# piotrmwojcik/GI-GS

Measured on AMD Instinct MI355X. Metric: train-step renders/sec (fwd+bwd, G-buffer+indirect) at 800x800; PSNR vs the CPU oracle, higher is better.
Workload: dtype f32; 1 GPU; C2 (configs[1] TensoIR lego stand-in): 300k surface Gaussians, 800x800, SH deg 2, GI step=16 start=8 delta=0.0625; P=300000, N=640000, M=9, hip_graphs=on, fused_glue=on, gi_march=proj, rasterizer=whole step = 2 hand-captured hipGraphs (fwd, bwd), asynchronous binning

## Files before the change

gi-gs_amd/build.py:

```python
from __future__ import annotations

import os
import subprocess
import sys
from concurrent.futures import ThreadPoolExecutor

HERE = os.path.dirname(os.path.abspath(__file__))
CSRC = os.path.join(HERE, "csrc")
OBJ = os.environ.get("GIGS_OBJ", os.path.join(HERE, "build"))
LIB = os.environ.get("GIGS_LIB", os.path.join(HERE, "libgigs_hip.so"))
SOURCES = ["api.hip", "preprocess.hip", "binning.hip", "blend.hip", "gi.hip", "pbr.hip", "stage2.hip", "train_glue.hip", "knn.hip", "lpips.hip",
           "image_out.hip", "mesh.hip"]
HIPCC = os.environ.get("HIPCC", "/opt/rocm/bin/hipcc")
FLAGS = [
    "-O3", "--offload-arch=gfx950", "-ffp-contract=off", "-fPIC", "-std=c++17",
    "-Wall", "-Wno-unused-function", "-Wno-unused-result", "-DNDEBUG",
] + os.environ.get("GIGS_EXTRA_FLAGS", "").split()


def _deps(src: str):
    yield os.path.join(CSRC, src)
    yield os.path.join(CSRC, "gigs_common.h")
    yield os.path.join(CSRC, "pixel_ops.h")
    yield os.path.join(HERE, "..", "include", "gigs_hip.h")


def _stale(target: str, deps) -> bool:
    if not os.path.exists(target):
        return True
    t = os.path.getmtime(target)
    return any(os.path.getmtime(d) > t for d in deps if os.path.exists(d))


def build(force: bool = False, save_temps: bool = False, verbose: bool = True) -> str:
    os.makedirs(OBJ, exist_ok=True)
    sources = [s for s in SOURCES if os.path.exists(os.path.join(CSRC, s))]
    objs, jobs = [], []
    for src in sources:
        obj = os.path.join(OBJ, src.replace(".hip", ".o"))
        objs.append(obj)
        if force or _stale(obj, _deps(src)):
            cmd = [HIPCC, *FLAGS, "-c", os.path.join(CSRC, src), "-o", obj]
            if save_temps:
                cmd += ["-save-temps=obj", "-Rpass-analysis=kernel-resource-usage"]
            jobs.append(cmd)

    def run(cmd):
        if verbose:
            print(" ".join(cmd), flush=True)
        r = subprocess.run(cmd, capture_output=True, text=True)
        if r.returncode != 0:
            raise RuntimeError("hipcc failed:\n" + " ".join(cmd) + "\n" + r.stdout + r.stderr)
        return r.stderr

    with ThreadPoolExecutor(max_workers=min(6, max(1, len(jobs)))) as ex:
        logs = list(ex.map(run, jobs))
    if save_temps:
        with open(os.path.join(OBJ, "resource_usage.txt"), "w") as f:
            f.write("\n".join(logs))
    if jobs or force or _stale(LIB, objs):
        run([HIPCC, "--offload-arch=gfx950", "-shared", "-fPIC", "-o", LIB, *objs])
    return LIB


if __name__ == "__main__":
    print(build(force="--force" in sys.argv, save_temps="--save-temps" in sys.argv))
```

gi-gs_amd/csrc/api.hip:

```cpp
#include <cstdarg>
#include <cstdio>
#include <cstdlib>
#include <cstring>
#include <map>
#include <algorithm>
#include <new>
#include <mutex>
#include <vector>

#include "../../include/gigs_hip.h"
#include "gigs_common.h"

namespace {

thread_local char g_err[512] = "";

int fail(int code, const char* fmt, ...) {
  va_list ap;
  va_start(ap, fmt);
  vsnprintf(g_err, sizeof(g_err), fmt, ap);
  va_end(ap);
  return code;
}

// ... 10 lines not shown
    if (_e == hipSuccess && debug) _e = hipStreamSynchronize(s);                           \
    if (_e != hipSuccess)                                                                  \
      return fail(GIGS_ERR_HIP, "stage '%s' failed: %s", name, hipGetErrorString(_e));     \
  } while (0)

std::mutex g_size_mu;
std::map<int, size_t> g_scan_sizes, g_sort_sizes;
size_t scan_size_cached(int P) {
  std::lock_guard<std::mutex> lk(g_size_mu);
  auto it = g_scan_sizes.find(P);
  if (it != g_scan_sizes.end()) return it->second;
  const size_t v = gigs::scan_temp_bytes(P);
  g_scan_sizes[P] = v;
  return v;
}
size_t sort_size_cached(int R) {
  int bucket = 1024;
  while (bucket < R) bucket <<= 1;
  std::lock_guard<std::mutex> lk(g_size_mu);
  auto it = g_sort_sizes.find(bucket);
  if (it != g_sort_sizes.end()) return it->second;
  const size_t v = std::max(gigs::sort_temp_bytes(bucket), gigs::long_space_bytes((size_t)gigs::kBinMaxTiles, (size_t)bucket));
  g_sort_sizes[bucket] = v;
  return v;
}

uint32_t higher_msb(uint32_t n) {
  uint32_t msb = sizeof(n) * 4;
  uint32_t step = msb;
  while (step > 1) {
    step /= 2;
    if (n >> msb) msb += step;
    else msb -= step;
  }
  if (n >> msb) msb++;
  return msb;
}

enum Stage {
  kPreprocess = 0, kScan, kDuplicate, kSort, kRanges, kBlendFwd, kBlendBwd, kPreprocessBwd,
  kDepthToNormal, kSsao, kSsr, kMedian, kBilateral, kMedianBwd, kShadeFwd, kShadeBwd,
  kCubemapFwd, kCubemapBwd, kGbufferPost, kLossFwd, kLossBwd, kL1SsimFwd, kL1SsimBwd, kTvFwd, kTvBwd,
  kMaskedL1, kAdam, kDensifyStats, kGatherRows, kDist2, kActivateFwd, kActivateBwd, kNumStages
};
const char* kStageNames[kNumStages] = {
  "preprocess_fwd", "scan", "duplicate", "sort", "tile_ranges", "blend_fwd", "blend_bwd",
  "preprocess_bwd", "depth_to_normal", "ssao", "ssr", "median3x3", "bilateral3x3",
  "median3x3_bwd", "shade_fwd", "shade_bwd", "cubemap_fwd", "cubemap_bwd", "gbuffer_post",
  "stage2_loss_fwd", "stage2_loss_bwd", "l1_ssim_fwd", "l1_ssim_bwd", "tv_loss_fwd", "tv_loss_bwd", "masked_l1",
  "adam_step", "densify_stats", "gather_rows", "dist2", "activate_fwd", "activate_bwd"};

int env_int(const char* name, int dflt) {
  const char* e = getenv(name);
  return (e && e[0]) ? atoi(e) : dflt;
}
gigs::Options options_from_env() {
  gigs::Options o;
  const char* b = getenv("GIGS_BINNING");
  o.binning_legacy = (b && strcmp(b, "legacy") == 0) ? 1 : 0;
  o.bucket_max_mean = env_int("GIGS_BUCKET_MAX_MEAN", gigs::kBucketMaxMeanList);
  const char* ll = getenv("GIGS_LONG_LISTS");
  o.long_lists = (ll && ll[0]) ? (ll[0] == '1' ? 1 : 0) : -1;
  o.bucket_target = std::max(256, env_int("GIGS_BUCKET_TARGET", 1536));
  o.bin_bands = std::max(0, env_int("GIGS_BIN_BANDS", 0));
  o.blend_cull = env_int("GIGS_BLEND_CULL", 1) != 0;
  o.pre_bwd_sh_skip = env_int("GIGS_PRE_BWD_SH_SKIP", 1) != 0;
  o.gi_march = 4;
  if (const char* e = getenv("GIGS_GI_MARCH")) {
    if (strcmp(e, "exact") == 0) o.gi_march = 0;
  }
  o.gi_cert = env_int("GIGS_GI_CERT", 1) != 0;
  o.gi_interleave = env_int("GIGS_GI_INTERLEAVE", 1) != 0;
  o.gi_tile_log2w = env_int("GIGS_GI_TILE_LOG2W", 3);
  if (o.gi_tile_log2w < 0 || o.gi_tile_log2w > 6) o.gi_tile_log2w = 3;
  o.gi_zero_rays = env_int("GIGS_GI_ZERO_RAYS", 0) != 0;
  o.spec_max8 = env_int("GIGS_SPEC_MAX8", 128);
  o.spec_max16 = env_int("GIGS_SPEC_MAX16", 1500);
  o.shade_lds_floats = env_int("GIGS_SHADE_LDS_FLOATS", 30 * 1024);
  o.shade_bwd_blocks = std::max(0, env_int("GIGS_SHADE_BWD_BLOCKS", 0));
  o.shade_bwd_rows = env_int("GIGS_SHADE_BWD_ROWS", 0) != 0;
  o.spec_sparse = env_int("GIGS_SPEC_SPARSE", 1) != 0;
  o.spec_sparse_permille = env_int("GIGS_SPEC_SPARSE_PERMILLE", 37);
  if (o.spec_sparse_permille < 0 || o.spec_sparse_permille > 1000) o.spec_sparse_permille = 37;
  return o;
}
const gigs::Ctx& ctx_of(const gigs_ctx* c) { return c ? *reinterpret_cast<const gigs::Ctx*>(c) : gigs::default_ctx(); }

struct ProfRec { int stage; hipEvent_t a, b; };
std::mutex g_prof_mu;
bool g_prof_on = false;
std::vector<ProfRec> g_prof_recs;
std::vector<hipEvent_t> g_prof_pool;

hipEvent_t prof_event() {
  if (!g_prof_pool.empty()) {
    hipEvent_t e = g_prof_pool.back();
    g_prof_pool.pop_back();
    return e;
  }
  hipEvent_t e;
  hipEventCreate(&e);
  return e;
}

struct StageScope {
  hipStream_t s;
  int stage;
  bool on;
  hipEvent_t a, b;
  StageScope(int stage_, hipStream_t s_) : s(s_), stage(stage_), on(false) {
    std::lock_guard<std::mutex> lk(g_prof_mu);
    if (!g_prof_on) return;
    on = true;
    a = prof_event();
    b = prof_event();
    hipEventRecord(a, s);
  }
  ~StageScope() {
    if (!on) return;
    hipEventRecord(b, s);
    std::lock_guard<std::mutex> lk(g_prof_mu);
    g_prof_recs.push_back({stage, a, b});
  }
};

}

namespace gigs {
const Options& default_options() {
  static const Options o = options_from_env();
  return o;
}
const Ctx& default_ctx() {
  static const Ctx c = {default_options(), 0u, nullptr, nullptr, 0, nullptr, nullptr};
  return c;
}
}

extern "C" {
__attribute__((visibility("hidden"))) const gigs::Options* gigs_internal_options(const gigs_ctx* ctx) { return &ctx_of(ctx).opt; }
__attribute__((visibility("hidden"))) int gigs_internal_fail(int code, const char* msg) { return fail(code, "%s", msg); }
__attribute__((visibility("hidden"))) void gigs_internal_stage_begin(int stage, void* stream, void** token) {
  *token = new StageScope(stage, (hipStream_t)stream);
}
__attribute__((visibility("hidden"))) void gigs_internal_stage_end(void* token) { delete (StageScope*)token; }
}

extern "C" {

const char* gigs_last_error(void) { return g_err; }
const char* gigs_build_arch(void) { return "gfx950"; }

size_t gigs_required_geom(int P) {
  if (P < 0) { fail(GIGS_ERR_INVALID, "P < 0"); return 0; }
  return gigs::required_bytes<gigs::GeomState>((size_t)P, scan_size_cached(P));
}
size_t gigs_required_image(int width, int height) {
  const size_t N = (size_t)width * height;
  const size_t T = (size_t)((width + GIGS_BLOCK_X - 1) / GIGS_BLOCK_X) * ((height + GIGS_BLOCK_Y - 1) / GIGS_BLOCK_Y);
  return gigs::required_bytes<gigs::ImageState>(N, T);
}
size_t gigs_required_binning(int R) {
  if (R < 0) { fail(GIGS_ERR_INVALID, "R < 0"); return 0; }
  return gigs::required_bytes<gigs::BinningState>((size_t)R, sort_size_cached(R));
}

long long gigs_geom_offset(int P, int which) {
  char* base = nullptr;
  char* p = base;
  gigs::GeomState g = gigs::GeomState::fromChunk(p, (size_t)P, 0);
  const void* ptrs[] = {g.depths, g.pos_view, g.means2D, g.cov3D, g.conic_opacity, g.rgb,
                        g.clamped, g.tiles_touched, g.point_offsets, g.internal_radii, g.brec, g.grec};
  if (which < 0 || which >= (int)(sizeof(ptrs) / sizeof(ptrs[0]))) return -1;
  return (long long)((const char*)ptrs[which] - base);
}
long long gigs_binning_offset(int R, int which) {
  char* base = nullptr;
  char* p = base;
  gigs::BinningState b = gigs::BinningState::fromChunk(p, (size_t)R, 0);
  const void* ptrs[] = {b.keys_unsorted, b.values_unsorted, b.keys, b.point_list, b.hit_mask};
  if (which < 0 || which >= 5) return -1;
  return (long long)((const char*)ptrs[which] - base);
}
long long gigs_image_offset(int width, int height, int which) {
  const size_t N = (size_t)width * height;
  const size_t T = (size_t)((width + GIGS_BLOCK_X - 1) / GIGS_BLOCK_X) * ((height + GIGS_BLOCK_Y - 1) / GIGS_BLOCK_Y);
  char* base = nullptr;
  char* p = base;
  gigs::ImageState s = gigs::ImageState::fromChunk(p, N, T);
  const void* ptrs[] = {s.final_T, s.n_contrib, s.ranges, s.tile_order};
  if (which < 0 || which >= 4) return -1;
  return (long long)((const char*)ptrs[which] - base);
}

gigs_ctx* gigs_ctx_create(void) {
  gigs::Ctx* c = new (std::nothrow) gigs::Ctx(gigs::default_ctx());
  if (!c) fail(GIGS_ERR_ALLOC, "gigs_ctx_create: out of host memory");
  return reinterpret_cast<gigs_ctx*>(c);
}
void gigs_ctx_destroy(gigs_ctx* ctx) { delete reinterpret_cast<gigs::Ctx*>(ctx); }

int gigs_ctx_get_options(const gigs_ctx* ctx, gigs_options* out) {
  if (!out || out->struct_bytes < (int)sizeof(gigs_options)) return fail(GIGS_ERR_INVALID, "gigs_ctx_get_options: set struct_bytes = sizeof(gigs_options)");
  const gigs::Options& o = ctx_of(ctx).opt;
  out->struct_bytes = (int)sizeof(gigs_options);
  out->binning_legacy = o.binning_legacy; out->bucket_max_mean = o.bucket_max_mean; out->long_lists = o.long_lists;
  out->bucket_target = o.bucket_target; out->bin_bands = o.bin_bands; out->blend_cull = o.blend_cull; out->pre_bwd_sh_skip = o.pre_bwd_sh_skip;
  out->gi_march = o.gi_march; out->gi_cert = o.gi_cert; out->gi_interleave = o.gi_interleave;
  out->gi_tile_log2w = o.gi_tile_log2w; out->gi_zero_rays = o.gi_zero_rays; out->spec_max8 = o.spec_max8;
  out->spec_max16 = o.spec_max16; out->shade_lds_floats = o.shade_lds_floats; out->shade_bwd_blocks = o.shade_bwd_blocks;
  out->shade_bwd_rows = o.shade_bwd_rows; out->spec_sparse = o.spec_sparse; out->spec_sparse_permille = o.spec_sparse_permille;
  return 0;
}
int gigs_ctx_set_options(gigs_ctx* ctx, const gigs_options* in) {
  if (!ctx) return fail(GIGS_ERR_INVALID, "gigs_ctx_set_options: the default context is immutable, create one");
  if (!in || in->struct_bytes < (int)sizeof(gigs_options)) return fail(GIGS_ERR_INVALID, "gigs_ctx_set_options: set struct_bytes = sizeof(gigs_options)");
  if (in->gi_march != 0 && in->gi_march != 4) return fail(GIGS_ERR_INVALID, "gi_march must be 0 (exact) or 4 (proj)");
  if (in->gi_tile_log2w < 0 || in->gi_tile_log2w > 6) return fail(GIGS_ERR_INVALID, "gi_tile_log2w must be 0..6");
  if (in->long_lists < -1 || in->long_lists > 1) return fail(GIGS_ERR_INVALID, "long_lists must be -1, 0 or 1");
  if (in->bucket_target < 256 || in->bucket_max_mean < 0 || in->bin_bands < 0 || in->bin_bands > 64)
    return fail(GIGS_ERR_INVALID, "bucket_target >= 256, bucket_max_mean >= 0, 0 <= bin_bands <= 64");
  if (in->spec_max8 < 0 || in->spec_max16 < in->spec_max8) return fail(GIGS_ERR_INVALID, "0 <= spec_max8 <= spec_max16");
  if (in->shade_lds_floats < 0 || in->shade_bwd_blocks < 0) return fail(GIGS_ERR_INVALID, "shade_lds_floats, shade_bwd_blocks >= 0");
  if (in->spec_sparse_permille < 0 || in->spec_sparse_permille > 1000) return fail(GIGS_ERR_INVALID, "0 <= spec_sparse_permille <= 1000");
  gigs::Options& o = reinterpret_cast<gigs::Ctx*>(ctx)->opt;
  o.binning_legacy = in->binning_legacy != 0; o.bucket_max_mean = in->bucket_max_mean; o.long_lists = in->long_lists;
  o.bucket_target = in->bucket_target; o.bin_bands = in->bin_bands; o.blend_cull = in->blend_cull != 0; o.pre_bwd_sh_skip = in->pre_bwd_sh_skip != 0;
  o.gi_march = in->gi_march; o.gi_cert = in->gi_cert != 0; o.gi_interleave = in->gi_interleave != 0;
  o.gi_tile_log2w = in->gi_tile_log2w; o.gi_zero_rays = in->gi_zero_rays != 0; o.spec_max8 = in->spec_max8;
  o.spec_max16 = in->spec_max16; o.shade_lds_floats = in->shade_lds_floats; o.shade_bwd_blocks = in->shade_bwd_blocks;
  o.shade_bwd_rows = in->shade_bwd_rows != 0; o.spec_sparse = in->spec_sparse != 0; o.spec_sparse_permille = in->spec_sparse_permille;
  return 0;
}
int gigs_ctx_set_reuse_binning(gigs_ctx* ctx, int on) {
  if (!ctx) return fail(GIGS_ERR_INVALID, "gigs_ctx_set_reuse_binning: the default context is immutable, create one");
  reinterpret_cast<gigs::Ctx*>(ctx)->reuse_binning = on != 0;
  return 0;
}
int gigs_ctx_set_split_sh(gigs_ctx* ctx, const float* sh_rest) {
  if (!ctx) return fail(GIGS_ERR_INVALID, "gigs_ctx_set_split_sh: the default context is immutable, create one");
  reinterpret_cast<gigs::Ctx*>(ctx)->sh_rest = sh_rest;
  return 0;
}
int gigs_ctx_set_materials_only(gigs_ctx* ctx, void* violations) {
  if (!ctx) return fail(GIGS_ERR_INVALID, "gigs_ctx_set_materials_only: the default context is immutable, create one");
  reinterpret_cast<gigs::Ctx*>(ctx)->materials_only = reinterpret_cast<unsigned*>(violations);
  return 0;
}
int gigs_ctx_set_blend_begin_event(gigs_ctx* ctx, void* hip_event) {
  if (!ctx) return fail(GIGS_ERR_INVALID, "gigs_ctx_set_blend_begin_event: the default context is immutable, create one");
  reinterpret_cast<gigs::Ctx*>(ctx)->blend_begin_event = hip_event;
  return 0;
}

__global__ void __launch_bounds__(64) stream_delay_kernel(unsigned ticks) {
  const unsigned long long t0 = wall_clock64();
  while (wall_clock64() - t0 < (unsigned long long)ticks) __builtin_amdgcn_s_sleep(8);
}

int gigs_stream_delay(unsigned nanoseconds, void* stream) {
  if (nanoseconds == 0) return 0;
  const unsigned ns = nanoseconds > 1000000u ? 1000000u : nanoseconds;
  hipLaunchKernelGGL(stream_delay_kernel, dim3(1), dim3(64), 0, (hipStream_t)stream, (ns + 9u) / 10u);
  return hipGetLastError() == hipSuccess ? 0 : gigs_internal_fail(GIGS_ERR_HIP, "stream_delay: launch failed");
}

int gigs_ctx_set_async_binning(gigs_ctx* ctx, int r_capacity, unsigned* device_counters) {
  if (!ctx) return fail(GIGS_ERR_INVALID, "gigs_ctx_set_async_binning: the default context is immutable, create one");
  gigs::Ctx* c = reinterpret_cast<gigs::Ctx*>(ctx);
  c->async_capacity = r_capacity > 0 ? (unsigned)r_capacity : 0u;
  c->async_counters = r_capacity > 0 ? device_counters : nullptr;
  return 0;
}

void gigs_profile_begin(void) {
  std::lock_guard<std::mutex> lk(g_prof_mu);
  for (auto& r : g_prof_recs) { g_prof_pool.push_back(r.a); g_prof_pool.push_back(r.b); }
  g_prof_recs.clear();
  g_prof_on = true;
}

int gigs_profile_end(float* total_ms, int* launches, int n) {
  std::vector<ProfRec> recs;
  {
    std::lock_guard<std::mutex> lk(g_prof_mu);
    g_prof_on = false;
    recs.swap(g_prof_recs);
  }
  for (int i = 0; i < n; i++) { total_ms[i] = 0.0f; launches[i] = 0; }
  for (auto& r : recs) {
    hipEventSynchronize(r.b);
    float ms = 0.0f;
    if (hipEventElapsedTime(&ms, r.a, r.b) == hipSuccess && r.stage < n) {
      total_ms[r.stage] += ms;
      launches[r.stage] += 1;
    }
  }
  std::lock_guard<std::mutex> lk(g_prof_mu);
  for (auto& r : recs) { g_prof_pool.push_back(r.a); g_prof_pool.push_back(r.b); }
  return kNumStages;
}

const char* gigs_profile_stage_name(int stage) {
  return (stage >= 0 && stage < kNumStages) ? kStageNames[stage] : "";
}

int gigs_forward(gigs_ctx* ctx, gigs_alloc_fn geometryBuffer, void* geom_user, gigs_alloc_fn binningBuffer,
                 void* binning_user, gigs_alloc_fn imageBuffer, void* image_user, int P, int D, int M,
                 const float* background, int width, int height, const float* means3D,
                 const float* shs, const float* colors_precomp, const float* opacities,
                 const float* normal, const float* albedo, const float* roughness,
                 const float* metallic, const float* scales, float scale_modifier,
                 const float* rotations, const float* cov3D_precomp, const float* viewmatrix,
                 const float* projmatrix, const float* cam_pos, float tan_fovx, float tan_fovy,
                 int prefiltered, int argmax_depth, int inference, float* out_color,
                 float* out_opacity, float* out_depth, float* out_normal, float* out_normal_view,
                 float* out_pos, float* out_albedo, float* out_roughness, float* out_metallic,
                 int* radii, int debug, void* stream) {
  (void)prefiltered;
  hipStream_t s = (hipStream_t)stream;
  const gigs::Ctx& cx = ctx_of(ctx);
  const gigs::Options& opt = cx.opt;
  if (P < 0 || width <= 0 || height <= 0) return fail(GIGS_ERR_INVALID, "bad P / image size");
  if (P == 0) return 0;
  if (!geometryBuffer || !binningBuffer || !imageBuffer) return fail(GIGS_ERR_INVALID, "null allocation callback");
  if (!means3D || !opacities || !normal || !albedo || !roughness || !metallic || !viewmatrix ||
      !projmatrix || !cam_pos || !background)
    return fail(GIGS_ERR_INVALID, "null required input");
  if (!shs && !colors_precomp) return fail(GIGS_ERR_INVALID, "provide SHs or precomputed colors");
  if (!cov3D_precomp && (!scales || !rotations)) return fail(GIGS_ERR_INVALID, "provide scales+rotations or cov3D_precomp");
  if (!colors_precomp && (M <= 0 || (D + 1) * (D + 1) > M || D > 3)) return fail(GIGS_ERR_INVALID, "SH degree %d needs (D+1)^2 <= M=%d, D <= 3", D, M);

  gigs::FwdArgs a;
  a.P = P; a.D = D; a.M = M; a.W = width; a.H = height;
  a.gx = (width + GIGS_BLOCK_X - 1) / GIGS_BLOCK_X;
  a.gy = (height + GIGS_BLOCK_Y - 1) / GIGS_BLOCK_Y;
  a.focal_y = height / (2.0f * tan_fovy);
  a.focal_x = width / (2.0f * tan_fovx);
  a.tan_fovx = tan_fovx; a.tan_fovy = tan_fovy; a.scale_modifier = scale_modifier;
  a.means3D = means3D; a.shs = shs; a.colors_precomp = colors_precomp; a.opacities = opacities;
  a.normal = normal; a.albedo = albedo; a.roughness = roughness; a.metallic = metallic;
  a.scales = scales; a.rotations = rotations; a.cov3D_precomp = cov3D_precomp;
  a.viewmatrix = viewmatrix; a.projmatrix = projmatrix; a.cam_pos = cam_pos; a.background = background;
  a.argmax_depth = argmax_depth; a.inference = inference;
  a.shs_rest = (shs && !colors_precomp && M > 1) ? cx.sh_rest : nullptr;

  const size_t scan_sz = scan_size_cached(P);
  const size_t geom_bytes = gigs::required_bytes<gigs::GeomState>((size_t)P, scan_sz);
  char* geom_chunk = geometryBuffer(geom_bytes, geom_user);
  if (!geom_chunk) return fail(GIGS_ERR_ALLOC, "geometry buffer allocation of %zu bytes failed", geom_bytes);
  gigs::GeomState geom = gigs::GeomState::fromChunk(geom_chunk, (size_t)P, scan_sz);
  if (radii == nullptr) radii = geom.internal_radii;

  const size_t N = (size_t)width * height, T = (size_t)a.gx * a.gy;
  const size_t img_bytes = gigs::required_bytes<gigs::ImageState>(N, T);
  char* img_chunk = imageBuffer(img_bytes, image_user);
  if (!img_chunk) return fail(GIGS_ERR_ALLOC, "image buffer allocation of %zu bytes failed", img_bytes);
  gigs::ImageState img = gigs::ImageState::fromChunk(img_chunk, N, T);

  {
    StageScope sc(kPreprocess, s);
    gigs::launch_preprocess_fwd(a, geom, radii, s);
  }
  STAGE_CHECK("preprocess");
  int num_rendered = 0;
  gigs::BinningState bin;
  const unsigned async_cap = cx.async_capacity;
  const bool bucket = !opt.binning_legacy && T <= (size_t)gigs::kBinMaxTiles;
  if (async_cap > 0 && !bucket) return fail(GIGS_ERR_INVALID, "asynchronous binning needs the tile-bucketed path (options.binning_legacy = 0, <= %d tiles)", gigs::kBinMaxTiles);
  auto long_lists = [&](size_t est_mean) {
    if (opt.long_lists >= 0) return opt.long_lists == 1;
    return est_mean > (size_t)opt.bucket_max_mean;
  };
  bool dense = false;
  if (cx.reuse_binning) {
    if (async_cap == 0 || !bucket)
      return fail(GIGS_ERR_INVALID, "reuse_binning needs asynchronous binning (gigs_ctx_set_async_binning) on the tile-bucketed path");
    num_rendered = (int)async_cap;
    const size_t sort_sz = sort_size_cached(num_rendered);
    const size_t bin_bytes = gigs::required_bytes<gigs::BinningState>((size_t)num_rendered, sort_sz);
    char* bin_chunk = binningBuffer(bin_bytes, binning_user);
    if (!bin_chunk) return fail(GIGS_ERR_ALLOC, "binning buffer allocation of %zu bytes failed", bin_bytes);
    bin = gigs::BinningState::fromChunk(bin_chunk, (size_t)num_rendered, sort_sz);
  } else if (bucket) {
    {
      StageScope sc(kDuplicate, s);
      gigs::launch_bin_count(P, radii, a.gx, a.gy, geom, img, s);
      gigs::launch_bin_prefix(P, (int)T, async_cap > 0 ? async_cap : 0x7fffffffu, img, cx.async_counters, s);
    }
    STAGE_CHECK("bin count / prefix");
    if (async_cap > 0) {
      num_rendered = (int)async_cap;
      dense = long_lists((size_t)async_cap / (2 * T));
    } else {
      uint32_t num_rendered_u = 0;
      HIP_TRY(hipMemcpyAsync(&num_rendered_u, img.bin_counters, sizeof(uint32_t), hipMemcpyDeviceToHost, s));
      HIP_TRY(hipStreamSynchronize(s));
      if (num_rendered_u > 0x7fffffffu) return fail(GIGS_ERR_INVALID, "num_rendered overflows int");
      num_rendered = (int)num_rendered_u;
      dense = long_lists((size_t)num_rendered / T);
    }
    const size_t sort_sz = sort_size_cached(num_rendered);
    const size_t bin_bytes = gigs::required_bytes<gigs::BinningState>((size_t)num_rendered, sort_sz);
    char* bin_chunk = binningBuffer(bin_bytes, binning_user);
    if (!bin_chunk) return fail(GIGS_ERR_ALLOC, "binning buffer allocation of %zu bytes failed", bin_bytes);
    bin = gigs::BinningState::fromChunk(bin_chunk, (size_t)num_rendered, sort_sz);
    {
      StageScope sc(kRanges, s);
      gigs::launch_tile_order((int)T, img.ranges, img.tile_order, s);
    }
    {
      StageScope sc(kSort, s);
      const unsigned bands = opt.bin_bands > 0 ? (unsigned)opt.bin_bands : (dense ? 4u : 1u);
      gigs::launch_bin_scatter(P, radii, a.gx, a.gy, (unsigned)num_rendered, bands, geom, bin, img, s);
      if (gigs::launch_bin_sort((int)T, P, dense && num_rendered > 0, (unsigned)opt.bucket_target, (unsigned)num_rendered, bin, img, s) != 0)
        return fail(GIGS_ERR_HIP, "bin_sort: cannot fork the sort streams");
    }
    STAGE_CHECK("bin scatter / sort");
  } else {
  {
    StageScope sc(kScan, s);
    HIP_TRY(gigs::scan_tiles(geom, P, s));
  }
  STAGE_CHECK("scan");
  uint32_t num_rendered_u = 0;
  HIP_TRY(hipMemcpyAsync(&num_rendered_u, geom.point_offsets + P - 1, sizeof(uint32_t), hipMemcpyDeviceToHost, s));
  HIP_TRY(hipStreamSynchronize(s));
  if (num_rendered_u > 0x7fffffffu) return fail(GIGS_ERR_INVALID, "num_rendered overflows int");
  num_rendered = (int)num_rendered_u;

  const size_t sort_sz = sort_size_cached(num_rendered);
  const size_t bin_bytes = gigs::required_bytes<gigs::BinningState>((size_t)num_rendered, sort_sz);
  char* bin_chunk = binningBuffer(bin_bytes, binning_user);
  if (!bin_chunk) return fail(GIGS_ERR_ALLOC, "binning buffer allocation of %zu bytes failed", bin_bytes);
  bin = gigs::BinningState::fromChunk(bin_chunk, (size_t)num_rendered, sort_sz);

  {
    StageScope sc(kDuplicate, s);
    gigs::launch_duplicate(P, radii, a.gx, a.gy, geom, bin, s);
  }
  STAGE_CHECK("duplicateWithKeys");
  const int bit = (int)higher_msb(a.gx * a.gy);
  if (num_rendered > 0) {
    StageScope sc(kSort, s);
    HIP_TRY(gigs::sort_pairs(bin, num_rendered, 32 + bit, s));
  }
  STAGE_CHECK("sort");
  {
    StageScope sc(kRanges, s);
    HIP_TRY(hipMemsetAsync(img.ranges, 0, T * sizeof(uint2), s));
    gigs::launch_tile_ranges(num_rendered, bin, img.ranges, s);
    gigs::launch_tile_order((int)T, img.ranges, img.tile_order, s);
  }
  STAGE_CHECK("identifyTileRanges");
  }
  if (void* ev = cx.blend_begin_event) HIP_TRY(hipEventRecord((hipEvent_t)ev, s));
  {
    StageScope sc(kBlendFwd, s);
    gigs::launch_blend_fwd(a, geom, bin, img, out_color, out_opacity, out_depth, out_normal,
                           out_normal_view, out_pos, out_albedo, out_roughness, out_metallic, opt.blend_cull,
                           (size_t)num_rendered, s, cx.reuse_binning != 0);
  }
  STAGE_CHECK("render");
  return num_rendered;
}

namespace {
struct LiteChunk { char* base; size_t bytes; };
char* lite_chunk_alloc(size_t n, void* user) {
  LiteChunk* c = static_cast<LiteChunk*>(user);
  return n <= c->bytes ? c->base : nullptr;
}
}

int gigs_lite_forward(gigs_ctx* ctx, gigs_alloc_fn geometryBuffer, void* geom_user, gigs_alloc_fn binningBuffer, void* binning_user,
                      gigs_alloc_fn imageBuffer, void* image_user, int P, int D, int M, const float* background, int width,
                      int height, const float* means3D, const float* shs, const float* colors_precomp, const float* opacities,
                      const float* scales, float scale_modifier, const float* rotations, const float* cov3D_precomp,
                      const float* viewmatrix, const float* projmatrix, const float* cam_pos, float tan_fovx, float tan_fovy,
                      int prefiltered, int argmax_depth, float* out_color, float* out_opacity, float* out_depth, int* radii,
                      int debug, void* stream) {
  if (P < 0 || width <= 0 || height <= 0) return fail(GIGS_ERR_INVALID, "bad P / image size");
  if (P == 0) return 0;
  if (!geometryBuffer || !binningBuffer || !imageBuffer) return fail(GIGS_ERR_INVALID, "null allocation callback");
  if (!out_color || !out_opacity || !out_depth) return fail(GIGS_ERR_INVALID, "null output");
  const size_t N = (size_t)width * height;
  const size_t geom_bytes = gigs_required_geom(P), img_bytes = gigs_required_image(width, height);
  const size_t geom_extra = 8 * (size_t)P * sizeof(float) + gigs::kAlign, img_extra = 14 * N * sizeof(float) + gigs::kAlign;
  char* gb = geometryBuffer(geom_bytes + geom_extra, geom_user);
  char* ib = imageBuffer(img_bytes + img_extra, image_user);
  if (!gb || !ib) return fail(GIGS_ERR_ALLOC, "lite_forward: scratch allocation failed");
  auto up = [](char* p) { return reinterpret_cast<char*>((reinterpret_cast<uintptr_t>(p) + gigs::kAlign - 1) & ~(uintptr_t)(gigs::kAlign - 1)); };
  float* zeros = reinterpret_cast<float*>(up(gb + geom_bytes));
  float* spare = reinterpret_cast<float*>(up(ib + img_bytes));
  gigs::launch_zero_words(reinterpret_cast<uint32_t*>(zeros), 8 * (size_t)P, (hipStream_t)stream);
  LiteChunk gc{gb, geom_bytes}, ic{ib, img_bytes};
  return gigs_forward(ctx, lite_chunk_alloc, &gc, binningBuffer, binning_user, lite_chunk_alloc, &ic, P, D, M, background, width, height,
                      means3D, shs, colors_precomp, opacities, zeros, zeros + 3 * (size_t)P, zeros + 6 * (size_t)P,
                      zeros + 7 * (size_t)P, scales, scale_modifier, rotations, cov3D_precomp, viewmatrix, projmatrix, cam_pos,
                      tan_fovx, tan_fovy, prefiltered, argmax_depth, 0, out_color, out_opacity, out_depth, spare, spare + 3 * N,
                      spare + 6 * N, spare + 9 * N, spare + 12 * N, spare + 13 * N, radii, debug, stream);
}

int gigs_backward(gigs_ctx* ctx, int P, int D, int M, int R, const float* background, int width, int height,
                  const float* means3D, const float* shs, const float* colors_precomp,
                  const float* normal, const float* albedo, const float* roughness,
                  const float* metallic, const float* scales, const float* rotations,
                  const float* cov3D_precomp, const float* viewmatrix, const float* projmatrix,
                  const float* cam_pos, const int* radii, float scale_modifier, float tan_fovx,
                  float tan_fovy, char* geom_buffer, char* binning_buffer, char* image_buffer,
                  const float* dL_dpix_depth, const float* dL_dpix, const float* dL_dpix_opacity,
                  const float* dL_dpix_normal, const float* dL_dpix_albedo,
                  const float* dL_dpix_roughness, const float* dL_dpix_metallic, float* dL_dmean2D,
                  float* dL_dconic, float* dL_ddepth, float* dL_dopacity, float* dL_dnormal,
                  float* dL_dalbedo, float* dL_droughness, float* dL_dmetallic, float* dL_dcolor,
                  float* dL_dmean3D, float* dL_dcov3D, float* dL_dsh, float* dL_dscale,
                  float* dL_drot, int debug, void* stream) {
  (void)normal; (void)albedo; (void)roughness; (void)metallic;
  hipStream_t s = (hipStream_t)stream;
  if (P == 0) return 0;
  if (P < 0 || R < 0 || width <= 0 || height <= 0) return fail(GIGS_ERR_INVALID, "bad sizes");
  if (!geom_buffer || !binning_buffer || !image_buffer) return fail(GIGS_ERR_INVALID, "null scratch buffer");
  unsigned* const materials_only = ctx_of(ctx).materials_only;
  if (ctx_of(ctx).sh_rest && shs && M > 1 && !materials_only)
    return fail(GIGS_ERR_INVALID, "a split-SH forward (gigs_ctx_set_split_sh) has a materials-only backward only");
  if (!dL_dmean2D || !dL_dalbedo || !dL_droughness || !dL_dmetallic)
    return fail(GIGS_ERR_INVALID, "null gradient output");
  if (!materials_only && (!dL_dopacity || !dL_dnormal || !dL_dcolor || !dL_dmean3D || !dL_dcov3D || !dL_dscale || !dL_drot ||
                          (shs && !dL_dsh)))
    return fail(GIGS_ERR_INVALID, "null gradient output");

  gigs::BwdArgs a;
  a.P = P; a.D = D; a.M = M; a.R = R; a.W = width; a.H = height;
  a.gx = (width + GIGS_BLOCK_X - 1) / GIGS_BLOCK_X;
  a.gy = (height + GIGS_BLOCK_Y - 1) / GIGS_BLOCK_Y;
  a.focal_y = height / (2.0f * tan_fovy);
  a.focal_x = width / (2.0f * tan_fovx);
  a.tan_fovx = tan_fovx; a.tan_fovy = tan_fovy; a.scale_modifier = scale_modifier;
  a.means3D = means3D; a.shs = shs; a.colors_precomp = colors_precomp; a.scales = scales;
  a.rotations = rotations; a.cov3D_precomp = cov3D_precomp; a.viewmatrix = viewmatrix;
  a.projmatrix = projmatrix; a.cam_pos = cam_pos; a.background = background;
  a.dL_dpix_depth = dL_dpix_depth; a.dL_dpix = dL_dpix; a.dL_dpix_opacity = dL_dpix_opacity;
  a.dL_dpix_normal = dL_dpix_normal; a.dL_dpix_albedo = dL_dpix_albedo;
  a.dL_dpix_roughness = dL_dpix_roughness; a.dL_dpix_metallic = dL_dpix_metallic;
  a.dL_dmean2D = dL_dmean2D; a.dL_dconic = dL_dconic; a.dL_ddepth = dL_ddepth;
  a.dL_dopacity = dL_dopacity; a.dL_dnormal = dL_dnormal; a.dL_dalbedo = dL_dalbedo;
  a.dL_droughness = dL_droughness; a.dL_dmetallic = dL_dmetallic; a.dL_dcolor = dL_dcolor;
  a.dL_dmean3D = dL_dmean3D; a.dL_dcov3D = dL_dcov3D; a.dL_dsh = dL_dsh; a.dL_dscale = dL_dscale;
  a.dL_drot = dL_drot;

  const size_t N = (size_t)width * height, T = (size_t)a.gx * a.gy;
  char* gp = geom_buffer;
  gigs::GeomState geom = gigs::GeomState::fromChunk(gp, (size_t)P, scan_size_cached(P));
  char* bp = binning_buffer;
  gigs::BinningState bin = gigs::BinningState::fromChunk(bp, (size_t)R, 0);
  char* ip = image_buffer;
  gigs::ImageState img = gigs::ImageState::fromChunk(ip, N, T);
  a.radii = radii ? radii : geom.internal_radii;

  {
    StageScope sc(kBlendBwd, s);
    gigs::launch_blend_bwd(a, geom, bin, img, s);
  }
  STAGE_CHECK("render backward");
  {
    StageScope sc(kPreprocessBwd, s);
    gigs::launch_preprocess_bwd(a, geom, ctx_of(ctx).opt.pre_bwd_sh_skip, s, materials_only);
  }
  STAGE_CHECK("preprocess backward");
  return 0;
}

int gigs_mark_visible(int P, const float* means3D, const float* viewmatrix,
                      const float* projmatrix, uint8_t* present, void* stream) {
  (void)projmatrix;
  if (P == 0) return 0;
  if (P < 0 || !means3D || !viewmatrix || !present) return fail(GIGS_ERR_INVALID, "bad argument");
  gigs::launch_mark_visible(P, means3D, viewmatrix, present, (hipStream_t)stream);
  HIP_TRY(hipGetLastError());
  return 0;
// ... 197 lines not shown
```

gi-gs_amd/csrc/binning.hip:

```cpp
#include <algorithm>
#include <cstdlib>
#include <cstring>
#include <mutex>
#include <string.h>
#include <rocprim/block/block_radix_sort.hpp>
#include <rocprim/device/device_radix_sort.hpp>
#include <rocprim/device/device_scan.hpp>

#include "gigs_common.h"

namespace gigs {

size_t scan_temp_bytes(int P) {
  size_t bytes = 0;
  uint32_t* dummy = nullptr;
  (void)rocprim::inclusive_scan(nullptr, bytes, dummy, dummy, (size_t)P, rocprim::plus<uint32_t>());
  return bytes;
}

hipError_t scan_tiles(const GeomState& g, int P, hipStream_t s) {
  size_t bytes = g.scan_size;
  return rocprim::inclusive_scan(g.scan_space, bytes, g.tiles_touched, g.point_offsets, (size_t)P,
                                 rocprim::plus<uint32_t>(), s);
}

size_t sort_temp_bytes(int R) {
  size_t bytes = 0;
  uint64_t* k = nullptr;
  uint32_t* v = nullptr;
  (void)rocprim::radix_sort_pairs(nullptr, bytes, k, k, v, v, (size_t)R, 0, 64);
  return bytes;
}

hipError_t sort_pairs(const BinningState& b, int R, int end_bit, hipStream_t s) {
  size_t bytes = b.sort_size;
  return rocprim::radix_sort_pairs(b.sort_space, bytes, b.keys_unsorted, b.keys, b.values_unsorted,
                                   b.point_list, (size_t)R, 0, (unsigned)end_bit, s);
}

__global__ void __launch_bounds__(256)
duplicate_kernel(int P, const int* __restrict__ radii, unsigned gx, unsigned gy,
                 const float* __restrict__ means2D, const float* __restrict__ depths,
                 const uint32_t* __restrict__ offsets, uint64_t* __restrict__ keys,
                 uint32_t* __restrict__ values) {
  const int idx = blockIdx.x * 256 + threadIdx.x;
  if (idx >= P) return;
  const int r = radii[idx];
  if (r > 0) {
    uint32_t off = (idx == 0) ? 0 : offsets[idx - 1];
    const float2 xy = reinterpret_cast<const float2*>(means2D)[idx];
    unsigned minx, miny, maxx, maxy;
    tile_rect(xy.x, xy.y, r, gx, gy, minx, miny, maxx, maxy);
    const uint32_t dbits = __float_as_uint(depths[idx]);
    for (int y = (int)miny; y < (int)maxy; y++) {
      for (int x = (int)minx; x < (int)maxx; x++) {
        uint64_t key = (uint64_t)(y * gx + x);
        key <<= 32;
        key |= dbits;
        keys[off] = key;
        values[off] = (uint32_t)idx;
        off++;
      }
    }
  }
}

void launch_duplicate(int P, const int* radii, unsigned gx, unsigned gy, const GeomState& g,
                      const BinningState& b, hipStream_t s) {
  hipLaunchKernelGGL(duplicate_kernel, dim3((P + 255) / 256), dim3(256), 0, s, P, radii, gx, gy,
                     g.means2D, g.depths, g.point_offsets, b.keys_unsorted, b.values_unsorted);
}

__global__ void __launch_bounds__(256)
tile_ranges_kernel(int L, const uint64_t* __restrict__ keys, uint2* __restrict__ ranges) {
  const int idx = blockIdx.x * 256 + threadIdx.x;
  if (idx >= L) return;
  const uint32_t currtile = (uint32_t)(keys[idx] >> 32);
  if (idx == 0) {
    ranges[currtile].x = 0;
  } else {
    const uint32_t prevtile = (uint32_t)(keys[idx - 1] >> 32);
    if (currtile != prevtile) {
      ranges[prevtile].y = idx;
      ranges[currtile].x = idx;
    }
  }
  if (idx == L - 1) ranges[currtile].y = L;
}

constexpr int kMaxOrderedTiles = 16384;
__global__ void __launch_bounds__(256)
tile_order_kernel(int T, const uint2* __restrict__ ranges, uint32_t* __restrict__ order, int identity) {
  const int t = blockIdx.x * 4 + (threadIdx.x >> 6), lane = threadIdx.x & 63;
  if (t >= T) return;
  if (identity) {
    if (lane == 0) order[t] = (uint32_t)t;
    return;
  }
  const uint32_t mine = ranges[t].y - ranges[t].x;
  uint32_t rank = 0;
  for (int base = 0; base < T; base += 64) {
    const int u = base + lane;
    const uint32_t other = u < T ? ranges[u].y - ranges[u].x : 0u;
    const bool before = u < T && (other > mine || (other == mine && u < t));
    rank += (uint32_t)__popcll(__ballot(before));
  }
  if (lane == 0) order[rank] = (uint32_t)t;
}

void launch_tile_order(int T, const uint2* ranges, uint32_t* tile_order, hipStream_t s) {
  hipLaunchKernelGGL(tile_order_kernel, dim3((T + 3) / 4), dim3(256), 0, s, T, ranges, tile_order,
                     T > kMaxOrderedTiles ? 1 : 0);
}

void launch_tile_ranges(int R, const BinningState& b, uint2* ranges, hipStream_t s) {
  if (R > 0)
    hipLaunchKernelGGL(tile_ranges_kernel, dim3((R + 255) / 256), dim3(256), 0, s, R, b.keys, ranges);
}


__device__ __forceinline__ bool bin_rect(int idx, int end, const int* __restrict__ radii, const float* __restrict__ means2D,
                                         unsigned gx, unsigned gy, unsigned& minx, unsigned& miny, unsigned& w, unsigned& n,
                                         unsigned row0 = 0u, unsigned row1 = 0xffffffffu) {
  minx = miny = w = n = 0;
  if (idx >= end) return false;
  const int r = radii[idx];
  if (r <= 0) return false;
  const float2 xy = reinterpret_cast<const float2*>(means2D)[idx];
  unsigned maxx, maxy;
  tile_rect(xy.x, xy.y, r, gx, gy, minx, miny, maxx, maxy);
  miny = max(miny, row0);
  maxy = min(maxy, row1);
  if (maxy <= miny) return false;
  w = maxx - minx;
  n = w * (maxy - miny);
  return n > 0;
}

constexpr unsigned kBinWaveExpand = 12;

template <typename Pay, typename F>
__device__ __forceinline__ void bin_walk(int P, const int* __restrict__ radii, const float* __restrict__ means2D, unsigned gx,
                                         unsigned gy, Pay pay, F f, unsigned row0 = 0u, unsigned row1 = 0xffffffffu) {
  const int groups = min((int)kBinGroups, (P + 255) / 256);
  const int chunk = (P + groups - 1) / groups;
  const int begin = blockIdx.x * chunk, end = min(P, begin + chunk);
  const int lane = threadIdx.x & 63;
  for (int base = begin; base < end; base += blockDim.x) {
    const int idx = base + threadIdx.x;
    unsigned minx, miny, w, n;
    const bool any = bin_rect(idx, end, radii, means2D, gx, gy, minx, miny, w, n, row0, row1);
    const unsigned payload = any ? pay(idx) : 0u;
    const bool big = any && n > kBinWaveExpand;
    if (any && !big) {
      unsigned x = 0, y = 0;
      for (unsigned k = 0; k < n; k++) {
        f(idx, (miny + y) * gx + minx + x, payload);
        if (++x == w) { x = 0; y++; }
      }
    }
    unsigned long long m = __builtin_amdgcn_ballot_w64(big);
    while (m) {
      const int l = __builtin_ctzll(m);
      m &= m - 1;
      const unsigned bminx = __shfl(minx, l), bminy = __shfl(miny, l), bw = __shfl(w, l), bn = __shfl(n, l);
      const unsigned bpay = __shfl(payload, l);
      const int bidx = __shfl(idx, l);
      const unsigned bh = bn / max(bw, 1u);
      for (unsigned y = 0; y < bh; y++)
        for (unsigned x = lane; x < bw; x += 64) f(bidx, (bminy + y) * gx + bminx + x, bpay);
    }
  }
}
struct NoPay { __device__ __forceinline__ unsigned operator()(int) const { return 0u; } };

template <int kLanes>
__global__ void __launch_bounds__(kLanes)
bin_count_kernel(int P, int T, const int* __restrict__ radii, const float* __restrict__ means2D, unsigned gx, unsigned gy,
                 uint32_t* __restrict__ bin_hist) {
  extern __shared__ uint32_t s_hist[];
  for (int t = threadIdx.x; t < T; t += kLanes) s_hist[t] = 0;
  __syncthreads();
  bin_walk(P, radii, means2D, gx, gy, NoPay(), [&](int, unsigned tile, unsigned) { atomicAdd(&s_hist[tile], 1u); });
  __syncthreads();
  uint32_t* row = bin_hist + (size_t)blockIdx.x * T;
  for (int t = threadIdx.x; t < T; t += kLanes) row[t] = s_hist[t];
}

__global__ void __launch_bounds__(1024)
bin_prefix_groups_kernel(int groups, int T, uint32_t* __restrict__ bin_hist, uint32_t* __restrict__ totals) {
  __shared__ uint32_t s_q[16][64];
  const int tl = threadIdx.x & 63, q = threadIdx.x >> 6;
  const int t = blockIdx.x * 64 + tl;
  const int per = (groups + 15) / 16, g0 = min(groups, q * per), g1 = min(groups, g0 + per);
  constexpr int kPer = (kBinGroups + 15) / 16;
  uint32_t c[kPer];
  uint32_t run = 0;
  if (t < T) {
#pragma unroll
    for (int k = 0; k < kPer; k++) c[k] = (g0 + k < g1) ? bin_hist[(size_t)(g0 + k) * T + t] : 0u;
#pragma unroll
    for (int k = 0; k < kPer; k++) { const uint32_t v = c[k]; c[k] = run; run += v; }
  }
  s_q[q][tl] = run;
  __syncthreads();
  uint32_t add = 0;
  for (int k = 0; k < q; k++) add += s_q[k][tl];
  if (t < T) {
#pragma unroll
    for (int k = 0; k < kPer; k++)
      if (g0 + k < g1) bin_hist[(size_t)(g0 + k) * T + t] = c[k] + add;
    if (q == 15) totals[t] = add + run;
  }
}

__global__ void __launch_bounds__(1024)
bin_prefix_tiles_kernel(int T, unsigned capacity, unsigned P, const uint32_t* __restrict__ totals, uint2* __restrict__ ranges,
                        uint32_t* __restrict__ tile_start, uint32_t* __restrict__ counters,
                        uint32_t* __restrict__ user_counters) {
  __shared__ uint32_t s_sum[1024];
  const int per = (T + 1023) / 1024;
  const int t0 = threadIdx.x * per, t1 = min(T, t0 + per);
  uint32_t local = 0;
  for (int t = t0; t < t1; t++) local += totals[t];
  s_sum[threadIdx.x] = local;
  __syncthreads();
  for (int off = 1; off < 1024; off <<= 1) {
    const uint32_t v = threadIdx.x >= (unsigned)off ? s_sum[threadIdx.x - off] : 0u;
    __syncthreads();
    s_sum[threadIdx.x] += v;
    __syncthreads();
  }
  uint32_t run = s_sum[threadIdx.x] - local;
  for (int t = t0; t < t1; t++) {
    const uint32_t c = totals[t];
    ranges[t] = c ? make_uint2(min(run, capacity), min(run + c, capacity)) : make_uint2(0u, 0u);
    tile_start[t] = run;
    run += c;
  }
  if (threadIdx.x == 1023) {
    const uint32_t R = s_sum[1023];
    counters[0] = R;
    counters[1] = R > capacity ? R : 0u;
    counters[2] = P;
    counters[3] = capacity;
    if (user_counters) { user_counters[0] = R; user_counters[1] = R > capacity ? R : 0u; }
  }
}

template <int kLanes>
__global__ void __launch_bounds__(kLanes)
bin_scatter_kernel(int P, int T, const int* __restrict__ radii, const float* __restrict__ means2D,
                   const float* __restrict__ depths, unsigned gx, unsigned gy, unsigned capacity, unsigned idx_bits,
                   const uint32_t* __restrict__ bin_hist, const uint32_t* __restrict__ tile_start,
                   uint64_t* __restrict__ keys, unsigned bands) {
  extern __shared__ uint32_t s_cur[];
  const uint32_t* row = bin_hist + (size_t)blockIdx.x * T;
  for (int t = threadIdx.x; t < T; t += kLanes) s_cur[t] = tile_start[t] + row[t];
  __syncthreads();
  const unsigned rows = (gy + bands - 1) / bands;
  for (unsigned b = 0; b < bands; b++)
    bin_walk(P, radii, means2D, gx, gy, NoPay(), [&](int idx, unsigned tile, unsigned) {
      const uint32_t slot = atomicAdd(&s_cur[tile], 1u);
      if (slot < capacity) keys[slot] = ((uint64_t)__float_as_uint(depths[idx]) << idx_bits) | (uint32_t)idx;
    }, b * rows, min(gy, (b + 1) * rows));
}

template <typename Get, typename Put>
__device__ __forceinline__ void bitonic_sort_asc(unsigned n, unsigned npad_log2, unsigned nthreads, Get get, Put put) {
  const unsigned half = (1u << npad_log2) >> 1;
  for (unsigned kb = 1; kb <= npad_log2; kb++) {
    const unsigned k = 1u << kb;
    for (unsigned i = threadIdx.x; i < half; i += nthreads) {
      const unsigned blk = i >> (kb - 1), off = i & ((k >> 1) - 1);
      const unsigned a = (blk << kb) + off, b = (blk << kb) + (k - 1 - off);
      if (b < n) {
        const uint64_t x = get(a), y = get(b);
        if (x > y) { put(a, y); put(b, x); }
      }
    }
    __syncthreads();
    for (int jb = (int)kb - 2; jb >= 0; jb--) {
      const unsigned j = 1u << jb;
      for (unsigned i = threadIdx.x; i < half; i += nthreads) {
        const unsigned a = ((i >> jb) << (jb + 1)) + (i & (j - 1)), b = a + j;
        if (b < n) {
          const uint64_t x = get(a), y = get(b);
          if (x > y) { put(a, y); put(b, x); }
        }
      }
      __syncthreads();
    }
  }
}

template <int kItems, typename Storage, int kBlock = 1024>
__device__ __forceinline__ void sort_tile_radix(Storage& storage, const uint64_t* __restrict__ src, unsigned n, unsigned idx_bits,
                                                uint64_t tile_hi, uint32_t base, uint64_t* __restrict__ keys_out,
                                                uint32_t* __restrict__ point_list) {
  using sorter = rocprim::block_radix_sort<uint64_t, kBlock, kItems, rocprim::empty_type, 1, 1, 8>;
  static_assert(sizeof(Storage) >= sizeof(uint64_t) * kBlock * kItems, "the sorted keys are staged in the sorter's storage");
  const uint64_t idx_mask = (1ull << idx_bits) - 1;
  uint64_t k[kItems];
#pragma unroll
  for (int i = 0; i < kItems; i++) {
    const unsigned idx = threadIdx.x * kItems + i;
    k[i] = idx < n ? src[idx] : ~0ull;
  }
  __shared__ unsigned long long s_diff;
  if (threadIdx.x == 0) s_diff = 0ull;
  __syncthreads();
  {
    const uint64_t ref = src[0];
    uint64_t diff = 0;
#pragma unroll
    for (int i = 0; i < kItems; i++)
      if (threadIdx.x * kItems + i < n) diff |= k[i] ^ ref;
    diff >>= idx_bits;
    if (diff) atomicOr(&s_diff, (unsigned long long)diff);
  }
  __syncthreads();
  const unsigned dd = (unsigned)s_diff;
  const unsigned hi = dd ? 32u - (unsigned)__builtin_clz(dd) : 1u;
  sorter().sort(k, storage, idx_bits, idx_bits + hi);
  __syncthreads();
  uint64_t* s_k = reinterpret_cast<uint64_t*>(&storage);
#pragma unroll
  for (int i = 0; i < kItems; i++) s_k[threadIdx.x * kItems + i] = k[i];
  __syncthreads();
  bool tie = false;
#pragma unroll
  for (int i = 0; i < kItems; i++) {
    const unsigned idx = threadIdx.x * kItems + i;
    if (idx > 0 && idx < n) {
      const uint64_t prev = i > 0 ? k[i - 1] : s_k[idx - 1];
      tie |= (prev >> idx_bits) == (k[i] >> idx_bits) && prev > k[i];
    }
  }
  if (__syncthreads_or(tie)) {
    constexpr unsigned kPairs = (unsigned)kBlock * kItems / 2;
    constexpr int kFixRounds = 64;
    bool more = true;
    for (int round = 0; round < kFixRounds && more; round++) {
      bool swapped = false;
#pragma unroll
      for (int phase = 0; phase < 2; phase++) {
        for (unsigned p = threadIdx.x; p < kPairs; p += kBlock) {
          const unsigned a = 2 * p + phase, c = a + 1;
          if (c < n) {
            const uint64_t x = s_k[a], y = s_k[c];
            if ((x >> idx_bits) == (y >> idx_bits) && x > y) { s_k[a] = y; s_k[c] = x; swapped = true; }
          }
        }
        __syncthreads();
      }
      more = __syncthreads_or(swapped);
    }
    if (more) {
#pragma unroll
      for (int i = 0; i < kItems; i++) k[i] = s_k[threadIdx.x * kItems + i];
      __syncthreads();
      sorter().sort(k, storage, 0, idx_bits + hi);
      __syncthreads();
#pragma unroll
      for (int i = 0; i < kItems; i++) s_k[threadIdx.x * kItems + i] = k[i];
      __syncthreads();
    }
  }
  for (unsigned idx = threadIdx.x; idx < n; idx += kBlock) {
    const uint64_t kk = s_k[idx];
    point_list[base + idx] = (uint32_t)(kk & idx_mask);
    keys_out[base + idx] = tile_hi | (kk >> idx_bits);
  }
  __syncthreads();
}

using SortS4 = rocprim::block_radix_sort<uint64_t, 1024, 4, rocprim::empty_type, 1, 1, 8>::storage_type;
using SortS8 = rocprim::block_radix_sort<uint64_t, 1024, 8, rocprim::empty_type, 1, 1, 8>::storage_type;
using SortS16 = rocprim::block_radix_sort<uint64_t, 1024, 16, rocprim::empty_type, 1, 1, 8>::storage_type;

constexpr unsigned kSmallList = 2048;
using SortSmall = rocprim::block_radix_sort<uint64_t, 256, 8, rocprim::empty_type, 1, 1, 8>::storage_type;
__global__ void __launch_bounds__(256)
bin_sort_small_kernel(int T, unsigned idx_bits, const uint32_t* __restrict__ tile_order, const uint2* __restrict__ ranges,
                      const uint64_t* __restrict__ keys_unsorted, uint64_t* __restrict__ keys_out,
                      uint32_t* __restrict__ point_list) {
  __shared__ SortSmall storage;
  for (int ob = T - 1 - (int)blockIdx.x; ob >= 0; ob -= (int)gridDim.x) {
    const uint32_t tile = tile_order[ob];
    const uint2 rg = ranges[tile];
    const unsigned n = rg.y - rg.x;
    if (n > kSmallList) break;
    if (n == 0) continue;
    sort_tile_radix<8, SortSmall, 256>(storage, keys_unsorted + rg.x, n, idx_bits, (uint64_t)tile << 32, rg.x, keys_out,
                                       point_list);
  }
}

template <bool kBig>
__global__ void __launch_bounds__(1024)
bin_sort_kernel(int T, unsigned idx_bits, const uint32_t* __restrict__ tile_order, const uint2* __restrict__ ranges,
                uint64_t* __restrict__ keys_unsorted, uint64_t* __restrict__ keys_out, uint32_t* __restrict__ point_list) {
  __shared__ union SortStorage {
    SortS4 s4; SortS8 s8;
    char big[kBig ? sizeof(SortS16) : 8];
    __device__ SortStorage() {}
  } storage;
  constexpr unsigned kSplit = 8192;
  for (int ob = blockIdx.x; ob < T; ob += gridDim.x) {
    const uint32_t tile = tile_order[ob];
    const uint2 rg = ranges[tile];
    const unsigned n = rg.y - rg.x;
    if (kBig ? n <= kSplit : n <= kSmallList) break;
    if (!kBig && n > kSplit) continue;
    uint64_t* src = keys_unsorted + rg.x;
    const uint64_t tile_hi = (uint64_t)tile << 32;
    if constexpr (kBig) {
      if (n <= 16384) {
        sort_tile_radix<16>(*reinterpret_cast<SortS16*>(storage.big), src, n, idx_bits, tile_hi, rg.x, keys_out, point_list);
      } else {
        const uint64_t idx_mask = (1ull << idx_bits) - 1;
        unsigned npad = 0;
        while ((1u << npad) < n) npad++;
        bitonic_sort_asc(n, npad, 1024u, [&](unsigned i) { return __builtin_nontemporal_load(src + i); },
                         [&](unsigned i, uint64_t v) { __builtin_nontemporal_store(v, src + i); });
        for (unsigned i = threadIdx.x; i < n; i += 1024) {
          const uint64_t kk = __builtin_nontemporal_load(src + i);
          point_list[rg.x + i] = (uint32_t)(kk & idx_mask);
          keys_out[rg.x + i] = tile_hi | (kk >> idx_bits);
        }
      }
    } else {
      if (n <= 4096) sort_tile_radix<4>(storage.s4, src, n, idx_bits, tile_hi, rg.x, keys_out, point_list);
      else sort_tile_radix<8>(storage.s8, src, n, idx_bits, tile_hi, rg.x, keys_out, point_list);
    }
  }
}

constexpr unsigned kLongList = 8192;
constexpr unsigned kBucketTarget = 1536;
constexpr unsigned kMaxBuckets = 32;
constexpr unsigned kPartChunk = 4096;
#ifndef GIGS_SAMPLE_PER_LANE
#define GIGS_SAMPLE_PER_LANE 2
#endif
constexpr int kSamplePerLane = GIGS_SAMPLE_PER_LANE;
constexpr unsigned kSampleMax = 256 * kSamplePerLane;

struct LongTile { uint32_t tile, B, first_chunk, nchunks; };
struct LongState {
  uint32_t* counts;
  LongTile* tiles;
  uint64_t* splitters;
  uint32_t* bucket_start;
  uint2* chunk_desc;
  uint32_t* chunk_hist;
  uint4* cls_list;
  size_t max_chunks, max_buckets;
  static LongState fromChunk(char*& chunk, size_t T, size_t R) {
    LongState st;
    st.max_chunks = R / kPartChunk + T + 1;
    st.max_buckets = (R / kLongList + 1) * kMaxBuckets;
    carve(chunk, st.counts, 8);
    carve(chunk, st.tiles, T);
    carve(chunk, st.splitters, T * kMaxBuckets);
// ... 106 lines not shown
        run += v;
      }
    uint32_t incl = run;
#pragma unroll
    for (int off = 1; off < 32; off <<= 1) {
      const uint32_t v = __shfl_up(incl, off);
      if ((int)(b & 31) >= off) incl += v;
    }
    const uint32_t start = incl - run;
    if (b < kMaxBuckets) st.bucket_start[(size_t)slot * kMaxBuckets + b] = start;
    const int cls = (b < kMaxBuckets && run) ? (run <= 2048u ? 0 : run <= 8192u ? 1 : run <= 16384u ? 2 : 3) : -1;
#pragma unroll
    for (int c = 0; c < 4; c++) {
      const unsigned long long m = __builtin_amdgcn_ballot_w64(cls == c);
      if (m == 0) continue;
      uint32_t base = 0;
      if (threadIdx.x == 0) base = atomicAdd(&st.counts[4 + c], (uint32_t)__popcll(m));
      base = __shfl(base, 0);
      if (cls == c)
        st.cls_list[(size_t)c * st.max_buckets + base + (uint32_t)__popcll(m & ((1ull << threadIdx.x) - 1))] =
            make_uint4(rg.x + start, run, lt.tile, 0u);
    }
  }
}

__global__ void __launch_bounds__(256)
long_sort_small_kernel(unsigned idx_bits, LongState st, uint64_t* __restrict__ keys_out, uint32_t* __restrict__ point_list) {
  __shared__ SortSmall storage;
  const unsigned count = st.counts[4];
  for (unsigned i = blockIdx.x; i < count; i += gridDim.x) {
    const uint4 d = st.cls_list[i];
    sort_tile_radix<8, SortSmall, 256>(storage, keys_out + d.x, d.y, idx_bits, (uint64_t)d.z << 32, d.x, keys_out, point_list);
  }
}

template <bool kHuge>
__global__ void __launch_bounds__(1024)
long_sort_kernel(unsigned idx_bits, LongState st, uint64_t* __restrict__ keys_out, uint32_t* __restrict__ point_list) {
  __shared__ union SortStorage {
    SortS4 s4; SortS8 s8;
    char big[kHuge ? sizeof(SortS16) : 8];
    __device__ SortStorage() {}
  } storage;
  const unsigned n2 = kHuge ? st.counts[6] : 0u, count = kHuge ? n2 + st.counts[7] : st.counts[5];
  for (unsigned i = blockIdx.x; i < count; i += gridDim.x) {
    const uint4 d = !kHuge ? st.cls_list[st.max_buckets + i]
                           : i < n2 ? st.cls_list[2 * st.max_buckets + i] : st.cls_list[3 * st.max_buckets + (i - n2)];
    const unsigned n = d.y;
    uint64_t* src = keys_out + d.x;
    const uint64_t tile_hi = (uint64_t)d.z << 32;
    if constexpr (!kHuge) {
      if (n <= 4096) sort_tile_radix<4>(storage.s4, src, n, idx_bits, tile_hi, d.x, keys_out, point_list);
      else sort_tile_radix<8>(storage.s8, src, n, idx_bits, tile_hi, d.x, keys_out, point_list);
    } else if (n <= 16384) {
      sort_tile_radix<16>(*reinterpret_cast<SortS16*>(storage.big), src, n, idx_bits, tile_hi, d.x, keys_out, point_list);
    } else {
      const uint64_t idx_mask = (1ull << idx_bits) - 1;
      unsigned npad = 0;
      while ((1u << npad) < n) npad++;
      bitonic_sort_asc(n, npad, 1024u, [&](unsigned k) { return __builtin_nontemporal_load(src + k); },
                       [&](unsigned k, uint64_t v) { __builtin_nontemporal_store(v, src + k); });
      for (unsigned k = threadIdx.x; k < n; k += 1024) {
        const uint64_t kk = __builtin_nontemporal_load(src + k);
        point_list[d.x + k] = (uint32_t)(kk & idx_mask);
        keys_out[d.x + k] = tile_hi | (kk >> idx_bits);
      }
      __syncthreads();
    }
  }
}

__global__ void __launch_bounds__(256) zero_words_kernel(uint32_t* __restrict__ p, size_t n) {
  const size_t n4 = n / 4, stride = (size_t)gridDim.x * 256;
  uint4* p4 = reinterpret_cast<uint4*>(p);
  for (size_t i = (size_t)blockIdx.x * 256 + threadIdx.x; i < n4; i += stride) p4[i] = make_uint4(0, 0, 0, 0);
  if (blockIdx.x == 0 && threadIdx.x < (n & 3)) p[4 * n4 + threadIdx.x] = 0;
}
void launch_zero_words(uint32_t* p, size_t n, hipStream_t s) {
  if (n == 0) return;
  const unsigned blocks = (unsigned)std::min<size_t>((n / 4 + 255) / 256 + 1, 2048);
  hipLaunchKernelGGL(zero_words_kernel, dim3(blocks), dim3(256), 0, s, p, n);
}

static unsigned bin_index_bits(int P) {
  unsigned ib = 1;
  while (ib < 32 && (1ull << ib) < (unsigned long long)P) ib++;
  return ib;
}

static int bin_groups(int P) { return std::min((int)kBinGroups, (P + 255) / 256); }
constexpr int kWideWalk = 1 << 20;

void launch_bin_count(int P, const int* radii, unsigned gx, unsigned gy, const GeomState& g, const ImageState& img, hipStream_t s) {
  const int T = (int)(gx * gy);
  if (P >= kWideWalk)
    hipLaunchKernelGGL(bin_count_kernel<1024>, dim3(bin_groups(P)), dim3(1024), (size_t)T * sizeof(uint32_t), s, P, T, radii,
                       g.means2D, gx, gy, img.bin_hist);
  else
    hipLaunchKernelGGL(bin_count_kernel<256>, dim3(bin_groups(P)), dim3(256), (size_t)T * sizeof(uint32_t), s, P, T, radii,
                       g.means2D, gx, gy, img.bin_hist);
}

void launch_bin_prefix(int P, int T, unsigned capacity, const ImageState& img, unsigned* user_counters, hipStream_t s) {
  uint32_t* totals = img.bin_hist + (size_t)(kBinGroups) * T;
  uint32_t* tile_start = img.bin_hist + (size_t)(kBinGroups + 1) * T;
  hipLaunchKernelGGL(bin_prefix_groups_kernel, dim3((T + 63) / 64), dim3(1024), 0, s, bin_groups(P), T, img.bin_hist, totals);
  hipLaunchKernelGGL(bin_prefix_tiles_kernel, dim3(1), dim3(1024), 0, s, T, capacity, (unsigned)P, totals, img.ranges, tile_start,
                     img.bin_counters, user_counters);
}

void launch_bin_scatter(int P, const int* radii, unsigned gx, unsigned gy, unsigned capacity, unsigned bands, const GeomState& g,
                        const BinningState& b, const ImageState& img, hipStream_t s) {
  const int T = (int)(gx * gy);
  const uint32_t* tile_start = img.bin_hist + (size_t)(kBinGroups + 1) * T;
  bands = std::max(1u, std::min(bands, gy));
  if (P >= kWideWalk)
    hipLaunchKernelGGL(bin_scatter_kernel<1024>, dim3(bin_groups(P)), dim3(1024), (size_t)T * sizeof(uint32_t), s, P, T, radii,
                       g.means2D, g.depths, gx, gy, capacity, bin_index_bits(P), img.bin_hist, tile_start, b.keys_unsorted, bands);
  else
    hipLaunchKernelGGL(bin_scatter_kernel<256>, dim3(bin_groups(P)), dim3(256), (size_t)T * sizeof(uint32_t), s, P, T, radii,
                       g.means2D, g.depths, gx, gy, capacity, bin_index_bits(P), img.bin_hist, tile_start, b.keys_unsorted, bands);
}

void launch_long_lists(int T, int P, unsigned target, unsigned capacity, const BinningState& b, const ImageState& img, hipStream_t s) {
  char* space = b.sort_space;
  LongState st = LongState::fromChunk(space, (size_t)T, (size_t)capacity);
  const unsigned ib = bin_index_bits(P);
  launch_zero_words(st.counts, 8, s);
  if (target < 256u) target = kBucketTarget;
  hipLaunchKernelGGL(long_plan_kernel, dim3(std::min(T, 1024)), dim3(256), 0, s, T, ib, target, img.ranges, b.keys_unsorted, st);
  hipLaunchKernelGGL(long_chunks_kernel<false>, dim3(2048), dim3(256), 0, s, img.ranges, b.keys_unsorted, b.keys, st);
  hipLaunchKernelGGL(long_prefix_kernel, dim3(std::min(T, 1024)), dim3(64), 0, s, img.ranges, st);
  hipLaunchKernelGGL(long_chunks_kernel<true>, dim3(2048), dim3(256), 0, s, img.ranges, b.keys_unsorted, b.keys, st);
  hipLaunchKernelGGL(long_sort_kernel<true>, dim3(256), dim3(1024), 0, s, ib, st, b.keys, b.point_list);
  hipLaunchKernelGGL(long_sort_kernel<false>, dim3(512), dim3(1024), 0, s, ib, st, b.keys, b.point_list);
  hipLaunchKernelGGL(long_sort_small_kernel, dim3(2048), dim3(256), 0, s, ib, st, b.keys, b.point_list);
}

int launch_bin_sort(int T, int P, bool long_lists, unsigned bucket_target, unsigned capacity, const BinningState& b, const ImageState& img,
                    hipStream_t s) {
  const unsigned ib = bin_index_bits(P);
  if (long_lists)
    launch_long_lists(T, P, bucket_target, capacity, b, img, s);
  else
    hipLaunchKernelGGL(bin_sort_kernel<true>, dim3(std::min(T, 256)), dim3(1024), 0, s, T, ib, img.tile_order, img.ranges,
                       b.keys_unsorted, b.keys, b.point_list);
  hipLaunchKernelGGL(bin_sort_kernel<false>, dim3(std::min(T, 512)), dim3(1024), 0, s, T, ib, img.tile_order, img.ranges,
                     b.keys_unsorted, b.keys, b.point_list);
  hipLaunchKernelGGL(bin_sort_small_kernel, dim3(std::min(T, 2048)), dim3(256), 0, s, T, ib, img.tile_order, img.ranges,
                     b.keys_unsorted, b.keys, b.point_list);
  return 0;
}

}
```

gi-gs_amd/csrc/blend.hip:

```cpp
#include <cstdlib>
#include "gigs_common.h"

namespace gigs {

typedef float f32x2 __attribute__((ext_vector_type(2)));

__device__ __forceinline__ unsigned long long ballot64(bool p) { return __builtin_amdgcn_ballot_w64(p); }

constexpr int kLongTile = 2048;

template <int kCtrl, int kRowMask = 0xf, int kBankMask = 0xf>
__device__ __forceinline__ float dpp_mov0(float v) {
  return __int_as_float(__builtin_amdgcn_update_dpp(0, __float_as_int(v), kCtrl, kRowMask, kBankMask, false));
}
template <int N>
__device__ __forceinline__ void wave_sum_n(float* v);
template <>
__device__ __forceinline__ void wave_sum_n<1>(float* v) {
  asm("s_nop 4\n\t"
      "v_add_f32_dpp %0, %0, %0 quad_perm:[1,0,3,2] row_mask:0xf bank_mask:0xf bound_ctrl:1\n\t"
      "s_nop 1\n\t"
      "v_add_f32_dpp %0, %0, %0 quad_perm:[2,3,0,1] row_mask:0xf bank_mask:0xf bound_ctrl:1\n\t"
      "s_nop 1\n\t"
      "v_add_f32_dpp %0, %0, %0 row_ror:4 row_mask:0xf bank_mask:0xf bound_ctrl:1\n\t"
      "s_nop 1\n\t"
      "v_add_f32_dpp %0, %0, %0 row_ror:8 row_mask:0xf bank_mask:0xf bound_ctrl:1\n\t"
      "s_nop 1\n\t"
      "v_add_f32_dpp %0, %0, %0 row_bcast:15 row_mask:0xa bank_mask:0xf\n\t"
      "s_nop 1\n\t"
      "v_add_f32_dpp %0, %0, %0 row_bcast:31 row_mask:0xc bank_mask:0xf\n\t"
      "s_nop 1"
      : "+v"(v[0]));
}
template <>
__device__ __forceinline__ void wave_sum_n<3>(float* v) {
  asm("s_nop 4\n\t"
      "v_add_f32_dpp %0, %0, %0 quad_perm:[1,0,3,2] row_mask:0xf bank_mask:0xf bound_ctrl:1\n\t"
      "v_add_f32_dpp %1, %1, %1 quad_perm:[1,0,3,2] row_mask:0xf bank_mask:0xf bound_ctrl:1\n\t"
      "v_add_f32_dpp %2, %2, %2 quad_perm:[1,0,3,2] row_mask:0xf bank_mask:0xf bound_ctrl:1\n\t"
      "v_add_f32_dpp %0, %0, %0 quad_perm:[2,3,0,1] row_mask:0xf bank_mask:0xf bound_ctrl:1\n\t"
      "v_add_f32_dpp %1, %1, %1 quad_perm:[2,3,0,1] row_mask:0xf bank_mask:0xf bound_ctrl:1\n\t"
      "v_add_f32_dpp %2, %2, %2 quad_perm:[2,3,0,1] row_mask:0xf bank_mask:0xf bound_ctrl:1\n\t"
      "v_add_f32_dpp %0, %0, %0 row_ror:4 row_mask:0xf bank_mask:0xf bound_ctrl:1\n\t"
      "v_add_f32_dpp %1, %1, %1 row_ror:4 row_mask:0xf bank_mask:0xf bound_ctrl:1\n\t"
      "v_add_f32_dpp %2, %2, %2 row_ror:4 row_mask:0xf bank_mask:0xf bound_ctrl:1\n\t"
      "v_add_f32_dpp %0, %0, %0 row_ror:8 row_mask:0xf bank_mask:0xf bound_ctrl:1\n\t"
      "v_add_f32_dpp %1, %1, %1 row_ror:8 row_mask:0xf bank_mask:0xf bound_ctrl:1\n\t"
      "v_add_f32_dpp %2, %2, %2 row_ror:8 row_mask:0xf bank_mask:0xf bound_ctrl:1\n\t"
      "v_add_f32_dpp %0, %0, %0 row_bcast:15 row_mask:0xa bank_mask:0xf\n\t"
      "v_add_f32_dpp %1, %1, %1 row_bcast:15 row_mask:0xa bank_mask:0xf\n\t"
      "v_add_f32_dpp %2, %2, %2 row_bcast:15 row_mask:0xa bank_mask:0xf\n\t"
      "v_add_f32_dpp %0, %0, %0 row_bcast:31 row_mask:0xc bank_mask:0xf\n\t"
      "v_add_f32_dpp %1, %1, %1 row_bcast:31 row_mask:0xc bank_mask:0xf\n\t"
      "v_add_f32_dpp %2, %2, %2 row_bcast:31 row_mask:0xc bank_mask:0xf"
      : "+v"(v[0]), "+v"(v[1]), "+v"(v[2]));
}
template <>
__device__ __forceinline__ void wave_sum_n<5>(float* v) {
  asm("s_nop 4\n\t"
      "v_add_f32_dpp %0, %0, %0 quad_perm:[1,0,3,2] row_mask:0xf bank_mask:0xf bound_ctrl:1\n\t"
      "v_add_f32_dpp %1, %1, %1 quad_perm:[1,0,3,2] row_mask:0xf bank_mask:0xf bound_ctrl:1\n\t"
      "v_add_f32_dpp %2, %2, %2 quad_perm:[1,0,3,2] row_mask:0xf bank_mask:0xf bound_ctrl:1\n\t"
      "v_add_f32_dpp %3, %3, %3 quad_perm:[1,0,3,2] row_mask:0xf bank_mask:0xf bound_ctrl:1\n\t"
      "v_add_f32_dpp %4, %4, %4 quad_perm:[1,0,3,2] row_mask:0xf bank_mask:0xf bound_ctrl:1\n\t"
      "v_add_f32_dpp %0, %0, %0 quad_perm:[2,3,0,1] row_mask:0xf bank_mask:0xf bound_ctrl:1\n\t"
      "v_add_f32_dpp %1, %1, %1 quad_perm:[2,3,0,1] row_mask:0xf bank_mask:0xf bound_ctrl:1\n\t"
      "v_add_f32_dpp %2, %2, %2 quad_perm:[2,3,0,1] row_mask:0xf bank_mask:0xf bound_ctrl:1\n\t"
      "v_add_f32_dpp %3, %3, %3 quad_perm:[2,3,0,1] row_mask:0xf bank_mask:0xf bound_ctrl:1\n\t"
      "v_add_f32_dpp %4, %4, %4 quad_perm:[2,3,0,1] row_mask:0xf bank_mask:0xf bound_ctrl:1\n\t"
      "v_add_f32_dpp %0, %0, %0 row_ror:4 row_mask:0xf bank_mask:0xf bound_ctrl:1\n\t"
      "v_add_f32_dpp %1, %1, %1 row_ror:4 row_mask:0xf bank_mask:0xf bound_ctrl:1\n\t"
      "v_add_f32_dpp %2, %2, %2 row_ror:4 row_mask:0xf bank_mask:0xf bound_ctrl:1\n\t"
      "v_add_f32_dpp %3, %3, %3 row_ror:4 row_mask:0xf bank_mask:0xf bound_ctrl:1\n\t"
      "v_add_f32_dpp %4, %4, %4 row_ror:4 row_mask:0xf bank_mask:0xf bound_ctrl:1\n\t"
      "v_add_f32_dpp %0, %0, %0 row_ror:8 row_mask:0xf bank_mask:0xf bound_ctrl:1\n\t"
      "v_add_f32_dpp %1, %1, %1 row_ror:8 row_mask:0xf bank_mask:0xf bound_ctrl:1\n\t"
      "v_add_f32_dpp %2, %2, %2 row_ror:8 row_mask:0xf bank_mask:0xf bound_ctrl:1\n\t"
      "v_add_f32_dpp %3, %3, %3 row_ror:8 row_mask:0xf bank_mask:0xf bound_ctrl:1\n\t"
      "v_add_f32_dpp %4, %4, %4 row_ror:8 row_mask:0xf bank_mask:0xf bound_ctrl:1\n\t"
      "v_add_f32_dpp %0, %0, %0 row_bcast:15 row_mask:0xa bank_mask:0xf\n\t"
      "v_add_f32_dpp %1, %1, %1 row_bcast:15 row_mask:0xa bank_mask:0xf\n\t"
      "v_add_f32_dpp %2, %2, %2 row_bcast:15 row_mask:0xa bank_mask:0xf\n\t"
      "v_add_f32_dpp %3, %3, %3 row_bcast:15 row_mask:0xa bank_mask:0xf\n\t"
      "v_add_f32_dpp %4, %4, %4 row_bcast:15 row_mask:0xa bank_mask:0xf\n\t"
// ... 25 lines not shown
      "v_add_f32_dpp %5, %5, %5 quad_perm:[2,3,0,1] row_mask:0xf bank_mask:0xf bound_ctrl:1\n\t"
      "v_add_f32_dpp %6, %6, %6 quad_perm:[2,3,0,1] row_mask:0xf bank_mask:0xf bound_ctrl:1\n\t"
      "v_add_f32_dpp %7, %7, %7 quad_perm:[2,3,0,1] row_mask:0xf bank_mask:0xf bound_ctrl:1\n\t"
      "v_add_f32_dpp %8, %8, %8 quad_perm:[2,3,0,1] row_mask:0xf bank_mask:0xf bound_ctrl:1\n\t"
      "v_add_f32_dpp %9, %9, %9 quad_perm:[2,3,0,1] row_mask:0xf bank_mask:0xf bound_ctrl:1\n\t"
      "v_add_f32_dpp %0, %0, %0 row_ror:4 row_mask:0xf bank_mask:0xf bound_ctrl:1\n\t"
      "v_add_f32_dpp %1, %1, %1 row_ror:4 row_mask:0xf bank_mask:0xf bound_ctrl:1\n\t"
      "v_add_f32_dpp %2, %2, %2 row_ror:4 row_mask:0xf bank_mask:0xf bound_ctrl:1\n\t"
      "v_add_f32_dpp %3, %3, %3 row_ror:4 row_mask:0xf bank_mask:0xf bound_ctrl:1\n\t"
      "v_add_f32_dpp %4, %4, %4 row_ror:4 row_mask:0xf bank_mask:0xf bound_ctrl:1\n\t"
      "v_add_f32_dpp %5, %5, %5 row_ror:4 row_mask:0xf bank_mask:0xf bound_ctrl:1\n\t"
      "v_add_f32_dpp %6, %6, %6 row_ror:4 row_mask:0xf bank_mask:0xf bound_ctrl:1\n\t"
      "v_add_f32_dpp %7, %7, %7 row_ror:4 row_mask:0xf bank_mask:0xf bound_ctrl:1\n\t"
      "v_add_f32_dpp %8, %8, %8 row_ror:4 row_mask:0xf bank_mask:0xf bound_ctrl:1\n\t"
      "v_add_f32_dpp %9, %9, %9 row_ror:4 row_mask:0xf bank_mask:0xf bound_ctrl:1\n\t"
      "v_add_f32_dpp %0, %0, %0 row_ror:8 row_mask:0xf bank_mask:0xf bound_ctrl:1\n\t"
      "v_add_f32_dpp %1, %1, %1 row_ror:8 row_mask:0xf bank_mask:0xf bound_ctrl:1\n\t"
      "v_add_f32_dpp %2, %2, %2 row_ror:8 row_mask:0xf bank_mask:0xf bound_ctrl:1\n\t"
      "v_add_f32_dpp %3, %3, %3 row_ror:8 row_mask:0xf bank_mask:0xf bound_ctrl:1\n\t"
      "v_add_f32_dpp %4, %4, %4 row_ror:8 row_mask:0xf bank_mask:0xf bound_ctrl:1\n\t"
      "v_add_f32_dpp %5, %5, %5 row_ror:8 row_mask:0xf bank_mask:0xf bound_ctrl:1\n\t"
      "v_add_f32_dpp %6, %6, %6 row_ror:8 row_mask:0xf bank_mask:0xf bound_ctrl:1\n\t"
      "v_add_f32_dpp %7, %7, %7 row_ror:8 row_mask:0xf bank_mask:0xf bound_ctrl:1\n\t"
      "v_add_f32_dpp %8, %8, %8 row_ror:8 row_mask:0xf bank_mask:0xf bound_ctrl:1\n\t"
      "v_add_f32_dpp %9, %9, %9 row_ror:8 row_mask:0xf bank_mask:0xf bound_ctrl:1\n\t"
      "v_add_f32_dpp %0, %0, %0 row_bcast:15 row_mask:0xa bank_mask:0xf\n\t"
      "v_add_f32_dpp %1, %1, %1 row_bcast:15 row_mask:0xa bank_mask:0xf\n\t"
      "v_add_f32_dpp %2, %2, %2 row_bcast:15 row_mask:0xa bank_mask:0xf\n\t"
      "v_add_f32_dpp %3, %3, %3 row_bcast:15 row_mask:0xa bank_mask:0xf\n\t"
      "v_add_f32_dpp %4, %4, %4 row_bcast:15 row_mask:0xa bank_mask:0xf\n\t"
      "v_add_f32_dpp %5, %5, %5 row_bcast:15 row_mask:0xa bank_mask:0xf\n\t"
      "v_add_f32_dpp %6, %6, %6 row_bcast:15 row_mask:0xa bank_mask:0xf\n\t"
      "v_add_f32_dpp %7, %7, %7 row_bcast:15 row_mask:0xa bank_mask:0xf\n\t"
      "v_add_f32_dpp %8, %8, %8 row_bcast:15 row_mask:0xa bank_mask:0xf\n\t"
      "v_add_f32_dpp %9, %9, %9 row_bcast:15 row_mask:0xa bank_mask:0xf\n\t"
      "v_add_f32_dpp %0, %0, %0 row_bcast:31 row_mask:0xc bank_mask:0xf\n\t"
      "v_add_f32_dpp %1, %1, %1 row_bcast:31 row_mask:0xc bank_mask:0xf\n\t"
      "v_add_f32_dpp %2, %2, %2 row_bcast:31 row_mask:0xc bank_mask:0xf\n\t"
      "v_add_f32_dpp %3, %3, %3 row_bcast:31 row_mask:0xc bank_mask:0xf\n\t"
      "v_add_f32_dpp %4, %4, %4 row_bcast:31 row_mask:0xc bank_mask:0xf\n\t"
      "v_add_f32_dpp %5, %5, %5 row_bcast:31 row_mask:0xc bank_mask:0xf\n\t"
      "v_add_f32_dpp %6, %6, %6 row_bcast:31 row_mask:0xc bank_mask:0xf\n\t"
      "v_add_f32_dpp %7, %7, %7 row_bcast:31 row_mask:0xc bank_mask:0xf\n\t"
      "v_add_f32_dpp %8, %8, %8 row_bcast:31 row_mask:0xc bank_mask:0xf\n\t"
      "v_add_f32_dpp %9, %9, %9 row_bcast:31 row_mask:0xc bank_mask:0xf"
      : "+v"(v[0]), "+v"(v[1]), "+v"(v[2]), "+v"(v[3]), "+v"(v[4]), "+v"(v[5]), "+v"(v[6]), "+v"(v[7]), "+v"(v[8]), "+v"(v[9]));
}
__device__ __forceinline__ float wave_sum_lane63(float v) {
  wave_sum_n<1>(&v);
  return v;
}

__device__ __forceinline__ bool box_never_blends(float ua, float ub, float va, float vb, float A, float B, float C, float op) {
  if (op < 1.0f / 255.0f) return true;
  if (!(A > 0.0f && C > 0.0f && A * C - B * B > 0.0f)) return false;
  if (ua <= 0.0f && ub >= 0.0f && va <= 0.0f && vb >= 0.0f) return false;
  const float iA = __builtin_amdgcn_rcpf(A), iC = __builtin_amdgcn_rcpf(C);
  auto f = [&](float u, float v) { return 0.5f * (A * u * u + C * v * v) + B * u * v; };
  const float q1 = f(ua, fminf(fmaxf(-B * ua * iC, va), vb));
  const float q2 = f(ub, fminf(fmaxf(-B * ub * iC, va), vb));
  const float q3 = f(fminf(fmaxf(-B * va * iA, ua), ub), va);
  const float q4 = f(fminf(fmaxf(-B * vb * iA, ua), ub), vb);
  const float qmin = fminf(fminf(q1, q2), fminf(q3, q4));
  const float um = fmaxf(fabsf(ua), fabsf(ub)), vm = fmaxf(fabsf(va), fabsf(vb));
  const float smax = 0.5f * (A * um * um + C * vm * vm) + fabsf(B) * um * vm;
  const float tau = __logf(255.0f * op);
  return qmin > tau + 1e-5f * smax + 1e-2f;
}

__device__ __forceinline__ float blend_exp(float x) {
  const float L = 0x1.715476p+0f, L_lo = 0x1.4ae0cp-26f;
  const float y = x * L;
  const float lo = __builtin_fmaf(x, L_lo, __builtin_fmaf(x, L, -y));
  const float e = __builtin_amdgcn_exp2f(y);
  return __builtin_fmaf(e, lo * 0x1.62e43p-1f, e);
}

struct BlendOut {
  float *color, *opacity, *depth, *normal, *normal_view, *pos, *albedo, *roughness, *metallic;
};

__global__ void __launch_bounds__(GIGS_TILE)
blend_fwd_kernel(int W, int H, unsigned gx, const uint2* __restrict__ ranges,
                 const uint32_t* __restrict__ point_list, const float4* __restrict__ brec,
                 const float* __restrict__ viewmatrix, const float* __restrict__ bg_color,
                 uint32_t* __restrict__ n_contrib, float* __restrict__ final_T, BlendOut o,
                 int argmax_depth, int inference, uint8_t* __restrict__ hit_mask, size_t hit_stride, int cull,
                 const uint32_t* __restrict__ tile_order, const uint32_t* __restrict__ reuse_guard, uint2 reuse_expect) {
  __shared__ float4 s_rec[4][GIGS_BREC_F4 * 64];

  const unsigned tile = tile_order[blockIdx.x];
  const unsigned ty = tile / gx, tx = tile - ty * gx;
  const int tid = threadIdx.x, wave = tid >> 6, lane = tid & 63;
  const unsigned px = tx * GIGS_BLOCK_X + (wave & 1) * 8 + (lane & 7);
  const unsigned py = ty * GIGS_BLOCK_Y + (wave >> 1) * 8 + (lane >> 3);
  const bool inside = px < (unsigned)W && py < (unsigned)H;
  const size_t pix_id = (size_t)W * py + px;
  float pixfx = (float)px, pixfy = (float)py;
  asm volatile("" : "+v"(pixfx), "+v"(pixfy));
  bool done = !inside;

  uint2 range = ranges[tile];
  if (reuse_guard && (reuse_guard[2] != reuse_expect.x || reuse_guard[3] != reuse_expect.y || range.y > reuse_expect.y ||
                      range.x > range.y))
    range = make_uint2(0u, 0u);
  const int n = (int)(range.y - range.x);
  if (n > kLongTile) __builtin_amdgcn_s_setprio(3);
  float4* sw = s_rec[wave];
  uint8_t* hit = hit_mask + (size_t)wave * hit_stride + range.x;

  float T = 1.0f;
  uint32_t last_contributor = 0;
  f32x2 C01 = {0, 0}, C2P0 = {0, 0}, N01 = {0, 0}, N2P1 = {0, 0}, A01 = {0, 0}, A2P2 = {0, 0}, RM = {0, 0};
  float O = 0;
  float max_weight = 0.0f, e0 = 0, e1 = 0, e2 = 0;

  const float qx0 = (float)(tx * GIGS_BLOCK_X + (wave & 1) * 8), qy0 = (float)(ty * GIGS_BLOCK_Y + (wave >> 1) * 8);

  float4 rec[GIGS_BREC_F4];
#pragma unroll
  for (int k = 0; k < GIGS_BREC_F4; k++) rec[k] = make_float4(0, 0, 0, 0);
  if (lane < n) {
    const float4* src = brec + (size_t)point_list[range.x + lane] * GIGS_BREC_F4;
#pragma unroll
    for (int k = 0; k < GIGS_BREC_F4; k++) rec[k] = src[k];
  }
  uint32_t id_next = (64 + lane < n) ? point_list[range.x + 64 + lane] : 0u;

  int base = 0;
  bool wave_done = ballot64(!done) == 0ull;
  for (; base < n && !wave_done; base += 64) {
    const bool valid = base + lane < n;
    const float4 q0 = rec[0], q1 = rec[1];
#pragma unroll
    for (int k = 0; k < GIGS_BREC_F4; k++) sw[k * 64 + lane] = rec[k];
    if (base + 64 + lane < n) {
      const float4* src = brec + (size_t)id_next * GIGS_BREC_F4;
#pragma unroll
      for (int k = 0; k < GIGS_BREC_F4; k++) rec[k] = src[k];
    }
    id_next = (base + 128 + lane < n) ? point_list[range.x + base + 128 + lane] : 0u;

    const unsigned long long open_px = ballot64(!done);
    unsigned long long fold = open_px | (open_px >> 32);
    fold |= fold >> 16;
    fold |= fold >> 8;
    const unsigned cols = (unsigned)fold & 0xffu;
    const float bx0 = qx0 + (float)__builtin_ctz(cols), bx1 = qx0 + (float)(31 - __builtin_clz(cols));
    const float by0 = qy0 + (float)(__builtin_ctzll(open_px) >> 3), by1 = qy0 + (float)((63 - __builtin_clzll(open_px)) >> 3);
    unsigned long long m = ballot64(
        valid && !(cull && box_never_blends(q0.x - bx1, q0.x - bx0, q0.y - by1, q0.y - by0, q1.x, q1.y, q1.z, q1.w)));
    unsigned long long hits = 0ull;
    __builtin_amdgcn_fence(__ATOMIC_RELEASE, "wavefront");
    __builtin_amdgcn_wave_barrier();
    while (m != 0ull) {
      const int bit = __builtin_ctzll(m);
      m &= m - 1ull;
      const float4 r0 = sw[bit];
      const float4 r1 = sw[64 + bit];
      const float dx = r0.x - pixfx, dy = r0.y - pixfy;
      const float power = -0.5f * (r1.x * dx * dx + r1.z * dy * dy) - r1.y * dx * dy;
      const float alpha = fminf(0.99f, r1.w * blend_exp(power));
      const float test_T = T * (1 - alpha);
      const bool cand = !done && !(power > 0.0f) && !(alpha < 1.0f / 255.0f);
      const bool stop = cand && test_T < 0.0001f;
      const bool contrib = cand && !stop;
      if (stop) done = true;
      if (ballot64(contrib) != 0ull) hits |= 1ull << bit;
      if (contrib) {
        const float weight = alpha * T;
        const float4 r2 = sw[2 * 64 + bit];
        const float4 r3 = sw[3 * 64 + bit];
        const float4 r4 = sw[4 * 64 + bit];
        const f32x2 w2 = {weight, weight};
        C01 += f32x2{r2.x, r2.y} * w2; C2P0 += f32x2{r2.z, r2.w} * w2;
        N01 += f32x2{r3.x, r3.y} * w2; N2P1 += f32x2{r3.z, r3.w} * w2;
        A01 += f32x2{r4.x, r4.y} * w2; A2P2 += f32x2{r4.z, r4.w} * w2;
        RM += f32x2{r0.z, r0.w} * w2;
        O += weight;
        if (argmax_depth) {
          if (weight > max_weight) {
            e0 = r2.w; e1 = r3.w; e2 = r4.w;
            max_weight = weight;
          }
        }
        T = test_T;
        last_contributor = (uint32_t)(base + bit + 1);
      }
    }
    wave_done = ballot64(!done) == 0ull;
    __builtin_amdgcn_wave_barrier();
    if (valid) hit[base + lane] = (uint8_t)((hits >> lane) & 1ull);
  }
  for (int i = base + lane; i < n; i += 64) hit[i] = 0;

  const float C0 = C01.x, C1 = C01.y, C2 = C2P0.x, P0 = C2P0.y, N0 = N01.x, N1 = N01.y, N2 = N2P1.x, P1 = N2P1.y;
  const float A0 = A01.x, A1 = A01.y, A2 = A2P2.x, P2 = A2P2.y, Rr = RM.x, Mm = RM.y;
  if (inside) {
    const size_t HW = (size_t)H * W;
    final_T[pix_id] = T;
    n_contrib[pix_id] = last_contributor;
    const v3 nv = normalize3(xform_vec_4x3({N0, N1, N2}, viewmatrix));
    o.normal_view[pix_id] = nv.x;
    o.normal_view[HW + pix_id] = nv.y;
    o.normal_view[2 * HW + pix_id] = nv.z;
    o.color[pix_id] = C0 + T * bg_color[0];
    o.color[HW + pix_id] = C1 + T * bg_color[1];
    o.color[2 * HW + pix_id] = C2 + T * bg_color[2];
    o.normal[pix_id] = N0; o.normal[HW + pix_id] = N1; o.normal[2 * HW + pix_id] = N2;
    o.albedo[pix_id] = A0; o.albedo[HW + pix_id] = A1; o.albedo[2 * HW + pix_id] = A2;
    o.roughness[pix_id] = inference ? (Rr + T) : Rr;
    o.metallic[pix_id] = Mm;
    if ((double)O > 1e-6) {
      o.depth[pix_id] = argmax_depth ? e2 : P2 / O;
      o.pos[pix_id] = argmax_depth ? e0 : P0 / O;
      o.pos[HW + pix_id] = argmax_depth ? e1 : P1 / O;
      o.pos[2 * HW + pix_id] = argmax_depth ? e2 : P2 / O;
    } else {
      o.depth[pix_id] = 0.0f;
      o.pos[pix_id] = 0.0f;
      o.pos[HW + pix_id] = 0.0f;
      o.pos[2 * HW + pix_id] = 0.0f;
    }
    o.opacity[pix_id] = O;
  }
}

void launch_blend_fwd(const FwdArgs& a, const GeomState& g, const BinningState& b,
                      const ImageState& im, float* out_color, float* out_opacity,
                      float* out_depth, float* out_normal, float* out_normal_view, float* out_pos,
                      float* out_albedo, float* out_roughness, float* out_metallic, int cull, size_t hit_stride,
                      hipStream_t s, bool reused_lists) {
  BlendOut o{out_color, out_opacity, out_depth, out_normal, out_normal_view,
             out_pos, out_albedo, out_roughness, out_metallic};
  hipLaunchKernelGGL(blend_fwd_kernel, dim3(a.gx * a.gy), dim3(GIGS_TILE), 0, s, a.W, a.H, a.gx,
                     im.ranges, b.point_list, g.brec, a.viewmatrix, a.background, im.n_contrib,
                     im.final_T, o, a.argmax_depth, a.inference, b.hit_mask, hit_stride, cull, im.tile_order,
                     reused_lists ? (const uint32_t*)im.bin_counters : (const uint32_t*)nullptr,
                     make_uint2((unsigned)a.P, (unsigned)hit_stride));
}

struct BlendGradIn {
  const float *depth, *color, *opacity, *normal, *albedo, *roughness, *metallic;
};

__global__ void __launch_bounds__(GIGS_TILE)
blend_bwd_kernel(int W, int H, unsigned gx, const uint2* __restrict__ ranges,
                 const uint32_t* __restrict__ point_list, const float4* __restrict__ brec,
                 const float* __restrict__ bg_color, const float* __restrict__ final_Ts,
                 const uint32_t* __restrict__ n_contrib, BlendGradIn gi, float* __restrict__ grec,
                 const uint8_t* __restrict__ hit_mask, size_t hit_stride, const uint32_t* __restrict__ tile_order) {
  __shared__ float4 s_rec[4][3 * 64];
  __shared__ __align__(16) float s_sum[4][2][GIGS_GREC];

  const unsigned tile = tile_order[blockIdx.x];
  const unsigned ty = tile / gx, tx = tile - ty * gx;
  const int tid = threadIdx.x, wave = tid >> 6, lane = tid & 63;
  const unsigned px = tx * GIGS_BLOCK_X + (wave & 1) * 8 + (lane & 7);
  const unsigned py = ty * GIGS_BLOCK_Y + (wave >> 1) * 8 + (lane >> 3);
  const bool inside = px < (unsigned)W && py < (unsigned)H;
  const size_t pix_id = (size_t)W * py + px;
  const size_t HW = (size_t)H * W;
  const float pixfx = (float)px, pixfy = (float)py;

  const uint2 range = ranges[tile];
  const int n = (int)(range.y - range.x);
  if (n > kLongTile) __builtin_amdgcn_s_setprio(3);
  float4* sw = s_rec[wave];
  float* ssum = s_sum[wave][0];
  float* ssum2 = s_sum[wave][1];
  const uint8_t* hit = hit_mask + (size_t)wave * hit_stride + range.x;

  const float T_final = inside ? final_Ts[pix_id] : 0;
  float T = T_final;
  const int last_contributor = inside ? (int)n_contrib[pix_id] : 0;

  float last_alpha = 0.0f, accum_opacity = 0.0f;
  float ar0 = 0, ar1 = 0, ar2 = 0, lc0 = 0, lc1 = 0, lc2 = 0;
  float dp0 = 0, dp1 = 0, dp2 = 0, dn0 = 0, dn1 = 0, dn2 = 0, da0 = 0, da1 = 0, da2 = 0;
  float dop = 0, drg = 0, dmt = 0, ddp = 0;
  if (inside) {
    if (gi.color) { dp0 = gi.color[pix_id]; dp1 = gi.color[HW + pix_id]; dp2 = gi.color[2 * HW + pix_id]; }
    if (gi.normal) { dn0 = gi.normal[pix_id]; dn1 = gi.normal[HW + pix_id]; dn2 = gi.normal[2 * HW + pix_id]; }
    if (gi.albedo) { da0 = gi.albedo[pix_id]; da1 = gi.albedo[HW + pix_id]; da2 = gi.albedo[2 * HW + pix_id]; }
    if (gi.opacity) dop = gi.opacity[pix_id];
    if (gi.roughness) drg = gi.roughness[pix_id];
    if (gi.metallic) dmt = gi.metallic[pix_id];
    if (gi.depth) ddp = gi.depth[pix_id];
  }
  if (px == 0 || px == (unsigned)(W - 1) || py == 0 || py == (unsigned)(H - 1)) {
    dn0 = dn1 = dn2 = 0.0f;
  }
  const float ddelx_dx = (float)(0.5 * W), ddely_dy = (float)(0.5 * H);
  const float bg_dot_dpixel = 0 + bg_color[0] * dp0 + bg_color[1] * dp1 + bg_color[2] * dp2;
  const bool any_geo = __any((dp0 != 0.0f) | (dp1 != 0.0f) | (dp2 != 0.0f) | (dop != 0.0f)) != 0;
  const bool any_nrm = __any((dn0 != 0.0f) | (dn1 != 0.0f) | (dn2 != 0.0f)) != 0;
  const bool any_mat = __any((da0 != 0.0f) | (da1 != 0.0f) | (da2 != 0.0f) | (drg != 0.0f) | (dmt != 0.0f)) != 0;
  const bool any_dep = __any(ddp != 0.0f) != 0;
  if (!(any_geo || any_nrm || any_mat || any_dep)) return;

  auto fetch_id = [&](int base, uint32_t& id, bool& h) {
    const int idx = n - 1 - (base + lane);
    h = idx >= 0 && hit[idx] != 0;
    id = h ? point_list[range.x + idx] : 0u;
  };
  uint32_t id_cur, id_next;
  bool h_cur, h_next;
  fetch_id(0, id_cur, h_cur);
  fetch_id(64, id_next, h_next);
  float4 rec[3];
#pragma unroll
  for (int k = 0; k < 3; k++) rec[k] = make_float4(0, 0, 0, 0);
  if (h_cur) {
    const float4* src = brec + (size_t)id_cur * GIGS_BREC_F4;
#pragma unroll
    for (int k = 0; k < 3; k++) rec[k] = src[k];
  }

  if (lane < GIGS_GREC) { ssum[lane] = 0.0f; ssum2[lane] = 0.0f; }
  const bool mat_only = any_mat && !any_geo && !any_nrm && !any_dep;
  for (int base = 0; base < n; base += 64) {
    unsigned long long m = __ballot(h_cur);
// ... 159 lines not shown
```

gi-gs_amd/csrc/gi.hip:

```cpp
#include <cmath>
#include <cstdlib>
#include <cstring>
#include <mutex>
#include <type_traits>
#include <vector>

#include "gigs_common.h"
#include "pixel_ops.h"

namespace gigs {

constexpr float kPiF = 3.14159265358979323846f;

__device__ __forceinline__ v3 get_position(int x, int y, float cx, float cy, float fx, float fy,
                                           float depth) {
  const v3 dir = {((float)x - cx) / fx, ((float)y - cy) / fy, 1.0f};
  return dir * depth;
}

__global__ void __launch_bounds__(256)
depth_to_normal_kernel(int W, int H, float fx, float fy, const float* __restrict__ vm,
                       const float* __restrict__ depth_map, float* __restrict__ normal_out,
                       float* __restrict__ depth_pos) {
  const int x = blockIdx.x * 16 + (threadIdx.x & 15);
// ... 580 lines not shown
            const u64 h = look & __builtin_amdgcn_ballot_w64(fabsf(z[k][g] - mid) <= c.hh);
            hit[k] = __builtin_amdgcn_inverse_ballot_w64(h) ? (int)off[k][g] : hit[k];
            open_m[k] &= ~((need & ~inb[k][g]) | h);
          }
        }
    }
    if ((open_m[0] | open_m[1]) == 0ull) break;
  }
}

__device__ __forceinline__ FastPix make_fast(const GiParams& p, v3 pos, float cx, float cy) {
  FastPix c;
  c.cxy = f32x2{cx + 0.49999997f, cy + 0.49999997f};
  c.cm = 0.5f * (p.bias - p.thick) - 0.0000001f;
  c.hh = 0.5f * (p.bias + p.thick);
  c.Axy = f32x2{pos.x * p.fx, pos.y * p.fy};
  c.Dz = pos.z + 0.0000001f;
  return c;
}
struct FastTbn { v3 mx, my, mz; };
__device__ __forceinline__ CertPix make_cert(const GiParams& p, const FastPix& c, float inv_scale) {
  CertPix cp;
  cp.Axy = c.Axy * inv_scale;
  cp.cxy = c.cxy * inv_scale;
  cp.scale = 1.0f / inv_scale;
  cp.bw = p.cert_w;
  cp.bh = p.cert_h;
  return cp;
}
__device__ __forceinline__ FastTbn make_fast_tbn(const GiParams& p, const Tbn& m, float a, float xy_scale = 1.0f) {
  const float s = a * a * p.radius;
  const float sx = (s * p.fx) * xy_scale, sy = (s * p.fy) * xy_scale;
  FastTbn r;
  r.mx = {m.t.x * sx, m.b.x * sx, m.n.x * sx};
  r.my = {m.t.y * sy, m.b.y * sy, m.n.y * sy};
  r.mz = {m.t.z * s, m.b.z * s, m.n.z * s};
  return r;
}
__device__ __forceinline__ void fast_ray(const FastTbn& ft, float4 ra, f32x2& bxy, float& bz) {
  const float bx = __builtin_fmaf(ft.mx.z, ra.z, __builtin_fmaf(ft.mx.y, ra.y, ft.mx.x * ra.x));
  const float by = __builtin_fmaf(ft.my.z, ra.z, __builtin_fmaf(ft.my.y, ra.y, ft.my.x * ra.x));
  bz = __builtin_fmaf(ft.mz.z, ra.z, __builtin_fmaf(ft.mz.y, ra.y, ft.mz.x * ra.x));
  bxy = f32x2{bx, by};
}

#ifndef GIGS_GI_GROUP
#define GIGS_GI_GROUP 4
#endif
#ifndef GIGS_GI_RAYS
#define GIGS_GI_RAYS 2
#endif
constexpr int kGiGroup = GIGS_GI_GROUP;
constexpr int kGiRays = GIGS_GI_RAYS;
constexpr int kGiWaves = 4;
constexpr int kGiTileLog2W = 3;

__device__ __forceinline__ bool gi_pixel(const GiParams& p, int& x, int& y, int& wave) {
  const int lane = threadIdx.x & 63;
  wave = __builtin_amdgcn_readfirstlane(threadIdx.x >> 6);
  x = (blockIdx.x << p.tile_log2w) + (lane & ((1 << p.tile_log2w) - 1));
  y = blockIdx.y * (64 >> p.tile_log2w) + (lane >> p.tile_log2w);
  return x < p.W && y < p.H;
}

#ifndef GIGS_GI_WAVES
#define GIGS_GI_WAVES 0
#endif
#if GIGS_GI_WAVES > 0
#define GIGS_GI_OCC __attribute__((amdgpu_waves_per_eu(GIGS_GI_WAVES, GIGS_GI_WAVES)))
#define GIGS_SSR_OCC GIGS_GI_OCC
#else
#define GIGS_GI_OCC
#define GIGS_SSR_OCC __attribute__((amdgpu_waves_per_eu(5)))
#endif
#ifndef GIGS_SSR_MULTI_WAVES
#define GIGS_SSR_MULTI_WAVES 4
#endif
#if GIGS_GI_WAVES > 0
#define GIGS_SSR_OCC_L(L) GIGS_SSR_OCC
#else
#define GIGS_SSR_OCC_L(L) __attribute__((amdgpu_waves_per_eu((L) == 1 ? 5 : GIGS_SSR_MULTI_WAVES)))
#endif

enum class March { kExactPow2, kExact, kProj, kProjCert };
constexpr bool march_is_proj(March m) { return m == March::kProj || m == March::kProjCert; }

template <March kMarch>
__global__ void __launch_bounds__(256) GIGS_GI_OCC
ssao_kernel(GiParams p, const float4* __restrict__ rays, float sum_w,
            const float* __restrict__ nrm, const float* __restrict__ pos_map,
            float* __restrict__ occlusion, const float2* __restrict__ cert_tab) {
  __shared__ float s_part[kGiWaves][64];
  extern __shared__ float2 s_cert[];
  constexpr bool kPow2 = kMarch == March::kExactPow2, kCert = kMarch == March::kProjCert;
  constexpr int kCertOff = sizeof(float) * kGiWaves * 64;
  if constexpr (kCert) {
    if ((unsigned)(size_t)s_cert != (unsigned)kCertOff) __builtin_trap();
    const int nb = (p.cert_w + 1) * (p.cert_h + 1);
    for (int i = threadIdx.x; i < nb; i += 256) s_cert[i] = cert_tab[i];
    __syncthreads();
  }
  int x, y, wave;
  const bool inside = gi_pixel(p, x, y, wave);
  const int lane = threadIdx.x & 63;
  const size_t HW = (size_t)p.H * p.W;
  const size_t pix_id = inside ? (size_t)p.W * y + x : 0;
  float occ = 0.0f;
  if (inside && p.start < p.step) {
    const Tbn tbn = make_tbn({nrm[pix_id], nrm[HW + pix_id], nrm[2 * HW + pix_id]});
    if (!tbn_never_hits(tbn)) {
      const v3 pos = {pos_map[pix_id], pos_map[HW + pix_id], pos_map[2 * HW + pix_id]};
      const __amdgpu_buffer_rsrc_t pos_z = z_plane_rsrc(pos_map + 2 * HW, HW);
      const float a = 1 + pos.z / 100;
      const float cx = float(p.W) / 2.0f, cy = float(p.H) / 2.0f;
      const int chunk = (p.n_live + kGiWaves - 1) / kGiWaves;
      const int r0 = wave * chunk, r1 = min(p.n_live, r0 + chunk);
      const bool mag_ok = gi_mag_ok(pos, a, p.radius);
      if constexpr (march_is_proj(kMarch)) {
        if (mag_ok) {
          const FastPix c = make_fast(p, pos, cx, cy);
          const float inv_scale = kCert ? __uint_as_float((127u - (unsigned)p.cert_shift) << 23) : 1.0f;
          const FastTbn ft = make_fast_tbn(p, tbn, a, inv_scale);
          const CertPix cp = make_cert(p, c, inv_scale);
          const int rs = p.ray_interleave ? 2 * wave : r0, re = p.ray_interleave ? p.n_live : r1;
          const int rstep = p.ray_interleave ? 2 * kGiWaves : 2;
          auto pair = [&](int r, int rb) {
            f32x2 Bxy[2], Bz2;
            float bz0, bz1;
            fast_ray(ft, rays[2 * r], Bxy[0], bz0);
            fast_ray(ft, rays[2 * rb], Bxy[1], bz1);
            Bz2 = f32x2{bz0, bz1};
            int hit[2];
            if constexpr (kCert) march2_cert<kGiGroup, kCertOff>(p, c, cp, Bxy, Bz2, pos_z, hit);
            else march2_fast<kGiGroup>(p, c, Bxy, Bz2, pos_z, hit);
            occ += hit[0] >= 0 ? rays[2 * r + 1].y : 0.0f;
            occ += (hit[1] >= 0 && rb != r) ? rays[2 * rb + 1].y : 0.0f;
          };
          for (int r = rs; r < re; r += rstep) pair(r, min(r + 1, re - 1));
          for (int r = p.n_live + wave; r < p.nrays; r += kGiWaves) pair(r, r);
        }
      } else {
      const unsigned sv_min_bits = gi_sv_min_bits(a, p.radius, p.inv_step);
      int r = r0;
      for (; r + kGiRays <= r1; r += kGiRays) {
        v3 sv[kGiRays];
        float w[kGiRays];
        int hit[kGiRays];
#pragma unroll
        for (int k = 0; k < kGiRays; k++) {
          const float4 ra = rays[2 * (r + k)];
          w[k] = rays[2 * (r + k) + 1].y;
          sv[k] = tbn_apply(tbn, ra.x, ra.y, ra.z);
        }
        march<kPow2, kGiGroup, kGiRays>(p, pos, a, sv, cx, cy, pos_z, mag_ok, sv_min_bits, hit);
#pragma unroll
        for (int k = 0; k < kGiRays; k++) occ += hit[k] >= 0 ? w[k] : 0.0f;
      }
      auto single = [&](int q) {
        const float4 ra = rays[2 * q];
        const v3 sv = tbn_apply(tbn, ra.x, ra.y, ra.z);
        int hit;
        march<kPow2, kGiGroup, 1>(p, pos, a, &sv, cx, cy, pos_z, mag_ok, sv_min_bits, &hit);
        occ += hit >= 0 ? rays[2 * q + 1].y : 0.0f;
      };
      for (; r < r1; r++) single(r);
      for (r = p.n_live + wave; r < p.nrays; r += kGiWaves) single(r);
      }
    }
  }
  s_part[wave][lane] = occ;
  __syncthreads();
  if (wave == 0 && inside) {
    const float tot = ((s_part[0][lane] + s_part[1][lane]) + s_part[2][lane]) + s_part[3][lane];
    if (sum_w > 0.0f)
      occlusion[pix_id] = fmaxf(0.0f, fminf(1.0f, (float)(1.0 - (double)(tot / sum_w))));
    else
      occlusion[pix_id] = 1.0f;
  }
}

struct SsrHits {
  unsigned* counts;
  const unsigned* offsets;
  uint2* entries;
  unsigned capacity;
};

__device__ __forceinline__ void ssr_finish(v3 diffuse, const Tbn& tbn, v3 pos, size_t pix_id, size_t HW, int nrays_total,
                                           const float* __restrict__ albedo_map, const float* __restrict__ metallic_map,
                                           const float* __restrict__ F0_map, float* __restrict__ color, float* __restrict__ abd) {
  const v3 N = tbn.n;
  const v3 alb = {albedo_map[pix_id], albedo_map[HW + pix_id], albedo_map[2 * HW + pix_id]};
  const v3 F0 = {F0_map[pix_id], F0_map[HW + pix_id], F0_map[2 * HW + pix_id]};
  const float metallic = metallic_map[pix_id];
  const v3 V = normalize3({-pos.x, -pos.y, -pos.z});
  const float cosTheta = fmaxf(dot3(N, V), (float)0.0000001);
  const float pw = (float)pow((double)fminf(fmaxf((float)(1.0 - (double)cosTheta), (float)0.000001), 1.0f), 5.0);
  const v3 F = {F0.x + (1.0f - F0.x) * pw, F0.y + (1.0f - F0.y) * pw, F0.z + (1.0f - F0.z) * pw};
  v3 kD = {(float)(1.0 - (double)F.x), (float)(1.0 - (double)F.y), (float)(1.0 - (double)F.z)};
  kD.x = (float)((double)kD.x * (1.0 - (double)metallic));
  kD.y = (float)((double)kD.y * (1.0 - (double)metallic));
  kD.z = (float)((double)kD.z * (1.0 - (double)metallic));
  const float nrSamples = (float)nrays_total;
  v3 gd;
  if (nrSamples > 0.0f) {
    gd.x = (float)((double)(kPiF * diffuse.x) * (1.0 / (double)nrSamples) * (double)kD.x);
    gd.y = (float)((double)(kPiF * diffuse.y) * (1.0 / (double)nrSamples) * (double)kD.y);
    gd.z = (float)((double)(kPiF * diffuse.z) * (1.0 / (double)nrSamples) * (double)kD.z);
    diffuse = {gd.x * alb.x, gd.y * alb.y, gd.z * alb.z};
  } else {
    diffuse = {(float)0.0000001, (float)0.0000001, (float)0.0000001};
    gd = diffuse;
  }
  color[pix_id] = diffuse.x;
  color[HW + pix_id] = diffuse.y;
  color[2 * HW + pix_id] = diffuse.z;
  abd[pix_id] = gd.x;
  abd[HW + pix_id] = gd.y;
  abd[2 * HW + pix_id] = gd.z;
}

template <March kMarch, int kHits = 0, int kLights = 1>
__global__ void __launch_bounds__(256) GIGS_SSR_OCC_L(kLights)
ssr_kernel(GiParams p, const float4* __restrict__ rays, const float* __restrict__ nrm,
           const float* __restrict__ pos_map, const float* __restrict__ rgb,
           const float* __restrict__ albedo_map, const float* __restrict__ metallic_map,
           const float* __restrict__ F0_map, float* __restrict__ color, float* __restrict__ abd,
           const float2* __restrict__ cert_tab, SsrHits hits) {
  __shared__ float s_part[kGiWaves][3][64];
  extern __shared__ float2 s_cert[];
  static_assert(kHits == 0 || march_is_proj(kMarch), "hit lists exist for the projective march only");
  constexpr bool kPow2 = kMarch == March::kExactPow2, kCert = kMarch == March::kProjCert;
  constexpr int kCertOff = sizeof(float) * kGiWaves * 3 * 64;
  if constexpr (kCert) {
    if ((unsigned)(size_t)s_cert != (unsigned)kCertOff) __builtin_trap();
    const int nb = (p.cert_w + 1) * (p.cert_h + 1);
    for (int i = threadIdx.x; i < nb; i += 256) s_cert[i] = cert_tab[i];
    __syncthreads();
  }
  int x, y, wave;
  const bool inside = gi_pixel(p, x, y, wave);
  const int lane = threadIdx.x & 63;
  const size_t HW = (size_t)p.H * p.W;
  const size_t pix_id = inside ? (size_t)p.W * y + x : 0;
  const v3 pos = {pos_map[pix_id], pos_map[HW + pix_id], pos_map[2 * HW + pix_id]};
  const Tbn tbn = make_tbn({nrm[pix_id], nrm[HW + pix_id], nrm[2 * HW + pix_id]});
  v3 diffuse[kLights];
#pragma unroll
  for (int l = 0; l < kLights; l++) diffuse[l] = {0, 0, 0};
  unsigned hpos = 0;
  if (inside && p.start < p.step && !tbn_never_hits(tbn)) {
    const __amdgpu_buffer_rsrc_t pos_z = z_plane_rsrc(pos_map + 2 * HW, HW);
    const float a = 1 + pos.z / 100;
    const float cx = float(p.W) / 2.0f, cy = float(p.H) / 2.0f;
    const int chunk = (p.n_live + kGiWaves - 1) / kGiWaves;
    const int r0 = wave * chunk, r1 = min(p.n_live, r0 + chunk);
    const bool mag_ok = gi_mag_ok(pos, a, p.radius);
    if constexpr (kHits == 2) hpos = hits.offsets[4 * pix_id + wave];
    auto add_hit = [&](int q, float cos_t, float sin_t, int ray) {
      if (q >= 0) {
#pragma unroll
        for (int l = 0; l < kLights; l++) {
          const float* c = rgb + (size_t)l * 3 * HW;
          diffuse[l].x += c[q] * cos_t * sin_t;
          diffuse[l].y += c[HW + q] * cos_t * sin_t;
          diffuse[l].z += c[2 * HW + q] * cos_t * sin_t;
        }
        if constexpr (kHits == 1) hpos++;
        if constexpr (kHits == 2) {
          if (hpos < hits.capacity) hits.entries[hpos] = make_uint2((unsigned)q, (unsigned)ray);
          hpos++;
        }
      }
      (void)ray;
    };
    if constexpr (march_is_proj(kMarch)) {
      if (mag_ok) {
        const FastPix c = make_fast(p, pos, cx, cy);
        const float inv_scale = kCert ? __uint_as_float((127u - (unsigned)p.cert_shift) << 23) : 1.0f;
        const FastTbn ft = make_fast_tbn(p, tbn, a, inv_scale);
        const CertPix cp = make_cert(p, c, inv_scale);
        const int rs = p.ray_interleave ? 2 * wave : r0, re = p.ray_interleave ? p.n_live : r1;
        const int rstep = p.ray_interleave ? 2 * kGiWaves : 2;
        auto pair = [&](int r, int rb) {
          const float4 ra0 = rays[2 * r], ra1 = rays[2 * rb];
          f32x2 Bxy[2], Bz2;
          float bz0, bz1;
          fast_ray(ft, ra0, Bxy[0], bz0);
          fast_ray(ft, ra1, Bxy[1], bz1);
          Bz2 = f32x2{bz0, bz1};
          int hit[2];
          if constexpr (kCert) march2_cert<kGiGroup, kCertOff>(p, c, cp, Bxy, Bz2, pos_z, hit);
          else march2_fast<kGiGroup>(p, c, Bxy, Bz2, pos_z, hit);
          if (rb == r) hit[1] = -1;
          if (__any(hit[0] >= 0 || hit[1] >= 0)) {
            add_hit(hit[0], ra0.w, rays[2 * r + 1].x, r);
            add_hit(hit[1], ra1.w, rays[2 * rb + 1].x, rb);
          }
        };
        for (int r = rs; r < re; r += rstep) pair(r, min(r + 1, re - 1));
        for (int r = p.n_live + wave; r < p.nrays; r += kGiWaves) pair(r, r);
      }
    } else {
    const unsigned sv_min_bits = gi_sv_min_bits(a, p.radius, p.inv_step);
    int r = r0;
    for (; r + kGiRays <= r1; r += kGiRays) {
      v3 sv[kGiRays];
      float ct[kGiRays], st[kGiRays];
      int hit[kGiRays];
#pragma unroll
      for (int k = 0; k < kGiRays; k++) {
        const float4 ra = rays[2 * (r + k)];
        ct[k] = ra.w;
        st[k] = rays[2 * (r + k) + 1].x;
        sv[k] = tbn_apply(tbn, ra.x, ra.y, ra.z);
      }
      march<kPow2, kGiGroup, kGiRays>(p, pos, a, sv, cx, cy, pos_z, mag_ok, sv_min_bits, hit);
      bool any_hit = false;
#pragma unroll
      for (int k = 0; k < kGiRays; k++) any_hit = any_hit || hit[k] >= 0;
      if (__any(any_hit)) {
#pragma unroll
        for (int k = 0; k < kGiRays; k++) add_hit(hit[k], ct[k], st[k], r + k);
      }
    }
    auto single = [&](int q) {
      const float4 ra = rays[2 * q];
      const v3 sv = tbn_apply(tbn, ra.x, ra.y, ra.z);
      int hit;
      march<kPow2, kGiGroup, 1>(p, pos, a, &sv, cx, cy, pos_z, mag_ok, sv_min_bits, &hit);
      add_hit(hit, ra.w, rays[2 * q + 1].x, q);
    };
    for (; r < r1; r++) single(r);
    for (r = p.n_live + wave; r < p.nrays; r += kGiWaves) single(r);
// ... 86 lines not shown
          d[l].x += c[3 * l] * cos_t * sin_t;
          d[l].y += c[3 * l + 1] * cos_t * sin_t;
          d[l].z += c[3 * l + 2] * cos_t * sin_t;
        }
      }
#pragma unroll
      for (int l = 0; l < kLights; l++) {
        if (w == 0) sum[l] = d[l];
        else sum[l] = {sum[l].x + d[l].x, sum[l].y + d[l].y, sum[l].z + d[l].z};
      }
    }
#pragma unroll
    for (int l = 0; l < kLights; l++)
      ssr_finish(sum[l], tbn, pos, pix_id, HW, nrays_total, albedo_map, metallic_map, F0_map, color + (size_t)l * 3 * HW,
                 abd + (size_t)l * 3 * HW);
    return;
  }
  v3 part[4];
#pragma unroll
  for (int w = 0; w < 4; w++) {
    v3 d = {0, 0, 0};
    const unsigned e0 = offsets[4 * pix_id + w], e1 = offsets[4 * pix_id + w + 1];
    for (unsigned e = e0; e < e1; e++) {
      const uint2 h = entries[e];
      const float cos_t = rays[2 * h.y].w, sin_t = rays[2 * h.y + 1].x;
      d.x += rgb[h.x] * cos_t * sin_t;
      d.y += rgb[HW + h.x] * cos_t * sin_t;
      d.z += rgb[2 * HW + h.x] * cos_t * sin_t;
    }
    part[w] = d;
  }
  const v3 diffuse = {((part[0].x + part[1].x) + part[2].x) + part[3].x, ((part[0].y + part[1].y) + part[2].y) + part[3].y,
                      ((part[0].z + part[1].z) + part[2].z) + part[3].z};
  ssr_finish(diffuse, tbn, pos, pix_id, HW, nrays_total, albedo_map, metallic_map, F0_map, color, abd);
}

static GiParams make_params(const Options& o, int W, int H, float fx, float fy, float radius, float bias, float thick,
                            int step, int start, const RayTable& t, bool ssr, bool& pow2) {
  GiParams p;
  p.W = W; p.H = H; p.fx = fx; p.fy = fy; p.radius = radius; p.bias = bias; p.thick = thick;
  p.step = step; p.start = start;
  p.n_live = t.n_live;
  p.nrays = t.n_live + (o.gi_zero_rays ? t.n_dead : (ssr && t.n_dead > 0 ? 1 : 0));
  p.nrays_total = t.nrays;
  pow2 = step > 0 && (step & (step - 1)) == 0 && step <= (1 << 20);
  p.inv_step = pow2 ? 1.0f / (float)step : 0.0f;
  if (step - start > 64 - kGiGroup) pow2 = false;
  for (int k = 0; k < 64; k++) p.fjt[k] = pow2 ? (float)(start + k) * p.inv_step : (float)(start + k) / (float)step;
  for (int k = 0; k < 64; k++) p.fjc[k] = p.fjt[k < step - 1 - start ? k : (step - 1 - start > 0 ? step - 1 - start : 0)];
  p.tile_log2w = (o.gi_tile_log2w >= 0 && o.gi_tile_log2w <= 6) ? o.gi_tile_log2w : kGiTileLog2W;
  p.ray_interleave = o.gi_interleave ? 1 : 0;
  return p;
}
__global__ void __launch_bounds__(64)
gi_minmax_kernel(int W, int H, int shift, int bw, int bh, CertK ck, const float* __restrict__ z, float2* __restrict__ tab) {
  const int bx = (int)blockIdx.x, by = (int)blockIdx.y, B = 1 << shift;
  float mn = __builtin_inff(), mx = 0.0f;
  const bool full = bx < bw && by < bh && ((bx + 1) << shift) <= W && ((by + 1) << shift) <= H;
  if (full) {
    for (int i = threadIdx.x; i < B * B; i += 64) {
      const float v = z[(size_t)((by << shift) + (i >> shift)) * W + (bx << shift) + (i & (B - 1))];
      if (v != 0.0f) mn = fminf(mn, v);
      mx = fmaxf(mx, v);
    }
#pragma unroll
    for (int o = 32; o > 0; o >>= 1) {
      mn = fminf(mn, __shfl_xor(mn, o));
      mx = fmaxf(mx, __shfl_xor(mx, o));
    }
  } else {
    mn = -__builtin_inff();
    mx = __builtin_inff();
  }
  if (threadIdx.x == 0) {
    float t_hi = (mx - ck.lo_k) / (1.0f - 0x1p-16f);
    t_hi = t_hi + fabsf(t_hi) * 0x1p-20f + 1e-30f;
    float t_lo = (mn - ck.hi_k) / (1.0f + 0x1p-16f);
    t_lo = t_lo - fabsf(t_lo) * 0x1p-20f - 1e-30f;
    if (!(mx == mx) || !(mn == mn)) { t_hi = __builtin_inff(); t_lo = -__builtin_inff(); }
    tab[(size_t)by * (bw + 1) + bx] = make_float2(t_lo, t_hi);
  }
}

constexpr int kCertMaxBytes = 40 * 1024;
static size_t cert_table_bytes(int W, int H, int sh) {
  return (size_t)(((W + (1 << sh) - 1) >> sh) + 2) * (((H + (1 << sh) - 1) >> sh) + 2) * sizeof(float2);
}
static int cert_shift_for(int W, int H) {
  for (int sh = 4; sh <= 6; sh++)
    if (cert_table_bytes(W, H, sh) <= (size_t)kCertMaxBytes) return sh;
  return 0;
}
size_t gi_scratch_bytes(int W, int H) {
  const int sh = cert_shift_for(W, H);
  return sh ? cert_table_bytes(W, H, sh) : 0;
}
static size_t prepare_cert(const Options& o, GiParams& p, int mode, const float* pos, void* scratch, hipStream_t s) {
  p.cert_shift = p.cert_w = p.cert_h = 0;
  p.cert_d0 = cert_consts(p.bias, p.thick).d0;
  if (!scratch || mode != 4 || !o.gi_cert) return 0;
  const int sh = cert_shift_for(p.W, p.H);
  if (!sh) return 0;
  p.cert_shift = sh;
  p.cert_w = (p.W + (1 << sh) - 1) >> sh;
  p.cert_h = (p.H + (1 << sh) - 1) >> sh;
  hipLaunchKernelGGL(gi_minmax_kernel, dim3(p.cert_w + 1, p.cert_h + 1), dim3(64), 0, s, p.W, p.H, sh, p.cert_w, p.cert_h,
                     cert_consts(p.bias, p.thick), pos + 2 * (size_t)p.H * p.W, (float2*)scratch);
  return cert_table_bytes(p.W, p.H, sh);
}

#ifndef GIGS_GI_DEFAULT_MODE
#define GIGS_GI_DEFAULT_MODE 4
#endif
static int gi_march_mode(const Options& o, int step, int start) {
  int mode = (o.gi_march == 0 || o.gi_march == 4) ? o.gi_march : GIGS_GI_DEFAULT_MODE;
  if (step - start > 64 - kGiGroup || step <= 0) mode = 0;
  return mode;
}
template <March kMarch> using MarchTag = std::integral_constant<March, kMarch>;
template <class F>
static void gi_dispatch_march(int mode, bool pow2, size_t cert, F&& f) {
  if (mode == 4) {
    if (cert) f(MarchTag<March::kProjCert>{}, cert);
    else f(MarchTag<March::kProj>{}, (size_t)0);
  } else {
    if (pow2) f(MarchTag<March::kExactPow2>{}, (size_t)0);
    else f(MarchTag<March::kExact>{}, (size_t)0);
  }
}
static dim3 gi_grid(const GiParams& p) {
  const int tw = 1 << p.tile_log2w, th = 64 >> p.tile_log2w;
  return dim3((p.W + tw - 1) / tw, (p.H + th - 1) / th);
}

int launch_ssao(const Options& o, int W, int H, float fx, float fy, float radius, float bias, float thick,
                float delta, int step, int start, const float* normal, const float* pos,
                float* occlusion, void* scratch, hipStream_t s) {
  RayTable t;
  const int rc = get_ray_table(delta, s, t);
  if (rc) return rc;
  bool pow2;
  GiParams p = make_params(o, W, H, fx, fy, radius, bias, thick, step, start, t,  false, pow2);
  if (W >= (1 << 15) || H >= (1 << 15)) return -2;
  const dim3 grid = gi_grid(p);
  const int mode = gi_march_mode(o, step, start);
  const size_t cert = (start < step) ? prepare_cert(o, p, mode, pos, scratch, s) : 0;
  const float2* tab = (const float2*)scratch;
  gi_dispatch_march(mode, pow2, cert, [&](auto m, size_t lds) {
    hipLaunchKernelGGL((ssao_kernel<decltype(m)::value>), grid, dim3(256), lds, s, p, t.dev, t.sum_w, normal, pos, occlusion, tab);
  });
  return 0;
}

int launch_ssr_apply(int W, int H, float delta, const unsigned* offsets, const void* entries, const float* normal,
                     const float* pos, const float* rgb, const float* albedo, const float* metallic, const float* F0,
                     float* color, float* abd, hipStream_t s) {
  RayTable t;
  const int rc = get_ray_table(delta, s, t);
  if (rc) return rc;
  const size_t HW = (size_t)W * H;
  hipLaunchKernelGGL(ssr_apply_kernel<1>, dim3((unsigned)((HW + 255) / 256)), dim3(256), 0, s, W, H, t.nrays, t.dev, offsets,
                     (const uint2*)entries, normal, pos, rgb, albedo, metallic, F0, color, abd);
  return 0;
}

#ifndef GIGS_SSR_APPLY_LIGHTS
#define GIGS_SSR_APPLY_LIGHTS 8
// ... 439 lines not shown
```

gi-gs_amd/csrc/gigs_common.h:

```cpp
#pragma once
#include <hip/hip_runtime.h>
#include <stdint.h>

#define GIGS_BLOCK_X 16
#define GIGS_BLOCK_Y 16
#define GIGS_TILE (GIGS_BLOCK_X * GIGS_BLOCK_Y)
#define GIGS_BREC_F4 5
#define GIGS_GREC 20

namespace gigs {

struct v3 { float x, y, z; };
struct v4 { float x, y, z, w; };

__device__ __forceinline__ v3 operator+(v3 a, v3 b) { return {a.x + b.x, a.y + b.y, a.z + b.z}; }
__device__ __forceinline__ v3 operator-(v3 a, v3 b) { return {a.x - b.x, a.y - b.y, a.z - b.z}; }
__device__ __forceinline__ v3 operator*(v3 a, float s) { return {a.x * s, a.y * s, a.z * s}; }
__device__ __forceinline__ float dot3(v3 a, v3 b) { return a.x * b.x + a.y * b.y + a.z * b.z; }
__device__ __forceinline__ v3 cross3(v3 a, v3 b) {
  return {a.y * b.z - a.z * b.y, a.z * b.x - a.x * b.z, a.x * b.y - a.y * b.x};
}
__device__ __forceinline__ v3 normalize3(v3 v) {
  float inv = 1.0f / sqrtf(dot3(v, v));
  return v * inv;
// ... 104 lines not shown
    carve(chunk, g.point_offsets, P);
    carve(chunk, g.internal_radii, P);
    carve(chunk, g.brec, GIGS_BREC_F4 * P);
    carve(chunk, g.grec, (size_t)GIGS_GREC * P);
    g.scan_size = scan_size;
    carve(chunk, g.scan_space, scan_size);
    return g;
  }
};

#ifndef GIGS_BIN_GROUPS
#define GIGS_BIN_GROUPS 512
#endif
constexpr int kBinGroups = GIGS_BIN_GROUPS;
constexpr int kBinMaxTiles = 16384;
constexpr int kBucketMaxMeanList = 2500;

struct ImageState {
  float* final_T;
  uint32_t* n_contrib;
  uint2* ranges;
  uint32_t* tile_order;
  uint32_t* bin_hist;
  uint32_t* bin_counters;
  static ImageState fromChunk(char*& chunk, size_t N, size_t T) {
    ImageState s;
    carve(chunk, s.final_T, N);
    carve(chunk, s.n_contrib, N);
    carve(chunk, s.ranges, T);
    carve(chunk, s.tile_order, T);
    carve(chunk, s.bin_hist, (size_t)(kBinGroups + 2) * T);
    carve(chunk, s.bin_counters, 4);
    return s;
  }
};

struct BinningState {
  uint64_t* keys_unsorted;
  uint32_t* values_unsorted;
  uint64_t* keys;
  uint32_t* point_list;
  uint8_t* hit_mask;
  char* sort_space;
  size_t sort_size;
  static BinningState fromChunk(char*& chunk, size_t R, size_t sort_size) {
    BinningState b;
    carve(chunk, b.keys_unsorted, R);
    carve(chunk, b.values_unsorted, R);
    carve(chunk, b.keys, R);
    carve(chunk, b.point_list, R);
    carve(chunk, b.hit_mask, 4 * R);
    b.sort_size = sort_size;
    carve(chunk, b.sort_space, sort_size);
    return b;
  }
};

template <typename S, typename... A>
inline size_t required_bytes(A... a) {
  char* p = nullptr;
  S::fromChunk(p, a...);
  return reinterpret_cast<size_t>(p) + kAlign;
}

struct Options {
  int binning_legacy;
  int bucket_max_mean;
  int long_lists;
  int bucket_target;
  int bin_bands;
  int blend_cull;
  int pre_bwd_sh_skip;
  int gi_march;
  int gi_cert;
  int gi_interleave;
  int gi_tile_log2w;
  int gi_zero_rays;
  int spec_max8, spec_max16;
  int shade_lds_floats;
  int shade_bwd_blocks;
  int shade_bwd_rows;
  int spec_sparse;
  int spec_sparse_permille;
};
struct Ctx {
  Options opt;
  unsigned async_capacity;
  unsigned* async_counters;
  void* blend_begin_event;
  int reuse_binning;
  unsigned* materials_only;
  const float* sh_rest;
};
const Options& default_options();
const Ctx& default_ctx();

struct FwdArgs {
  int P, D, M, W, H;
  unsigned gx, gy;
  float focal_x, focal_y, tan_fovx, tan_fovy, scale_modifier;
  const float *means3D, *shs, *colors_precomp, *opacities, *normal, *albedo, *roughness,
      *metallic, *scales, *rotations, *cov3D_precomp, *viewmatrix, *projmatrix, *cam_pos,
      *background;
  int argmax_depth, inference;
  const float* shs_rest;
};

void launch_preprocess_fwd(const FwdArgs& a, const GeomState& g, int* radii, hipStream_t s);
void launch_zero_words(uint32_t* p, size_t n, hipStream_t s);
void launch_bin_count(int P, const int* radii, unsigned gx, unsigned gy, const GeomState& g, const ImageState& img, hipStream_t s);
void launch_bin_prefix(int P, int T, unsigned capacity, const ImageState& img, unsigned* user_counters, hipStream_t s);
void launch_bin_scatter(int P, const int* radii, unsigned gx, unsigned gy, unsigned capacity, unsigned bands, const GeomState& g,
                        const BinningState& b, const ImageState& img, hipStream_t s);
int launch_bin_sort(int T, int P, bool long_lists, unsigned bucket_target, unsigned capacity, const BinningState& b, const ImageState& img,
                    hipStream_t s);
size_t long_space_bytes(size_t T, size_t R);
void launch_mark_visible(int P, const float* means3D, const float* viewmatrix, uint8_t* present,
                         hipStream_t s);
hipError_t scan_tiles(const GeomState& g, int P, hipStream_t s);
size_t scan_temp_bytes(int P);
size_t sort_temp_bytes(int R);
void launch_duplicate(int P, const int* radii, unsigned gx, unsigned gy, const GeomState& g,
                      const BinningState& b, hipStream_t s);
hipError_t sort_pairs(const BinningState& b, int R, int end_bit, hipStream_t s);
void launch_tile_ranges(int R, const BinningState& b, uint2* ranges, hipStream_t s);
void launch_tile_order(int T, const uint2* ranges, uint32_t* tile_order, hipStream_t s);
void launch_blend_fwd(const FwdArgs& a, const GeomState& g, const BinningState& b,
                      const ImageState& im, float* out_color, float* out_opacity,
                      float* out_depth, float* out_normal, float* out_normal_view, float* out_pos,
                      float* out_albedo, float* out_roughness, float* out_metallic, int cull, size_t hit_stride,
                      hipStream_t s, bool reused_lists = false);

struct BwdArgs {
  int P, D, M, R, W, H;
  unsigned gx, gy;
  float focal_x, focal_y, tan_fovx, tan_fovy, scale_modifier;
  const float *means3D, *shs, *colors_precomp, *scales, *rotations, *cov3D_precomp, *viewmatrix,
      *projmatrix, *cam_pos, *background;
  const int* radii;
  const float *dL_dpix_depth, *dL_dpix, *dL_dpix_opacity, *dL_dpix_normal, *dL_dpix_albedo,
      *dL_dpix_roughness, *dL_dpix_metallic;
  float *dL_dmean2D, *dL_dconic, *dL_ddepth, *dL_dopacity, *dL_dnormal, *dL_dalbedo,
      *dL_droughness, *dL_dmetallic, *dL_dcolor, *dL_dmean3D, *dL_dcov3D, *dL_dsh, *dL_dscale,
      *dL_drot;
};
void launch_blend_bwd(const BwdArgs& a, const GeomState& g, const BinningState& b,
                      const ImageState& im, hipStream_t s);
void launch_preprocess_bwd(const BwdArgs& a, const GeomState& g, int sh_skip, hipStream_t s, unsigned* materials_only = nullptr);

void launch_depth_to_normal(int W, int H, float fx, float fy, const float* viewmatrix,
                            const float* depth, float* normal, float* depth_pos, hipStream_t s);
int launch_ssao(const Options& o, int W, int H, float fx, float fy, float radius, float bias, float thick,
                float delta, int step, int start, const float* normal, const float* pos,
                float* occlusion, void* scratch, hipStream_t s);
size_t gi_scratch_bytes(int W, int H);
int launch_ssr(const Options& o, int W, int H, float fx, float fy, float radius, float bias, float thick,
               float delta, int step, int start, const float* normal, const float* pos,
               const float* rgb, const float* albedo, const float* roughness,
               const float* metallic, const float* F0, float* color, float* abd, void* scratch, hipStream_t s,
               int hits_mode = 0, unsigned* hit_counts = nullptr, const unsigned* hit_offsets = nullptr,
               void* hit_entries = nullptr, unsigned hit_capacity = 0);
int launch_ssr_multi(const Options& o, int n_lights, int W, int H, float fx, float fy, float radius, float bias, float thick,
                     float delta, int step, int start, const float* normal, const float* pos, const float* rgb,
                     const float* albedo, const float* metallic, const float* F0, float* color, float* abd, void* scratch,
                     hipStream_t s);
int launch_ssr_apply(int W, int H, float delta, const unsigned* offsets, const void* entries, const float* normal,
                     const float* pos, const float* rgb, const float* albedo, const float* metallic, const float* F0,
                     float* color, float* abd, hipStream_t s);
int launch_ssr_apply_multi(int n_lights, int W, int H, float delta, const unsigned* offsets, const void* entries,
                           const float* normal, const float* pos, const float* rgb, const float* albedo, const float* metallic,
                           const float* F0, float* color, float* abd, void* scratch, hipStream_t s);
size_t ssr_apply_multi_scratch_bytes(int n_lights, int W, int H);
void launch_median3x3(int C, int H, int W, const float* in, float* out, hipStream_t s);
void launch_median3x3_bwd(int C, int H, int W, const float* in, const float* gout, float* gin,
                          hipStream_t s);
void launch_bilateral3x3(int C, int H, int W, float sigma_color, float sx, float sy,
                         const float* in, float* out, hipStream_t s);
void launch_derive_normal_fused(int W, int H, float fx, float fy, const float* viewmatrix, float sigma_color, float sx,
                                float sy, const float* depth_raw, float* normal_out, float* pos_filter_out, hipStream_t s);

}
```

gi-gs_amd/gigs_lib.py:

```python
from __future__ import annotations

import ctypes as C
import functools
import os
import threading

_HERE = os.path.dirname(os.path.abspath(__file__))
LIB_PATH = os.environ.get("GIGS_LIB", os.path.join(_HERE, "libgigs_hip.so"))

ALLOC_FN = C.CFUNCTYPE(C.c_void_p, C.c_size_t, C.c_void_p)

_f = C.c_void_p
_i = C.c_int
_fl = C.c_float

SIGNATURES = {
    "gigs_last_error": (C.c_char_p, []),
    "gigs_build_arch": (C.c_char_p, []),
    "gigs_required_geom": (C.c_size_t, [_i]),
    "gigs_required_image": (C.c_size_t, [_i, _i]),
    "gigs_required_binning": (C.c_size_t, [_i]),
    "gigs_forward": (_i, [C.c_void_p, ALLOC_FN, C.c_void_p, ALLOC_FN, C.c_void_p, ALLOC_FN, C.c_void_p,
                          _i, _i, _i, _f, _i, _i,
                          _f, _f, _f, _f, _f, _f, _f, _f,
# ... 66 lines not shown
                                  C.POINTER(C.c_void_p), C.POINTER(C.c_int), _f, _i, _i, _i, _i, _f, _f, C.c_void_p]),
    "gigs_shade_bwd_ex": (_i, [C.c_void_p, _i, _i, _f, _f, _f, _f, _f, _f, _f, _f, _i, _i, C.POINTER(C.c_void_p),
                               C.POINTER(C.c_int), _f, _i, _i, _i, _i, _f, _f, _f, _f, _f, _f, _f, _f,
                               C.POINTER(C.c_void_p), C.c_void_p, C.c_void_p]),
    "gigs_gbuffer_post": (_i, [_i, _i, _f, _f, _f, _f, _f, _f, _f, C.c_void_p]),
    "gigs_gbuffer_post_pad": (_i, [_i, _i, _f, _f, _f, _f, _f, _f, _f, _f, _f, _f, _f, _f, C.c_void_p]),
    "gigs_gbuffer_post_bwd": (_i, [_i, _i, _f, _f, _f, _f, _f, C.c_void_p]),
    "gigs_normalize_mask": (_i, [_i, _i, _f, _f, _f, C.c_void_p]),
    "gigs_nonzero_mask": (_i, [_i, _i, _f, _f, C.c_void_p]),
    "gigs_stage2_loss_fwd": (_i, [_i, _i, _f, _f, _f, _f, _f, _f, _f, _f, _f, C.c_void_p]),
    "gigs_stage2_loss_bwd": (_i, [_i, _i, _f, _f, _f, _f, _f, _f, _f, _f, _f, _f, C.c_void_p]),
    "gigs_stage2_loss_fwd_grad": (_i, [_i, _i, _f, _f, _f, _f, _f, _f, _f, _f, _f, _f, _f, C.c_void_p]),
    "gigs_cube_texture_fwd": (_i, [_i, _f, _i, _f, _f, _i, C.c_void_p]),
    "gigs_cube_texture_fwd_precise": (_i, [_i, _f, _i, _f, _f, C.c_void_p]),
    "gigs_cube_texture_bwd": (_i, [_i, _i, _f, _f, _f, _i, C.c_void_p]),
    "gigs_cube_taps": (_i, [_i, _i, _f, _f, _f, C.c_void_p]),
    "gigs_cube_texture_bwd_gather": (_i, [_i, _i, _i, _f, _f, _f, _i, _i, _f, _f, _f, C.c_void_p]),
    "gigs_latlong_to_cubemap": (_i, [_i, _i, _i, _i, _i, _f, _f, C.c_void_p]),
    "gigs_latlong_to_cubemap_rot": (_i, [_i, _i, _i, _i, _i, _f, _i, _f, _f, C.c_void_p]),
    "gigs_loss_scratch_floats": (C.c_size_t, [_i, _i, _i]),
    "gigs_l1_ssim_fwd": (_i, [_i, _i, _i, _f, _f, C.c_float, _f, _f, _f, _f, _f, C.c_void_p]),
    "gigs_l1_ssim_bwd": (_i, [_i, _i, _i, _f, _f, C.c_float, _f, _f, _f, _f, _f, C.c_void_p]),
    "gigs_image_metrics_scratch_bytes": (C.c_size_t, [_i, _i, _i]),
    "gigs_image_metrics": (_i, [_i, _i, _i, _f, _f, _f, _f, _f, _f, C.c_void_p]),
    "gigs_normal_angular_error": (_i, [_i, _i, _f, _f, _i, _f, _f, _f, C.c_void_p]),
    "gigs_lpips_vgg_weight_floats": (C.c_size_t, []),
    "gigs_lpips_vgg_pack": (_i, [C.POINTER(C.c_void_p), C.POINTER(C.c_void_p), C.POINTER(C.c_void_p), _f, C.c_void_p]),
    "gigs_lpips_vgg_scratch_bytes": (C.c_size_t, [_i, _i, _i]),
    "gigs_lpips_vgg": (_i, [_i, _i, _i, _f, _f, _i, _f, _f, _f, _f, C.POINTER(C.c_void_p), C.c_void_p]),
    "gigs_pack_images": (_i, [_i, _f, C.c_void_p]),
    "gigs_plane_minmax": (_i, [C.c_longlong, _f, _f, _f, C.c_void_p]),
    "gigs_png_filter": (_i, [_i, _f, C.c_void_p]),
    "gigs_tsdf_integrate": (_i, [C.c_void_p, _i, C.c_void_p, C.c_void_p]),
    "gigs_mesh_count": (_i, [C.c_void_p, _fl, _f, _f, C.c_void_p]),
    "gigs_mesh_write": (_i, [C.c_void_p, _fl, _f, _f, _i, _i, _f, _f, _f, _f, _f, _f, _f, C.c_void_p]),
    "gigs_tv_loss_fwd": (_i, [_i, _i, _i, _i, _f, _f, _f, _f, _f, C.c_void_p]),
    "gigs_tv_loss_bwd": (_i, [_i, _i, _i, _i, _f, _f, _f, _f, _f, C.c_void_p]),
    "gigs_masked_l1_fwd": (_i, [_i, _i, _i, _f, _f, _f, _f, _f, C.c_void_p]),
    "gigs_masked_l1_bwd": (_i, [_i, _i, _i, _f, _f, _f, _f, _f, _f, _f, C.c_void_p]),
    "gigs_adam_step": (_i, [_i, C.c_void_p, C.c_double, C.c_double, C.c_double, _i, C.c_void_p]),
    "gigs_adam_step_dyn": (_i, [_i, C.c_void_p, C.c_double, C.c_double, C.c_double, _i, _f, C.c_void_p]),
    "gigs_adam_scalars": (None, [C.c_double, _i, C.c_double, C.c_double, C.POINTER(C.c_float)]),
    "gigs_adam_step_watch": (_i, [_i, C.c_void_p, C.c_double, C.c_double, C.c_double, _i, _f, C.c_char_p, _f, C.c_void_p]),
    "gigs_adam_step_guarded": (_i, [_i, C.c_void_p, C.c_double, C.c_double, C.c_double, _i, _f, C.c_char_p, _f, _f, C.c_void_p]),
    "gigs_ctx_set_reuse_binning": (_i, [C.c_void_p, _i]),
    "gigs_ctx_set_materials_only": (_i, [C.c_void_p, C.c_void_p]),
    "gigs_ctx_set_split_sh": (_i, [C.c_void_p, C.c_void_p]),
    "gigs_activate_fwd": (_i, [_i, _i, C.c_void_p, C.c_void_p, C.c_void_p]),
    "gigs_activate_bwd": (_i, [_i, _i, C.c_void_p, C.c_void_p, C.c_void_p, C.c_void_p]),
    "gigs_densify_stats": (_i, [_i, _f, _f, _f, _f, _f, _f, _f, C.c_void_p]),
    "gigs_densify_stats_guarded": (_i, [_i, _f, _f, _f, _f, _f, _f, _f, _f, C.c_void_p]),
    "gigs_gather_rows": (_i, [_i, C.c_void_p, C.c_longlong, C.c_longlong, _f, _f, C.c_void_p]),
    "gigs_dist2_scratch_bytes": (C.c_size_t, [_i]),
    "gigs_dist2": (_i, [_i, _f, _f, _f, C.c_size_t, C.c_void_p]),
    "gigs_geom_offset": (C.c_longlong, [_i, _i]),
    "gigs_binning_offset": (C.c_longlong, [_i, _i]),
    "gigs_image_offset": (C.c_longlong, [_i, _i, _i]),
    "gigs_selftest_div2": (_i, [_i, _f, _f, _f, _f, _f, _f, C.c_void_p]),
    "gigs_selftest_round": (_i, [_f, C.c_void_p]),
    "gigs_ctx_set_blend_begin_event": (_i, [C.c_void_p, C.c_void_p]),
    "gigs_stream_delay": (_i, [C.c_uint, C.c_void_p]),
    "gigs_ctx_set_async_binning": (_i, [C.c_void_p, _i, C.c_void_p]),
    "gigs_ctx_create": (C.c_void_p, []),
    "gigs_ctx_destroy": (None, [C.c_void_p]),
    "gigs_ctx_get_options": (_i, [C.c_void_p, C.c_void_p]),
    "gigs_ctx_set_options": (_i, [C.c_void_p, C.c_void_p]),
    "gigs_profile_begin": (None, []),
    "gigs_profile_end": (_i, [C.POINTER(C.c_float), C.POINTER(C.c_int), _i]),
    "gigs_profile_stage_name": (C.c_char_p, [_i]),
}

class ShadeExt(C.Structure):
    _fields_ = [("planar", C.c_int), ("rough_scale", C.c_float), ("rough_bias", C.c_float),
                ("out_F0", C.c_void_p), ("out_linear", C.c_void_p), ("out_roughness", C.c_void_p),
                ("g_albedo_mul_a", C.c_void_p), ("g_albedo_mul_b", C.c_void_p),
                ("g_roughness_add", C.c_void_p), ("g_metallic_add", C.c_void_p),
                ("g_scale", C.c_void_p), ("lamb_mask", C.c_void_p), ("lamb_acc4", C.c_void_p)]


class Options(C.Structure):
    _fields_ = [(n, C.c_int) for n in (
        "struct_bytes", "binning_legacy", "bucket_max_mean", "long_lists", "bucket_target", "bin_bands", "blend_cull",
        "pre_bwd_sh_skip", "gi_march", "gi_cert", "gi_interleave", "gi_tile_log2w", "gi_zero_rays", "spec_max8",
        "spec_max16", "shade_lds_floats", "shade_bwd_blocks", "shade_bwd_rows", "spec_sparse", "spec_sparse_permille")]


OPTION_NAMES = tuple(n for n, _ in Options._fields_ if n != "struct_bytes")
GI_MARCHES = {0: "exact", 4: "proj"}
_GI_MARCH_VALUES = {name: value for value, name in GI_MARCHES.items()}


class SpecLevel(C.Structure):
    _fields_ = [("res", C.c_int), ("avg_window", C.c_int), ("src", C.c_void_p), ("bounds", C.c_void_p),
                ("offsets", C.c_void_p), ("weights", C.c_void_p), ("dst", C.c_void_p), ("wsum", C.c_void_p)]


class AdamGroup(C.Structure):
    _fields_ = [("param", C.c_void_p), ("grad", C.c_void_p), ("exp_avg", C.c_void_p), ("exp_avg_sq", C.c_void_p),
                ("n", C.c_longlong), ("lr", C.c_double), ("step", C.c_int)]


class ActivationRaw(C.Structure):
    _fields_ = [(n, C.c_void_p) for n in ("f_dc", "f_rest", "opacity", "normal", "albedo", "roughness", "metallic",
                                          "scaling", "rotation")]


class ActivationOut(C.Structure):
    _fields_ = [(n, C.c_void_p) for n in ("shs", "opacities", "normal", "albedo", "roughness", "metallic", "scales",
                                          "rotations")]


class GatherTensor(C.Structure):
    _fields_ = [("src", C.c_void_p), ("dst", C.c_void_p), ("row_floats", C.c_int), ("zero_new", C.c_int)]


class PackDesc(C.Structure):
    _fields_ = [("src", C.c_void_p), ("dst", C.c_void_p), ("lohi", C.c_void_p), ("channels", C.c_int), ("height", C.c_int),
                ("width", C.c_int), ("dst_x", C.c_int), ("dst_stride", C.c_int), ("bias", C.c_float)]


class FilterDesc(C.Structure):
    _fields_ = [("sheet", C.c_void_p), ("out", C.c_void_p), ("height", C.c_int), ("width", C.c_int), ("stride", C.c_int),
                ("reserved", C.c_int)]


class TsdfGrid(C.Structure):
    _fields_ = [("lo", C.c_float * 3), ("voxel", C.c_float), ("dims", C.c_int * 3), ("trunc", C.c_float),
                ("opacity_min", C.c_float), ("carve", C.c_int), ("tsdf", C.c_void_p), ("weight", C.c_void_p),
                ("attr_weight", C.c_void_p), ("attr", C.c_void_p)]


class TsdfView(C.Structure):
    _fields_ = [("viewmatrix", C.c_float * 16), ("tanfovx", C.c_float), ("tanfovy", C.c_float), ("width", C.c_int),
                ("height", C.c_int), ("opacity", C.c_void_p), ("depth", C.c_void_p), ("normal", C.c_void_p),
                ("albedo", C.c_void_p), ("roughness", C.c_void_p), ("metallic", C.c_void_p)]


TSDF_MAX_VIEWS = 8
TSDF_MAX_AXIS = 1024
SPEC_SPARSE_STATE_INTS = 32
MAX_IMAGES = 4096
MINMAX_SCRATCH_FLOATS = 512

_lib = None


class GigsError(RuntimeError):
    pass


def lib():
    global _lib
    if _lib is None:
        if not os.path.exists(LIB_PATH):
            raise ImportError(
                f"{LIB_PATH} not found: build it with `python gi-gs_amd/build.py` "
                "(hipcc, --offload-arch=gfx950). There is no CPU fallback.")
        l = C.CDLL(LIB_PATH)
        for name, (res, args) in SIGNATURES.items():
            fn = getattr(l, name)
            fn.restype = res
            fn.argtypes = args
        _lib = l
    return _lib


def check(rc: int, what: str) -> int:
# ... 175 lines not shown
```

include/gigs_hip.h:

```cpp
#ifndef GIGS_HIP_H_
#define GIGS_HIP_H_

#include <stddef.h>
#include <stdint.h>

#ifdef __cplusplus
extern "C" {
#endif

#define GIGS_OK 0
#define GIGS_ERR_INVALID (-1)
#define GIGS_ERR_HIP (-2)
#define GIGS_ERR_ALLOC (-3)

typedef char* (*gigs_alloc_fn)(size_t nbytes, void* user);

const char* gigs_last_error(void);
const char* gigs_build_arch(void);

typedef struct gigs_ctx gigs_ctx;
typedef struct gigs_options {
  int struct_bytes;
  int binning_legacy;
  int bucket_max_mean;
  int long_lists;
  int bucket_target;
  int bin_bands;
  int blend_cull;
  int pre_bwd_sh_skip;
  int gi_march;
  int gi_cert;
  int gi_interleave;
  int gi_tile_log2w;
  int gi_zero_rays;
  int spec_max8;
  int spec_max16;
  int shade_lds_floats;
  int shade_bwd_blocks;
  int shade_bwd_rows;
  int spec_sparse;
  int spec_sparse_permille;
} gigs_options;
gigs_ctx* gigs_ctx_create(void);
void gigs_ctx_destroy(gigs_ctx* ctx);
int gigs_ctx_get_options(const gigs_ctx* ctx, gigs_options* out);
int gigs_ctx_set_options(gigs_ctx* ctx, const gigs_options* in);

size_t gigs_required_geom(int P);
size_t gigs_required_image(int width, int height);
size_t gigs_required_binning(int num_rendered);

int gigs_forward(gigs_ctx* ctx, gigs_alloc_fn geometryBuffer, void* geom_user, gigs_alloc_fn binningBuffer,
                 void* binning_user, gigs_alloc_fn imageBuffer, void* image_user, int P, int D, int M,
                 const float* background, int width, int height, const float* means3D,
                 const float* shs, const float* colors_precomp, const float* opacities,
                 const float* normal, const float* albedo, const float* roughness,
                 const float* metallic, const float* scales, float scale_modifier,
                 const float* rotations, const float* cov3D_precomp, const float* viewmatrix,
                 const float* projmatrix, const float* cam_pos, float tan_fovx, float tan_fovy,
                 int prefiltered, int argmax_depth, int inference, float* out_color,
                 float* out_opacity, float* out_depth, float* out_normal, float* out_normal_view,
                 float* out_pos, float* out_albedo, float* out_roughness, float* out_metallic,
                 int* radii, int debug, void* stream);

int gigs_backward(gigs_ctx* ctx, int P, int D, int M, int R, const float* background, int width, int height,
                  const float* means3D, const float* shs, const float* colors_precomp,
                  const float* normal, const float* albedo, const float* roughness,
                  const float* metallic, const float* scales, const float* rotations,
                  const float* cov3D_precomp, const float* viewmatrix, const float* projmatrix,
                  const float* cam_pos, const int* radii, float scale_modifier, float tan_fovx,
                  float tan_fovy, char* geom_buffer, char* binning_buffer, char* image_buffer,
                  const float* dL_dpix_depth, const float* dL_dpix, const float* dL_dpix_opacity,
                  const float* dL_dpix_normal, const float* dL_dpix_albedo,
                  const float* dL_dpix_roughness, const float* dL_dpix_metallic, float* dL_dmean2D,
                  float* dL_dconic, float* dL_ddepth, float* dL_dopacity, float* dL_dnormal,
                  float* dL_dalbedo, float* dL_droughness, float* dL_dmetallic, float* dL_dcolor,
                  float* dL_dmean3D, float* dL_dcov3D, float* dL_dsh, float* dL_dscale,
                  float* dL_drot, int debug, void* stream);

int gigs_mark_visible(int P, const float* means3D, const float* viewmatrix,
                      const float* projmatrix, uint8_t* present, void* stream);

int gigs_depth_to_normal(int width, int height, float focal_x, float focal_y,
                         const float* viewmatrix, const float* depth, float* normal,
                         float* depth_pos, void* stream);

int gigs_derive_normal(int width, int height, float focal_x, float focal_y, const float* viewmatrix, const float* depth,
                       float sigma_color, float sigma_x, float sigma_y, float* normal_from_depth, float* depth_pos_filter,
                       void* stream);
int gigs_ssao(int width, int height, float focal_x, float focal_y, float radius, float bias,
              float thick, float delta, int step, int start, const float* normal_view,
              const float* pos, float* occlusion, void* stream);

int gigs_ssr(int width, int height, float focal_x, float focal_y, float radius, float bias,
             float thick, float delta, int step, int start, const float* normal_view,
             const float* pos, const float* rgb, const float* albedo, const float* roughness,
             const float* metallic, const float* F0, float* color, float* abd, void* stream);

size_t gigs_gi_scratch_bytes(int width, int height);
int gigs_ssao_ex(gigs_ctx* ctx, int width, int height, float focal_x, float focal_y, float radius, float bias,
                 float thick, float delta, int step, int start, const float* normal_view,
                 const float* pos, float* occlusion, void* scratch, void* stream);
int gigs_ssr_ex(gigs_ctx* ctx, int width, int height, float focal_x, float focal_y, float radius, float bias,
                float thick, float delta, int step, int start, const float* normal_view,
                const float* pos, const float* rgb, const float* albedo, const float* roughness,
                const float* metallic, const float* F0, float* color, float* abd, void* scratch, void* stream);

int gigs_ssr_hits(gigs_ctx* ctx, int width, int height, float focal_x, float focal_y, float radius, float bias, float thick,
                  float delta, int step, int start, const float* normal_view, const float* pos, const float* rgb,
                  const float* albedo, const float* roughness, const float* metallic, const float* F0, float* color, float* abd,
                  int mode, unsigned* counts, const unsigned* offsets, void* entries, unsigned capacity, void* scratch,
                  void* stream);
int gigs_ssr_apply(int width, int height, float delta, const unsigned* offsets, const void* entries, const float* normal_view,
                   const float* pos, const float* rgb, const float* albedo, const float* metallic, const float* F0,
                   float* color, float* abd, void* stream);

#define GIGS_MAX_LIGHTS 16
#define GIGS_SSR_LIGHTS_PER_MARCH 4
int gigs_ssr_multi(gigs_ctx* ctx, int n_lights, int width, int height, float focal_x, float focal_y, float radius, float bias,
                   float thick, float delta, int step, int start, const float* normal_view, const float* pos, const float* rgb,
                   const float* albedo, const float* roughness, const float* metallic, const float* F0, float* color,
                   float* abd, void* scratch, void* stream);

size_t gigs_ssr_apply_multi_scratch_bytes(int n_lights, int width, int height);
// ... 286 lines not shown
```

Before: 352.9 renders/s.

## Fuse small-tile sort into blend forward and tile ordering into bin scatter

```diff
diff --git a/gi-gs_amd/build.py b/gi-gs_amd/build.py
--- a/gi-gs_amd/build.py
+++ b/gi-gs_amd/build.py
@@ -22,6 +22,7 @@
     yield os.path.join(CSRC, src)
     yield os.path.join(CSRC, "gigs_common.h")
     yield os.path.join(CSRC, "pixel_ops.h")
+    yield os.path.join(CSRC, "tile_sort.h")
     yield os.path.join(HERE, "..", "include", "gigs_hip.h")
 
 
diff --git a/gi-gs_amd/csrc/api.hip b/gi-gs_amd/csrc/api.hip
--- a/gi-gs_amd/csrc/api.hip
+++ b/gi-gs_amd/csrc/api.hip
@@ -116,6 +116,7 @@
   o.spec_sparse = env_int("GIGS_SPEC_SPARSE", 1) != 0;
   o.spec_sparse_permille = env_int("GIGS_SPEC_SPARSE_PERMILLE", 37);
   if (o.spec_sparse_permille < 0 || o.spec_sparse_permille > 1000) o.spec_sparse_permille = 37;
+  o.blend_sort = env_int("GIGS_BLEND_SORT", 1) != 0;
   return o;
 }
 const gigs::Ctx& ctx_of(const gigs_ctx* c) { return c ? *reinterpret_cast<const gigs::Ctx*>(c) : gigs::default_ctx(); }
@@ -244,6 +245,7 @@
   out->gi_tile_log2w = o.gi_tile_log2w; out->gi_zero_rays = o.gi_zero_rays; out->spec_max8 = o.spec_max8;
   out->spec_max16 = o.spec_max16; out->shade_lds_floats = o.shade_lds_floats; out->shade_bwd_blocks = o.shade_bwd_blocks;
   out->shade_bwd_rows = o.shade_bwd_rows; out->spec_sparse = o.spec_sparse; out->spec_sparse_permille = o.spec_sparse_permille;
+  out->blend_sort = o.blend_sort;
   return 0;
 }
 int gigs_ctx_set_options(gigs_ctx* ctx, const gigs_options* in) {
@@ -264,6 +266,7 @@
   o.gi_tile_log2w = in->gi_tile_log2w; o.gi_zero_rays = in->gi_zero_rays != 0; o.spec_max8 = in->spec_max8;
   o.spec_max16 = in->spec_max16; o.shade_lds_floats = in->shade_lds_floats; o.shade_bwd_blocks = in->shade_bwd_blocks;
   o.shade_bwd_rows = in->shade_bwd_rows != 0; o.spec_sparse = in->spec_sparse != 0; o.spec_sparse_permille = in->spec_sparse_permille;
+  o.blend_sort = in->blend_sort != 0;
   return 0;
 }
 int gigs_ctx_set_reuse_binning(gigs_ctx* ctx, int on) {
@@ -339,7 +342,7 @@
   return (stage >= 0 && stage < kNumStages) ? kStageNames[stage] : "";
 }
 
-int gigs_forward(gigs_ctx* ctx, gigs_alloc_fn geometryBuffer, void* geom_user, gigs_alloc_fn binningBuffer,
+static int forward_impl(bool allow_blend_sort, gigs_ctx* ctx, gigs_alloc_fn geometryBuffer, void* geom_user, gigs_alloc_fn binningBuffer,
                  void* binning_user, gigs_alloc_fn imageBuffer, void* image_user, int P, int D, int M,
                  const float* background, int width, int height, const float* means3D,
                  const float* shs, const float* colors_precomp, const float* opacities,
@@ -407,6 +410,7 @@
     return est_mean > (size_t)opt.bucket_max_mean;
   };
   bool dense = false;
+  unsigned blend_sort_bits = 0;
   if (cx.reuse_binning) {
     if (async_cap == 0 || !bucket)
       return fail(GIGS_ERR_INVALID, "reuse_binning needs asynchronous binning (gigs_ctx_set_async_binning) on the tile-bucketed path");
@@ -439,15 +443,13 @@
     char* bin_chunk = binningBuffer(bin_bytes, binning_user);
     if (!bin_chunk) return fail(GIGS_ERR_ALLOC, "binning buffer allocation of %zu bytes failed", bin_bytes);
     bin = gigs::BinningState::fromChunk(bin_chunk, (size_t)num_rendered, sort_sz);
-    {
-      StageScope sc(kRanges, s);
-      gigs::launch_tile_order((int)T, img.ranges, img.tile_order, s);
-    }
+    if (allow_blend_sort && opt.blend_sort && !inference) blend_sort_bits = gigs::bin_index_bits(P);
     {
       StageScope sc(kSort, s);
       const unsigned bands = opt.bin_bands > 0 ? (unsigned)opt.bin_bands : (dense ? 4u : 1u);
       gigs::launch_bin_scatter(P, radii, a.gx, a.gy, (unsigned)num_rendered, bands, geom, bin, img, s);
-      if (gigs::launch_bin_sort((int)T, P, dense && num_rendered > 0, (unsigned)opt.bucket_target, (unsigned)num_rendered, bin, img, s) != 0)
+      if (gigs::launch_bin_sort((int)T, P, dense && num_rendered > 0, (unsigned)opt.bucket_target, (unsigned)num_rendered, bin, img, s,
+                                blend_sort_bits == 0) != 0)
         return fail(GIGS_ERR_HIP, "bin_sort: cannot fork the sort streams");
     }
     STAGE_CHECK("bin scatter / sort");
@@ -493,10 +495,25 @@
     StageScope sc(kBlendFwd, s);
     gigs::launch_blend_fwd(a, geom, bin, img, out_color, out_opacity, out_depth, out_normal,
                            out_normal_view, out_pos, out_albedo, out_roughness, out_metallic, opt.blend_cull,
-                           (size_t)num_rendered, s, cx.reuse_binning != 0);
+                           (size_t)num_rendered, s, cx.reuse_binning != 0, blend_sort_bits);
   }
   STAGE_CHECK("render");
   return num_rendered;
+}
+
+int gigs_forward(gigs_ctx* ctx, gigs_alloc_fn geometryBuffer, void* geom_user, gigs_alloc_fn binningBuffer, void* binning_user,
+                 gigs_alloc_fn imageBuffer, void* image_user, int P, int D, int M, const float* background, int width, int height,
+                 const float* means3D, const float* shs, const float* colors_precomp, const float* opacities, const float* normal,
+                 const float* albedo, const float* roughness, const float* metallic, const float* scales, float scale_modifier,
+                 const float* rotations, const float* cov3D_precomp, const float* viewmatrix, const float* projmatrix,
+                 const float* cam_pos, float tan_fovx, float tan_fovy, int prefiltered, int argmax_depth, int inference,
+                 float* out_color, float* out_opacity, float* out_depth, float* out_normal, float* out_normal_view, float* out_pos,
+                 float* out_albedo, float* out_roughness, float* out_metallic, int* radii, int debug, void* stream) {
+  return forward_impl(true, ctx, geometryBuffer, geom_user, binningBuffer, binning_user, imageBuffer, image_user, P, D, M, background,
+                      width, height, means3D, shs, colors_precomp, opacities, normal, albedo, roughness, metallic, scales,
+                      scale_modifier, rotations, cov3D_precomp, viewmatrix, projmatrix, cam_pos, tan_fovx, tan_fovy, prefiltered,
+                      argmax_depth, inference, out_color, out_opacity, out_depth, out_normal, out_normal_view, out_pos, out_albedo,
+                      out_roughness, out_metallic, radii, debug, stream);
 }
 
 namespace {
@@ -529,7 +546,7 @@
   float* spare = reinterpret_cast<float*>(up(ib + img_bytes));
   gigs::launch_zero_words(reinterpret_cast<uint32_t*>(zeros), 8 * (size_t)P, (hipStream_t)stream);
   LiteChunk gc{gb, geom_bytes}, ic{ib, img_bytes};
-  return gigs_forward(ctx, lite_chunk_alloc, &gc, binningBuffer, binning_user, lite_chunk_alloc, &ic, P, D, M, background, width, height,
+  return forward_impl(false, ctx, lite_chunk_alloc, &gc, binningBuffer, binning_user, lite_chunk_alloc, &ic, P, D, M, background, width, height,
                       means3D, shs, colors_precomp, opacities, zeros, zeros + 3 * (size_t)P, zeros + 6 * (size_t)P,
                       zeros + 7 * (size_t)P, scales, scale_modifier, rotations, cov3D_precomp, viewmatrix, projmatrix, cam_pos,
                       tan_fovx, tan_fovy, prefiltered, argmax_depth, 0, out_color, out_opacity, out_depth, spare, spare + 3 * N,
diff --git a/gi-gs_amd/csrc/binning.hip b/gi-gs_amd/csrc/binning.hip
--- a/gi-gs_amd/csrc/binning.hip
+++ b/gi-gs_amd/csrc/binning.hip
@@ -3,11 +3,11 @@
 #include <cstring>
 #include <mutex>
 #include <string.h>
-#include <rocprim/block/block_radix_sort.hpp>
 #include <rocprim/device/device_radix_sort.hpp>
 #include <rocprim/device/device_scan.hpp>
 
 #include "gigs_common.h"
+#include "tile_sort.h"
 
 namespace gigs {
 
@@ -89,9 +89,9 @@
 }
 
 constexpr int kMaxOrderedTiles = 16384;
-__global__ void __launch_bounds__(256)
-tile_order_kernel(int T, const uint2* __restrict__ ranges, uint32_t* __restrict__ order, int identity) {
-  const int t = blockIdx.x * 4 + (threadIdx.x >> 6), lane = threadIdx.x & 63;
+__device__ __forceinline__ void tile_order_wave(int t, int T, const uint2* __restrict__ ranges, uint32_t* __restrict__ order,
+                                                int identity) {
+  const int lane = threadIdx.x & 63;
   if (t >= T) return;
   if (identity) {
     if (lane == 0) order[t] = (uint32_t)t;
@@ -106,6 +106,10 @@
     rank += (uint32_t)__popcll(__ballot(before));
   }
   if (lane == 0) order[rank] = (uint32_t)t;
+}
+__global__ void __launch_bounds__(256)
+tile_order_kernel(int T, const uint2* __restrict__ ranges, uint32_t* __restrict__ order, int identity) {
+  tile_order_wave(blockIdx.x * 4 + (threadIdx.x >> 6), T, ranges, order, identity);
 }
 
 void launch_tile_order(int T, const uint2* ranges, uint32_t* tile_order, hipStream_t s) {
@@ -253,8 +257,14 @@
 bin_scatter_kernel(int P, int T, const int* __restrict__ radii, const float* __restrict__ means2D,
                    const float* __restrict__ depths, unsigned gx, unsigned gy, unsigned capacity, unsigned idx_bits,
                    const uint32_t* __restrict__ bin_hist, const uint32_t* __restrict__ tile_start,
-                   uint64_t* __restrict__ keys, unsigned bands) {
+                   uint64_t* __restrict__ keys, unsigned bands, const uint2* __restrict__ ranges,
+                   uint32_t* __restrict__ tile_order, int order_identity) {
   extern __shared__ uint32_t s_cur[];
+  const int groups = min((int)kBinGroups, (P + 255) / 256);
+  if ((int)blockIdx.x >= groups) {
+    tile_order_wave(((int)blockIdx.x - groups) * (kLanes / 64) + (int)(threadIdx.x >> 6), T, ranges, tile_order, order_identity);
+    return;
+  }
   const uint32_t* row = bin_hist + (size_t)blockIdx.x * T;
   for (int t = threadIdx.x; t < T; t += kLanes) s_cur[t] = tile_start[t] + row[t];
   __syncthreads();
@@ -294,93 +304,11 @@
   }
 }
 
-template <int kItems, typename Storage, int kBlock = 1024>
-__device__ __forceinline__ void sort_tile_radix(Storage& storage, const uint64_t* __restrict__ src, unsigned n, unsigned idx_bits,
-                                                uint64_t tile_hi, uint32_t base, uint64_t* __restrict__ keys_out,
-                                                uint32_t* __restrict__ point_list) {
-  using sorter = rocprim::block_radix_sort<uint64_t, kBlock, kItems, rocprim::empty_type, 1, 1, 8>;
-  static_assert(sizeof(Storage) >= sizeof(uint64_t) * kBlock * kItems, "the sorted keys are staged in the sorter's storage");
-  const uint64_t idx_mask = (1ull << idx_bits) - 1;
-  uint64_t k[kItems];
-#pragma unroll
-  for (int i = 0; i < kItems; i++) {
-    const unsigned idx = threadIdx.x * kItems + i;
-    k[i] = idx < n ? src[idx] : ~0ull;
-  }
-  __shared__ unsigned long long s_diff;
-  if (threadIdx.x == 0) s_diff = 0ull;
-  __syncthreads();
-  {
-    const uint64_t ref = src[0];
-    uint64_t diff = 0;
-#pragma unroll
-    for (int i = 0; i < kItems; i++)
-      if (threadIdx.x * kItems + i < n) diff |= k[i] ^ ref;
-    diff >>= idx_bits;
-    if (diff) atomicOr(&s_diff, (unsigned long long)diff);
-  }
-  __syncthreads();
-  const unsigned dd = (unsigned)s_diff;
-  const unsigned hi = dd ? 32u - (unsigned)__builtin_clz(dd) : 1u;
-  sorter().sort(k, storage, idx_bits, idx_bits + hi);
-  __syncthreads();
-  uint64_t* s_k = reinterpret_cast<uint64_t*>(&storage);
-#pragma unroll
-  for (int i = 0; i < kItems; i++) s_k[threadIdx.x * kItems + i] = k[i];
-  __syncthreads();
-  bool tie = false;
-#pragma unroll
-  for (int i = 0; i < kItems; i++) {
-    const unsigned idx = threadIdx.x * kItems + i;
-    if (idx > 0 && idx < n) {
-      const uint64_t prev = i > 0 ? k[i - 1] : s_k[idx - 1];
-      tie |= (prev >> idx_bits) == (k[i] >> idx_bits) && prev > k[i];
-    }
-  }
-  if (__syncthreads_or(tie)) {
-    constexpr unsigned kPairs = (unsigned)kBlock * kItems / 2;
-    constexpr int kFixRounds = 64;
-    bool more = true;
-    for (int round = 0; round < kFixRounds && more; round++) {
-      bool swapped = false;
-#pragma unroll
-      for (int phase = 0; phase < 2; phase++) {
-        for (unsigned p = threadIdx.x; p < kPairs; p += kBlock) {
-          const unsigned a = 2 * p + phase, c = a + 1;
-          if (c < n) {
-            const uint64_t x = s_k[a], y = s_k[c];
-            if ((x >> idx_bits) == (y >> idx_bits) && x > y) { s_k[a] = y; s_k[c] = x; swapped = true; }
-          }
-        }
-        __syncthreads();
-      }
-      more = __syncthreads_or(swapped);
-    }
-    if (more) {
-#pragma unroll
-      for (int i = 0; i < kItems; i++) k[i] = s_k[threadIdx.x * kItems + i];
-      __syncthreads();
-      sorter().sort(k, storage, 0, idx_bits + hi);
-      __syncthreads();
-#pragma unroll
-      for (int i = 0; i < kItems; i++) s_k[threadIdx.x * kItems + i] = k[i];
-      __syncthreads();
-    }
-  }
-  for (unsigned idx = threadIdx.x; idx < n; idx += kBlock) {
-    const uint64_t kk = s_k[idx];
-    point_list[base + idx] = (uint32_t)(kk & idx_mask);
-    keys_out[base + idx] = tile_hi | (kk >> idx_bits);
-  }
-  __syncthreads();
-}
 
 using SortS4 = rocprim::block_radix_sort<uint64_t, 1024, 4, rocprim::empty_type, 1, 1, 8>::storage_type;
 using SortS8 = rocprim::block_radix_sort<uint64_t, 1024, 8, rocprim::empty_type, 1, 1, 8>::storage_type;
 using SortS16 = rocprim::block_radix_sort<uint64_t, 1024, 16, rocprim::empty_type, 1, 1, 8>::storage_type;
 
-constexpr unsigned kSmallList = 2048;
-using SortSmall = rocprim::block_radix_sort<uint64_t, 256, 8, rocprim::empty_type, 1, 1, 8>::storage_type;
 __global__ void __launch_bounds__(256)
 bin_sort_small_kernel(int T, unsigned idx_bits, const uint32_t* __restrict__ tile_order, const uint2* __restrict__ ranges,
                       const uint64_t* __restrict__ keys_unsorted, uint64_t* __restrict__ keys_out,
@@ -653,7 +581,7 @@
   hipLaunchKernelGGL(zero_words_kernel, dim3(blocks), dim3(256), 0, s, p, n);
 }
 
-static unsigned bin_index_bits(int P) {
+unsigned bin_index_bits(int P) {
   unsigned ib = 1;
   while (ib < 32 && (1ull << ib) < (unsigned long long)P) ib++;
   return ib;
@@ -685,12 +613,15 @@
   const int T = (int)(gx * gy);
   const uint32_t* tile_start = img.bin_hist + (size_t)(kBinGroups + 1) * T;
   bands = std::max(1u, std::min(bands, gy));
+  const int order_identity = T > kMaxOrderedTiles ? 1 : 0;
   if (P >= kWideWalk)
-    hipLaunchKernelGGL(bin_scatter_kernel<1024>, dim3(bin_groups(P)), dim3(1024), (size_t)T * sizeof(uint32_t), s, P, T, radii,
-                       g.means2D, g.depths, gx, gy, capacity, bin_index_bits(P), img.bin_hist, tile_start, b.keys_unsorted, bands);
+    hipLaunchKernelGGL(bin_scatter_kernel<1024>, dim3(bin_groups(P) + (T + 15) / 16), dim3(1024), (size_t)T * sizeof(uint32_t), s, P,
+                       T, radii, g.means2D, g.depths, gx, gy, capacity, bin_index_bits(P), img.bin_hist, tile_start,
+                       b.keys_unsorted, bands, img.ranges, img.tile_order, order_identity);
   else
-    hipLaunchKernelGGL(bin_scatter_kernel<256>, dim3(bin_groups(P)), dim3(256), (size_t)T * sizeof(uint32_t), s, P, T, radii,
-                       g.means2D, g.depths, gx, gy, capacity, bin_index_bits(P), img.bin_hist, tile_start, b.keys_unsorted, bands);
+    hipLaunchKernelGGL(bin_scatter_kernel<256>, dim3(bin_groups(P) + (T + 3) / 4), dim3(256), (size_t)T * sizeof(uint32_t), s, P, T,
+                       radii, g.means2D, g.depths, gx, gy, capacity, bin_index_bits(P), img.bin_hist, tile_start, b.keys_unsorted,
+                       bands, img.ranges, img.tile_order, order_identity);
 }
 
 void launch_long_lists(int T, int P, unsigned target, unsigned capacity, const BinningState& b, const ImageState& img, hipStream_t s) {
@@ -709,7 +640,7 @@
 }
 
 int launch_bin_sort(int T, int P, bool long_lists, unsigned bucket_target, unsigned capacity, const BinningState& b, const ImageState& img,
-                    hipStream_t s) {
+                    hipStream_t s, bool sort_small) {
   const unsigned ib = bin_index_bits(P);
   if (long_lists)
     launch_long_lists(T, P, bucket_target, capacity, b, img, s);
@@ -718,8 +649,9 @@
                        b.keys_unsorted, b.keys, b.point_list);
   hipLaunchKernelGGL(bin_sort_kernel<false>, dim3(std::min(T, 512)), dim3(1024), 0, s, T, ib, img.tile_order, img.ranges,
                      b.keys_unsorted, b.keys, b.point_list);
-  hipLaunchKernelGGL(bin_sort_small_kernel, dim3(std::min(T, 2048)), dim3(256), 0, s, T, ib, img.tile_order, img.ranges,
-                     b.keys_unsorted, b.keys, b.point_list);
+  if (sort_small)
+    hipLaunchKernelGGL(bin_sort_small_kernel, dim3(std::min(T, 2048)), dim3(256), 0, s, T, ib, img.tile_order, img.ranges,
+                       b.keys_unsorted, b.keys, b.point_list);
   return 0;
 }
 
diff --git a/gi-gs_amd/csrc/blend.hip b/gi-gs_amd/csrc/blend.hip
--- a/gi-gs_amd/csrc/blend.hip
+++ b/gi-gs_amd/csrc/blend.hip
@@ -1,5 +1,6 @@
 #include <cstdlib>
 #include "gigs_common.h"
+#include "tile_sort.h"
 
 namespace gigs {
 
@@ -191,11 +192,12 @@
 
 __global__ void __launch_bounds__(GIGS_TILE)
 blend_fwd_kernel(int W, int H, unsigned gx, const uint2* __restrict__ ranges,
-                 const uint32_t* __restrict__ point_list, const float4* __restrict__ brec,
+                 uint32_t* point_list, const float4* __restrict__ brec,
                  const float* __restrict__ viewmatrix, const float* __restrict__ bg_color,
                  uint32_t* __restrict__ n_contrib, float* __restrict__ final_T, BlendOut o,
                  int argmax_depth, int inference, uint8_t* __restrict__ hit_mask, size_t hit_stride, int cull,
-                 const uint32_t* __restrict__ tile_order, const uint32_t* __restrict__ reuse_guard, uint2 reuse_expect) {
+                 const uint32_t* __restrict__ tile_order, const uint32_t* __restrict__ reuse_guard, uint2 reuse_expect,
+                 unsigned sort_idx_bits, const uint64_t* __restrict__ keys_unsorted, uint64_t* __restrict__ keys_sorted) {
   __shared__ float4 s_rec[4][GIGS_BREC_F4 * 64];
 
   const unsigned tile = tile_order[blockIdx.x];
@@ -215,6 +217,14 @@
     range = make_uint2(0u, 0u);
   const int n = (int)(range.y - range.x);
   if (n > kLongTile) __builtin_amdgcn_s_setprio(3);
+  if (sort_idx_bits != 0u && n > 0 && n <= (int)kSmallList) {
+    static_assert(sizeof(SortSmall) <= sizeof(s_rec), "the sorter's storage aliases the staging slab");
+    sort_tile_radix<8, SortSmall, 256>(*reinterpret_cast<SortSmall*>(&s_rec[0][0]), keys_unsorted + range.x, (unsigned)n,
+                                       sort_idx_bits, (uint64_t)tile << 32, range.x, keys_sorted, point_list);
+    __builtin_amdgcn_fence(__ATOMIC_RELEASE, "workgroup");
+    __syncthreads();
+    __builtin_amdgcn_fence(__ATOMIC_ACQUIRE, "workgroup");
+  }
   float4* sw = s_rec[wave];
   uint8_t* hit = hit_mask + (size_t)wave * hit_stride + range.x;
 
@@ -339,14 +349,15 @@
                       const ImageState& im, float* out_color, float* out_opacity,
                       float* out_depth, float* out_normal, float* out_normal_view, float* out_pos,
                       float* out_albedo, float* out_roughness, float* out_metallic, int cull, size_t hit_stride,
-                      hipStream_t s, bool reused_lists) {
+                      hipStream_t s, bool reused_lists, unsigned sort_idx_bits) {
   BlendOut o{out_color, out_opacity, out_depth, out_normal, out_normal_view,
              out_pos, out_albedo, out_roughness, out_metallic};
   hipLaunchKernelGGL(blend_fwd_kernel, dim3(a.gx * a.gy), dim3(GIGS_TILE), 0, s, a.W, a.H, a.gx,
                      im.ranges, b.point_list, g.brec, a.viewmatrix, a.background, im.n_contrib,
                      im.final_T, o, a.argmax_depth, a.inference, b.hit_mask, hit_stride, cull, im.tile_order,
                      reused_lists ? (const uint32_t*)im.bin_counters : (const uint32_t*)nullptr,
-                     make_uint2((unsigned)a.P, (unsigned)hit_stride));
+                     make_uint2((unsigned)a.P, (unsigned)hit_stride), sort_idx_bits,
+                     (const uint64_t*)b.keys_unsorted, b.keys);
 }
 
 struct BlendGradIn {
diff --git a/gi-gs_amd/csrc/gi.hip b/gi-gs_amd/csrc/gi.hip
--- a/gi-gs_amd/csrc/gi.hip
+++ b/gi-gs_amd/csrc/gi.hip
@@ -686,6 +686,31 @@
 #define GIGS_SSR_OCC_L(L) __attribute__((amdgpu_waves_per_eu((L) == 1 ? 5 : GIGS_SSR_MULTI_WAVES)))
 #endif
 
+constexpr int kCertMaxBytes = 40 * 1024;
+__device__ __forceinline__ bool cert_table_to_lds(bool live, int wave, float* flag, int flag_stride, int nb,
+                                                  const float2* __restrict__ cert_tab, float2* s_cert) {
+  const bool wave_live = __builtin_amdgcn_ballot_w64(live) != 0ull;
+  if ((threadIdx.x & 63) == 0) flag[wave * flag_stride] = wave_live ? 1.0f : 0.0f;
+  __syncthreads();
+  bool any = false;
+#pragma unroll
+  for (int w = 0; w < 4; w++) any = any || flag[w * flag_stride] != 0.0f;
+  if (!any) {
+    __syncthreads();
+    return false;
+  }
+  constexpr int kIters = kCertMaxBytes / (int)sizeof(float2) / 256;
+  float2 t[kIters];
+#pragma unroll
+  for (int k = 0; k < kIters; k++)
+    if (k * 256 < nb) t[k] = cert_tab[min(k * 256 + (int)threadIdx.x, nb - 1)];
+#pragma unroll
+  for (int k = 0; k < kIters; k++)
+    if (k * 256 + (int)threadIdx.x < nb) s_cert[k * 256 + threadIdx.x] = t[k];
+  __syncthreads();
+  return true;
+}
+
 enum class March { kExactPow2, kExact, kProj, kProjCert };
 constexpr bool march_is_proj(March m) { return m == March::kProj || m == March::kProjCert; }
 
@@ -698,78 +723,83 @@
   extern __shared__ float2 s_cert[];
   constexpr bool kPow2 = kMarch == March::kExactPow2, kCert = kMarch == March::kProjCert;
   constexpr int kCertOff = sizeof(float) * kGiWaves * 64;
-  if constexpr (kCert) {
-    if ((unsigned)(size_t)s_cert != (unsigned)kCertOff) __builtin_trap();
-    const int nb = (p.cert_w + 1) * (p.cert_h + 1);
-    for (int i = threadIdx.x; i < nb; i += 256) s_cert[i] = cert_tab[i];
-    __syncthreads();
-  }
   int x, y, wave;
   const bool inside = gi_pixel(p, x, y, wave);
   const int lane = threadIdx.x & 63;
   const size_t HW = (size_t)p.H * p.W;
   const size_t pix_id = inside ? (size_t)p.W * y + x : 0;
   float occ = 0.0f;
+  Tbn tbn;
+  v3 pos = {0.0f, 0.0f, 0.0f};
+  bool live = false;
   if (inside && p.start < p.step) {
-    const Tbn tbn = make_tbn({nrm[pix_id], nrm[HW + pix_id], nrm[2 * HW + pix_id]});
+    tbn = make_tbn({nrm[pix_id], nrm[HW + pix_id], nrm[2 * HW + pix_id]});
     if (!tbn_never_hits(tbn)) {
-      const v3 pos = {pos_map[pix_id], pos_map[HW + pix_id], pos_map[2 * HW + pix_id]};
-      const __amdgpu_buffer_rsrc_t pos_z = z_plane_rsrc(pos_map + 2 * HW, HW);
-      const float a = 1 + pos.z / 100;
-      const float cx = float(p.W) / 2.0f, cy = float(p.H) / 2.0f;
-      const int chunk = (p.n_live + kGiWaves - 1) / kGiWaves;
-      const int r0 = wave * chunk, r1 = min(p.n_live, r0 + chunk);
-      const bool mag_ok = gi_mag_ok(pos, a, p.radius);
-      if constexpr (march_is_proj(kMarch)) {
-        if (mag_ok) {
-          const FastPix c = make_fast(p, pos, cx, cy);
-          const float inv_scale = kCert ? __uint_as_float((127u - (unsigned)p.cert_shift) << 23) : 1.0f;
-          const FastTbn ft = make_fast_tbn(p, tbn, a, inv_scale);
-          const CertPix cp = make_cert(p, c, inv_scale);
-          const int rs = p.ray_interleave ? 2 * wave : r0, re = p.ray_interleave ? p.n_live : r1;
-          const int rstep = p.ray_interleave ? 2 * kGiWaves : 2;
-          auto pair = [&](int r, int rb) {
-            f32x2 Bxy[2], Bz2;
-            float bz0, bz1;
-            fast_ray(ft, rays[2 * r], Bxy[0], bz0);
-            fast_ray(ft, rays[2 * rb], Bxy[1], bz1);
-            Bz2 = f32x2{bz0, bz1};
-            int hit[2];
-            if constexpr (kCert) march2_cert<kGiGroup, kCertOff>(p, c, cp, Bxy, Bz2, pos_z, hit);
-            else march2_fast<kGiGroup>(p, c, Bxy, Bz2, pos_z, hit);
-            occ += hit[0] >= 0 ? rays[2 * r + 1].y : 0.0f;
-            occ += (hit[1] >= 0 && rb != r) ? rays[2 * rb + 1].y : 0.0f;
-          };
-          for (int r = rs; r < re; r += rstep) pair(r, min(r + 1, re - 1));
-          for (int r = p.n_live + wave; r < p.nrays; r += kGiWaves) pair(r, r);
-        }
-      } else {
-      const unsigned sv_min_bits = gi_sv_min_bits(a, p.radius, p.inv_step);
-      int r = r0;
-      for (; r + kGiRays <= r1; r += kGiRays) {
-        v3 sv[kGiRays];
-        float w[kGiRays];
-        int hit[kGiRays];
-#pragma unroll
-        for (int k = 0; k < kGiRays; k++) {
-          const float4 ra = rays[2 * (r + k)];
-          w[k] = rays[2 * (r + k) + 1].y;
-          sv[k] = tbn_apply(tbn, ra.x, ra.y, ra.z);
-        }
-        march<kPow2, kGiGroup, kGiRays>(p, pos, a, sv, cx, cy, pos_z, mag_ok, sv_min_bits, hit);
-#pragma unroll
-        for (int k = 0; k < kGiRays; k++) occ += hit[k] >= 0 ? w[k] : 0.0f;
-      }
-      auto single = [&](int q) {
-        const float4 ra = rays[2 * q];
-        const v3 sv = tbn_apply(tbn, ra.x, ra.y, ra.z);
-        int hit;
-        march<kPow2, kGiGroup, 1>(p, pos, a, &sv, cx, cy, pos_z, mag_ok, sv_min_bits, &hit);
-        occ += hit >= 0 ? rays[2 * q + 1].y : 0.0f;
-      };
-      for (; r < r1; r++) single(r);
-      for (r = p.n_live + wave; r < p.nrays; r += kGiWaves) single(r);
-      }
+      pos = {pos_map[pix_id], pos_map[HW + pix_id], pos_map[2 * HW + pix_id]};
+      live = true;
+    }
+  }
+  if constexpr (kCert) {
+    if ((unsigned)(size_t)s_cert != (unsigned)kCertOff) __builtin_trap();
+    live = live && gi_mag_ok(pos, 1 + pos.z / 100, p.radius);
+    if (!cert_table_to_lds(live, wave, &s_part[0][0], 64, (p.cert_w + 1) * (p.cert_h + 1), cert_tab, s_cert)) live = false;
+  }
+  if (live) {
+    const __amdgpu_buffer_rsrc_t pos_z = z_plane_rsrc(pos_map + 2 * HW, HW);
+    const float a = 1 + pos.z / 100;
+    const float cx = float(p.W) / 2.0f, cy = float(p.H) / 2.0f;
+    const int chunk = (p.n_live + kGiWaves - 1) / kGiWaves;
+    const int r0 = wave * chunk, r1 = min(p.n_live, r0 + chunk);
+    const bool mag_ok = gi_mag_ok(pos, a, p.radius);
+    if constexpr (march_is_proj(kMarch)) {
+      if (mag_ok) {
+        const FastPix c = make_fast(p, pos, cx, cy);
+        const float inv_scale = kCert ? __uint_as_float((127u - (unsigned)p.cert_shift) << 23) : 1.0f;
+        const FastTbn ft = make_fast_tbn(p, tbn, a, inv_scale);
+        const CertPix cp = make_cert(p, c, inv_scale);
+        const int rs = p.ray_interleave ? 2 * wave : r0, re = p.ray_interleave ? p.n_live : r1;
+        const int rstep = p.ray_interleave ? 2 * kGiWaves : 2;
+        auto pair = [&](int r, int rb) {
+          f32x2 Bxy[2], Bz2;
+          float bz0, bz1;
+          fast_ray(ft, rays[2 * r], Bxy[0], bz0);
+          fast_ray(ft, rays[2 * rb], Bxy[1], bz1);
+          Bz2 = f32x2{bz0, bz1};
+          int hit[2];
+          if constexpr (kCert) march2_cert<kGiGroup, kCertOff>(p, c, cp, Bxy, Bz2, pos_z, hit);
+          else march2_fast<kGiGroup>(p, c, Bxy, Bz2, pos_z, hit);
+          occ += hit[0] >= 0 ? rays[2 * r + 1].y : 0.0f;
+          occ += (hit[1] >= 0 && rb != r) ? rays[2 * rb + 1].y : 0.0f;
+        };
+        for (int r = rs; r < re; r += rstep) pair(r, min(r + 1, re - 1));
+        for (int r = p.n_live + wave; r < p.nrays; r += kGiWaves) pair(r, r);
+      }
+    } else {
+    const unsigned sv_min_bits = gi_sv_min_bits(a, p.radius, p.inv_step);
+    int r = r0;
+    for (; r + kGiRays <= r1; r += kGiRays) {
+      v3 sv[kGiRays];
+      float w[kGiRays];
+      int hit[kGiRays];
+#pragma unroll
+      for (int k = 0; k < kGiRays; k++) {
+        const float4 ra = rays[2 * (r + k)];
+        w[k] = rays[2 * (r + k) + 1].y;
+        sv[k] = tbn_apply(tbn, ra.x, ra.y, ra.z);
+      }
+      march<kPow2, kGiGroup, kGiRays>(p, pos, a, sv, cx, cy, pos_z, mag_ok, sv_min_bits, hit);
+#pragma unroll
+      for (int k = 0; k < kGiRays; k++) occ += hit[k] >= 0 ? w[k] : 0.0f;
+    }
+    auto single = [&](int q) {
+      const float4 ra = rays[2 * q];
+      const v3 sv = tbn_apply(tbn, ra.x, ra.y, ra.z);
+      int hit;
+      march<kPow2, kGiGroup, 1>(p, pos, a, &sv, cx, cy, pos_z, mag_ok, sv_min_bits, &hit);
+      occ += hit >= 0 ? rays[2 * q + 1].y : 0.0f;
+    };
+    for (; r < r1; r++) single(r);
+    for (r = p.n_live + wave; r < p.nrays; r += kGiWaves) single(r);
     }
   }
   s_part[wave][lane] = occ;
@@ -836,12 +866,6 @@
   static_assert(kHits == 0 || march_is_proj(kMarch), "hit lists exist for the projective march only");
   constexpr bool kPow2 = kMarch == March::kExactPow2, kCert = kMarch == March::kProjCert;
   constexpr int kCertOff = sizeof(float) * kGiWaves * 3 * 64;
-  if constexpr (kCert) {
-    if ((unsigned)(size_t)s_cert != (unsigned)kCertOff) __builtin_trap();
-    const int nb = (p.cert_w + 1) * (p.cert_h + 1);
-    for (int i = threadIdx.x; i < nb; i += 256) s_cert[i] = cert_tab[i];
-    __syncthreads();
-  }
   int x, y, wave;
   const bool inside = gi_pixel(p, x, y, wave);
   const int lane = threadIdx.x & 63;
@@ -853,7 +877,13 @@
 #pragma unroll
   for (int l = 0; l < kLights; l++) diffuse[l] = {0, 0, 0};
   unsigned hpos = 0;
-  if (inside && p.start < p.step && !tbn_never_hits(tbn)) {
+  bool live = inside && p.start < p.step && !tbn_never_hits(tbn);
+  if constexpr (kCert) {
+    if ((unsigned)(size_t)s_cert != (unsigned)kCertOff) __builtin_trap();
+    const bool marches = live && gi_mag_ok(pos, 1 + pos.z / 100, p.radius);
+    if (!cert_table_to_lds(marches, wave, &s_part[0][0][0], 3 * 64, (p.cert_w + 1) * (p.cert_h + 1), cert_tab, s_cert)) live = false;
+  }
+  if (live) {
     const __amdgpu_buffer_rsrc_t pos_z = z_plane_rsrc(pos_map + 2 * HW, HW);
     const float a = 1 + pos.z / 100;
     const float cx = float(p.W) / 2.0f, cy = float(p.H) / 2.0f;
@@ -1106,7 +1136,6 @@
   }
 }
 
-constexpr int kCertMaxBytes = 40 * 1024;
 static size_t cert_table_bytes(int W, int H, int sh) {
   return (size_t)(((W + (1 << sh) - 1) >> sh) + 2) * (((H + (1 << sh) - 1) >> sh) + 2) * sizeof(float2);
 }
diff --git a/gi-gs_amd/csrc/gigs_common.h b/gi-gs_amd/csrc/gigs_common.h
--- a/gi-gs_amd/csrc/gigs_common.h
+++ b/gi-gs_amd/csrc/gigs_common.h
@@ -210,6 +210,7 @@
   int shade_bwd_rows;
   int spec_sparse;
   int spec_sparse_permille;
+  int blend_sort;
 };
 struct Ctx {
   Options opt;
@@ -241,7 +242,8 @@
 void launch_bin_scatter(int P, const int* radii, unsigned gx, unsigned gy, unsigned capacity, unsigned bands, const GeomState& g,
                         const BinningState& b, const ImageState& img, hipStream_t s);
 int launch_bin_sort(int T, int P, bool long_lists, unsigned bucket_target, unsigned capacity, const BinningState& b, const ImageState& img,
-                    hipStream_t s);
+                    hipStream_t s, bool sort_small = true);
+unsigned bin_index_bits(int P);
 size_t long_space_bytes(size_t T, size_t R);
 void launch_mark_visible(int P, const float* means3D, const float* viewmatrix, uint8_t* present,
                          hipStream_t s);
@@ -257,7 +259,8 @@
                       const ImageState& im, float* out_color, float* out_opacity,
                       float* out_depth, float* out_normal, float* out_normal_view, float* out_pos,
                       float* out_albedo, float* out_roughness, float* out_metallic, int cull, size_t hit_stride,
-                      hipStream_t s, bool reused_lists = false);
+                      hipStream_t s, bool reused_lists = false,
+                      unsigned sort_idx_bits = 0);
 
 struct BwdArgs {
   int P, D, M, R, W, H;
diff --git a/gi-gs_amd/csrc/tile_sort.h b/gi-gs_amd/csrc/tile_sort.h
--- /dev/null
+++ b/gi-gs_amd/csrc/tile_sort.h
@@ -0,0 +1,92 @@
+#pragma once
+#include <rocprim/block/block_radix_sort.hpp>
+
+#include "gigs_common.h"
+
+namespace gigs {
+
+template <int kItems, typename Storage, int kBlock = 1024>
+__device__ __forceinline__ void sort_tile_radix(Storage& storage, const uint64_t* __restrict__ src, unsigned n, unsigned idx_bits,
+                                                uint64_t tile_hi, uint32_t base, uint64_t* __restrict__ keys_out,
+                                                uint32_t* __restrict__ point_list) {
+  using sorter = rocprim::block_radix_sort<uint64_t, kBlock, kItems, rocprim::empty_type, 1, 1, 8>;
+  static_assert(sizeof(Storage) >= sizeof(uint64_t) * kBlock * kItems, "the sorted keys are staged in the sorter's storage");
+  const uint64_t idx_mask = (1ull << idx_bits) - 1;
+  uint64_t k[kItems];
+#pragma unroll
+  for (int i = 0; i < kItems; i++) {
+    const unsigned idx = threadIdx.x * kItems + i;
+    k[i] = idx < n ? src[idx] : ~0ull;
+  }
+  __shared__ unsigned long long s_diff;
+  if (threadIdx.x == 0) s_diff = 0ull;
+  __syncthreads();
+  {
+    const uint64_t ref = src[0];
+    uint64_t diff = 0;
+#pragma unroll
+    for (int i = 0; i < kItems; i++)
+      if (threadIdx.x * kItems + i < n) diff |= k[i] ^ ref;
+    diff >>= idx_bits;
+    if (diff) atomicOr(&s_diff, (unsigned long long)diff);
+  }
+  __syncthreads();
+  const unsigned dd = (unsigned)s_diff;
+  const unsigned hi = dd ? 32u - (unsigned)__builtin_clz(dd) : 1u;
+  sorter().sort(k, storage, idx_bits, idx_bits + hi);
+  __syncthreads();
+  uint64_t* s_k = reinterpret_cast<uint64_t*>(&storage);
+#pragma unroll
+  for (int i = 0; i < kItems; i++) s_k[threadIdx.x * kItems + i] = k[i];
+  __syncthreads();
+  bool tie = false;
+#pragma unroll
+  for (int i = 0; i < kItems; i++) {
+    const unsigned idx = threadIdx.x * kItems + i;
+    if (idx > 0 && idx < n) {
+      const uint64_t prev = i > 0 ? k[i - 1] : s_k[idx - 1];
+      tie |= (prev >> idx_bits) == (k[i] >> idx_bits) && prev > k[i];
+    }
+  }
+  if (__syncthreads_or(tie)) {
+    constexpr unsigned kPairs = (unsigned)kBlock * kItems / 2;
+    constexpr int kFixRounds = 64;
+    bool more = true;
+    for (int round = 0; round < kFixRounds && more; round++) {
+      bool swapped = false;
+#pragma unroll
+      for (int phase = 0; phase < 2; phase++) {
+        for (unsigned p = threadIdx.x; p < kPairs; p += kBlock) {
+          const unsigned a = 2 * p + phase, c = a + 1;
+          if (c < n) {
+            const uint64_t x = s_k[a], y = s_k[c];
+            if ((x >> idx_bits) == (y >> idx_bits) && x > y) { s_k[a] = y; s_k[c] = x; swapped = true; }
+          }
+        }
+        __syncthreads();
+      }
+      more = __syncthreads_or(swapped);
+    }
+    if (more) {
+#pragma unroll
+      for (int i = 0; i < kItems; i++) k[i] = s_k[threadIdx.x * kItems + i];
+      __syncthreads();
+      sorter().sort(k, storage, 0, idx_bits + hi);
+      __syncthreads();
+#pragma unroll
+      for (int i = 0; i < kItems; i++) s_k[threadIdx.x * kItems + i] = k[i];
+      __syncthreads();
+    }
+  }
+  for (unsigned idx = threadIdx.x; idx < n; idx += kBlock) {
+    const uint64_t kk = s_k[idx];
+    point_list[base + idx] = (uint32_t)(kk & idx_mask);
+    keys_out[base + idx] = tile_hi | (kk >> idx_bits);
+  }
+  __syncthreads();
+}
+
+constexpr unsigned kSmallList = 2048;
+using SortSmall = rocprim::block_radix_sort<uint64_t, 256, 8, rocprim::empty_type, 1, 1, 8>::storage_type;
+
+}
diff --git a/gi-gs_amd/gigs_lib.py b/gi-gs_amd/gigs_lib.py
--- a/gi-gs_amd/gigs_lib.py
+++ b/gi-gs_amd/gigs_lib.py
@@ -172,7 +172,8 @@
     _fields_ = [(n, C.c_int) for n in (
         "struct_bytes", "binning_legacy", "bucket_max_mean", "long_lists", "bucket_target", "bin_bands", "blend_cull",
         "pre_bwd_sh_skip", "gi_march", "gi_cert", "gi_interleave", "gi_tile_log2w", "gi_zero_rays", "spec_max8",
-        "spec_max16", "shade_lds_floats", "shade_bwd_blocks", "shade_bwd_rows", "spec_sparse", "spec_sparse_permille")]
+        "spec_max16", "shade_lds_floats", "shade_bwd_blocks", "shade_bwd_rows", "spec_sparse", "spec_sparse_permille",
+        "blend_sort")]
 
 
 OPTION_NAMES = tuple(n for n, _ in Options._fields_ if n != "struct_bytes")
diff --git a/include/gigs_hip.h b/include/gigs_hip.h
--- a/include/gigs_hip.h
+++ b/include/gigs_hip.h
@@ -40,6 +40,7 @@
   int shade_bwd_rows;
   int spec_sparse;
   int spec_sparse_permille;
+  int blend_sort;
 } gigs_options;
 gigs_ctx* gigs_ctx_create(void);
 void gigs_ctx_destroy(gigs_ctx* ctx);
```

New measurement: 357.1 renders/s, median of 6. 1.2% higher.
